# syzhang092218-source/dgppo

Measured on AMD Instinct MI355X. Metric: env-steps/sec whole node, LidarSpread n=8 4096 envs, 1/2/4/8 GPUs, higher is better.
Workload: dtype f32

## Files before the change

dgppo_amd/csrc/graph_feats.hip:

```cpp
#include "graph_topo.h"

struct FeatArgs {
  dgppo_env_cfg cfg;
  Topo t;
  const float* agent; long agent_se, agent_st;
  const float* goal;
  const float* obst;
  const float* hits; long hits_se, hits_st;
  const int32_t* env_ids;
  int n_env, n_time;
  float* Xa;
  float* Xo;
  float* efeat;
  float* emask;
  int Fp;
  uint32_t rcp_fp, rcp_S;
};

template <int SD>
__global__ void graph_feats_kernel(FeatArgs a) {
  extern __shared__ float sm[];
  const dgppo_env_cfg& c = a.cfg;
  const Topo& t = a.t;
  const int g = blockIdx.x;
  const int e = g / a.n_time, tt = g - e * a.n_time;
  const int env = a.env_ids ? a.env_ids[e] : e;
  const int tid = threadIdx.x, nt = blockDim.x;
  const int n = t.n, ng = t.ng, S = t.S, Fp = a.Fp;
  const int n_on = t.Ns - n - ng;
  float* s_ag = sm;
  float* s_go = s_ag + n * SD;
  float* s_ob = s_go + ng * SD;
  float* s_fa = s_ob + n_on * SD;
  float* s_fg = s_fa + n * 4;
  const float* ag = a.agent + (size_t)env * a.agent_se + (size_t)tt * a.agent_st;
  for (int i = tid; i < n * SD; i += nt) s_ag[i] = ag[i];
  for (int i = tid; i < ng * SD; i += nt) s_go[i] = a.goal[(size_t)env * ng * SD + i];
  if (n_on > 0) {
    if (t.lidar) {
      const float* hp = a.hits + (size_t)env * a.hits_se + (size_t)tt * a.hits_st;
      for (int i = tid; i < n_on * 2; i += nt) {
        const int q = i >> 1, d = i & 1;
        s_ob[q * SD + d] = hp[i];
      }
      for (int i = tid; i < n_on * (SD - 2); i += nt) {
        const int q = i / (SD - 2), d = i - q * (SD - 2);
        s_ob[q * SD + 2 + d] = 0.0f;
      }
    } else {
      for (int i = tid; i < n_on * SD; i += nt) s_ob[i] = a.obst[(size_t)env * n_on * SD + i];
    }
  }
  __syncthreads();
  for (int i = tid; i < n + ng; i += nt) {
    const float* s = (i < n) ? s_ag + i * SD : s_go + (i - n) * SD;
    float* f = (i < n) ? s_fa + i * 4 : s_fg + (i - n) * 4;
    if constexpr (SD == 5) {
      f[0] = s[0]; f[1] = s[1]; f[2] = __fmul_rn(s[4], s[2]); f[3] = __fmul_rn(s[4], s[3]);
    } else {
      f[0] = s[0]; f[1] = s[1]; f[2] = s[2]; f[3] = s[3];
    }
  }
  __syncthreads();
  constexpr int ND = SD + 3;
  for (int idx = tid; idx < t.Ns * Fp; idx += nt) {
    const int nd = (int)__umulhi((uint32_t)idx, a.rcp_fp), col = idx - nd * Fp;
    float v = 0.0f;
    if (nd < n) v = (col < SD) ? s_ag[nd * SD + col] : ((col == SD + 2) ? 1.0f : 0.0f);
    else if (nd < n + ng) v = (col < SD) ? s_go[(nd - n) * SD + col] : ((col == SD + 1) ? 1.0f : 0.0f);
    else v = (col < SD) ? s_ob[(nd - n - ng) * SD + col] : ((col == SD) ? 1.0f : 0.0f);
    if (col >= ND) v = 0.0f;
    if (nd < n) a.Xa[((size_t)g * n + nd) * Fp + col] = v;
    else a.Xo[((size_t)g * (t.Ns - n) + (nd - n)) * Fp + col] = v;
  }
  for (int idx = tid; idx < n * S; idx += nt) {
    const int i = (int)__umulhi((uint32_t)idx, a.rcp_S), s = idx - i * S;
    float4 f;
    bool mask;
    const float* fi = s_fa + i * 4;
    const float px = s_ag[i * SD], py = s_ag[i * SD + 1];
    if (s < n) {
      const float* fj = s_fa + s * 4;
      f = make_float4(__fsub_rn(fi[0], fj[0]), __fsub_rn(fi[1], fj[1]), __fsub_rn(fi[2], fj[2]), __fsub_rn(fi[3], fj[3]));
      float d = __fadd_rn(dist_rn(__fsub_rn(px, s_ag[s * SD]), __fsub_rn(py, s_ag[s * SD + 1])), (i == s) ? c.eye_offset : 0.0f);
      mask = d < c.comm_radius;
    } else if (s < n + t.gs) {
      const int gi = t.spread ? (s - n) : i;
      const float* fg = s_fg + gi * 4;
      f = make_float4(__fsub_rn(fi[0], fg[0]), __fsub_rn(fi[1], fg[1]), __fsub_rn(fi[2], fg[2]), __fsub_rn(fi[3], fg[3]));
      mask = true;
    } else {
      const int m = s - n - t.gs;
      if (t.lidar) {
        const float* hp = s_ob + (i * t.per + m) * SD;
        const float lx = __fsub_rn(px, hp[0]), ly = __fsub_rn(py, hp[1]);
        f = make_float4(lx, ly, 0.0f, 0.0f);
        mask = dist_rn(lx, ly) < c.lidar_mask_radius;
      } else {
        const float* xo = s_ob + m * SD;
        const float* xi = s_ag + i * SD;
        f = make_float4(__fsub_rn(xi[0], xo[0]), __fsub_rn(xi[1], xo[1]), __fsub_rn(xi[2], xo[2]), __fsub_rn(xi[3], xo[3]));
        mask = dist_rn(__fsub_rn(xi[0], xo[0]), __fsub_rn(xi[1], xo[1])) < c.obs_mask_radius;
      }
    }
    reinterpret_cast<float4*>(a.efeat)[(size_t)g * n * S + idx] = f;
    a.emask[(size_t)g * n * S + idx] = mask ? 1.0f : 0.0f;
  }
}

extern "C" int32_t dgppo_graph_feats(const dgppo_env_cfg* cfg, const float* agent, int64_t agent_se, int64_t agent_st,
                                     const float* goal, const float* obst, const float* hits, int64_t hits_se,
                                     int64_t hits_st, const int32_t* env_ids, int32_t n_env, int32_t n_time, float* Xa,
                                     float* Xo, float* efeat, float* emask, int32_t Fp, void* stream) {
  int32_t rc = dgppo_validate_cfg(cfg);
  if (rc) return rc;
  DGPPO_REFUSE_VMAS(cfg, "dgppo_graph_feats", "dgppo_vmas_graph_feats");
  DGPPO_REQUIRE(n_env >= 0 && n_time >= 0, "graph_feats: negative counts");
  if (n_env == 0 || n_time == 0) return 0;
  DGPPO_REQUIRE(agent && goal && Xa && efeat && emask, "graph_feats: NULL operand");
  DGPPO_REQUIRE(Fp >= cfg->node_dim && Fp <= 32, "graph_feats: Fp must be in [node_dim, 32]");
  FeatArgs a;
  a.cfg = *cfg; a.t = make_topo(*cfg);
  const int n_on = a.t.Ns - a.t.n - a.t.ng;
  DGPPO_REQUIRE(n_on == 0 || Xo, "graph_feats: Xo is NULL");
  DGPPO_REQUIRE(a.t.Ns == a.t.n || Xo, "graph_feats: Xo is NULL");
  if (n_on > 0) {
    if (a.t.lidar) DGPPO_REQUIRE(hits, "graph_feats: hits is NULL");
    else DGPPO_REQUIRE(obst, "graph_feats: obst is NULL");
  }
  DGPPO_REQUIRE(((uintptr_t)efeat & 15) == 0, "graph_feats: efeat must be 16-byte aligned");
  a.agent = agent; a.agent_se = agent_se; a.agent_st = agent_st; a.goal = goal; a.obst = obst;
  a.hits = hits; a.hits_se = hits_se; a.hits_st = hits_st; a.env_ids = env_ids; a.n_env = n_env; a.n_time = n_time;
  a.Xa = Xa; a.Xo = Xo; a.efeat = efeat; a.emask = emask; a.Fp = Fp;
  a.rcp_fp = (uint32_t)((0x100000000ull + (uint64_t)Fp - 1) / (uint64_t)Fp);
  a.rcp_S = (uint32_t)((0x100000000ull + (uint64_t)a.t.S - 1) / (uint64_t)a.t.S);
  DGPPO_REQUIRE(Fp >= 2 && a.t.S >= 2 && (long)a.t.Ns * Fp < 65536 && (long)a.t.n * a.t.S < 65536, "graph_feats: sizes out of range");
  const int SD = cfg->state_dim;
  const size_t smem = sizeof(float) * ((size_t)a.t.n * SD + a.t.ng * SD + (size_t)n_on * SD + a.t.n * 4 + a.t.ng * 4);
  const long G = (long)n_env * n_time;
  if (SD == 5) hipLaunchKernelGGL(graph_feats_kernel<5>, dim3(G), dim3(128), smem, (hipStream_t)stream, a);
  else hipLaunchKernelGGL(graph_feats_kernel<4>, dim3(G), dim3(128), smem, (hipStream_t)stream, a);
  DGPPO_LAUNCH_CHECK();
  return 0;
}
```

dgppo_amd/csrc/nn_elem.hip:

```cpp
#include "common.h"
#include "nn_ln.h"

using f32x4 = __attribute__((ext_vector_type(4))) float;

__device__ inline float wave_sum(float v) {
#pragma unroll
  for (int o = 32; o >= 1; o >>= 1) v += __shfl_xor(v, o);
  return v;
}
template <int NV>
__device__ inline void block_atomic_sums(const float (&v)[NV], float* dst) {
  __shared__ float s_red[4][NV];
  const int lane = threadIdx.x & 63, wave = threadIdx.x >> 6;
#pragma unroll
  for (int k = 0; k < NV; ++k) {
    const float w = wave_sum(v[k]);
    if (lane == 0) s_red[wave][k] = w;
  }
  __syncthreads();
  if (threadIdx.x < NV) {
    float t = 0.0f;
    for (int w = 0; w < (int)(blockDim.x >> 6); ++w) t += s_red[w][threadIdx.x];
    atomicAdd(dst + threadIdx.x, t);
  }
}

__device__ inline float row16_sum(float v) {
  v += __int_as_float(__builtin_amdgcn_update_dpp(0, __float_as_int(v), 0xB1, 0xf, 0xf, false));
  v += __int_as_float(__builtin_amdgcn_update_dpp(0, __float_as_int(v), 0x4E, 0xf, 0xf, false));
  v += __int_as_float(__builtin_amdgcn_update_dpp(0, __float_as_int(v), 0x141, 0xf, 0xf, false));
  v += __int_as_float(__builtin_amdgcn_update_dpp(0, __float_as_int(v), 0x140, 0xf, 0xf, false));
  return v;
}

__global__ void __launch_bounds__(256) ln_relu_fwd_kernel(const float* __restrict__ x, const float* __restrict__ gamma,
                                                          const float* __restrict__ beta, float* __restrict__ y,
                                                          float* __restrict__ stats, int M) {
  const int lane = threadIdx.x & 63, li = lane & 15, lq = lane >> 4;
  const int wave = (blockIdx.x * blockDim.x + threadIdx.x) >> 6;
  const int nw = (gridDim.x * blockDim.x) >> 6;
  const float4 g = reinterpret_cast<const float4*>(gamma)[li], b = reinterpret_cast<const float4*>(beta)[li];
  for (int row0 = wave * 4; row0 < M; row0 += nw * 4) {
    const int row = row0 + lq;
    const bool ok = row < M;
    const float4 v = reinterpret_cast<const float4*>(x)[(size_t)(ok ? row : M - 1) * 16 + li];
    const float mean = row16_sum((v.x + v.y) + (v.z + v.w)) * (1.0f / 64.0f);
    const float mean2 = row16_sum((v.x * v.x + v.y * v.y) + (v.z * v.z + v.w * v.w)) * (1.0f / 64.0f);
    const float var = ln_fast_var(mean, mean2);
    const float rstd = rsqrtf(var + 1e-6f);
    float4 o;
    o.x = relu_nan((v.x - mean) * rstd * g.x + b.x);
    o.y = relu_nan((v.y - mean) * rstd * g.y + b.y);
    o.z = relu_nan((v.z - mean) * rstd * g.z + b.z);
    o.w = relu_nan((v.w - mean) * rstd * g.w + b.w);
    if (ok) {
      reinterpret_cast<float4*>(y)[(size_t)row * 16 + li] = o;
      if (stats != nullptr && li == 0) reinterpret_cast<float2*>(stats)[row] = make_float2(mean, rstd);
    }
  }
}

__global__ void __launch_bounds__(256) ln_relu_bwd_kernel(const float* __restrict__ x, const float* __restrict__ y,
                                                          const float* __restrict__ stats, const float* __restrict__ gamma,
                                                          const float* __restrict__ dy, float* __restrict__ dx,
                                                          float* __restrict__ dgamma, float* __restrict__ dbeta, int M) {
  const int lane = threadIdx.x & 63, li = lane & 15, lq = lane >> 4;
  const int wave = (blockIdx.x * blockDim.x + threadIdx.x) >> 6;
  const int nw = (gridDim.x * blockDim.x) >> 6;
  const float4 g = reinterpret_cast<const float4*>(gamma)[li];
  float dg[4] = {0.f, 0.f, 0.f, 0.f}, db[4] = {0.f, 0.f, 0.f, 0.f};
  for (int row0 = wave * 4; row0 < M; row0 += nw * 4) {
    const int row = row0 + lq;
    const bool ok = row < M;
    const size_t o = (size_t)(ok ? row : M - 1) * 16 + li;
    const float4 xv = reinterpret_cast<const float4*>(x)[o], yv = reinterpret_cast<const float4*>(y)[o];
    const float4 dv = reinterpret_cast<const float4*>(dy)[o];
    const float2 st = reinterpret_cast<const float2*>(stats)[ok ? row : M - 1];
    const float mean = st.x, rstd = st.y;
    const float xh[4] = {(xv.x - mean) * rstd, (xv.y - mean) * rstd, (xv.z - mean) * rstd, (xv.w - mean) * rstd};
    const float dl[4] = {(ok && yv.x > 0.0f) ? dv.x : 0.0f, (ok && yv.y > 0.0f) ? dv.y : 0.0f,
                         (ok && yv.z > 0.0f) ? dv.z : 0.0f, (ok && yv.w > 0.0f) ? dv.w : 0.0f};
    const float gg[4] = {g.x, g.y, g.z, g.w};
    float dxh[4], s1 = 0.0f, s2 = 0.0f;
#pragma unroll
    for (int q = 0; q < 4; ++q) {
      dg[q] += dl[q] * xh[q];
      db[q] += dl[q];
      dxh[q] = dl[q] * gg[q];
      s1 += dxh[q];
      s2 += dxh[q] * xh[q];
    }
    const float m1 = row16_sum(s1) * (1.0f / 64.0f), m2 = row16_sum(s2) * (1.0f / 64.0f);
    if (ok)
      reinterpret_cast<float4*>(dx)[o] = make_float4(rstd * (dxh[0] - m1 - xh[0] * m2), rstd * (dxh[1] - m1 - xh[1] * m2),
                                                     rstd * (dxh[2] - m1 - xh[2] * m2), rstd * (dxh[3] - m1 - xh[3] * m2));
  }
  __shared__ float red[2][16][64];
  const int slot = (threadIdx.x >> 6) * 4 + lq;
#pragma unroll
  for (int q = 0; q < 4; ++q) { red[0][slot][li * 4 + q] = dg[q]; red[1][slot][li * 4 + q] = db[q]; }
  __syncthreads();
  if (threadIdx.x < 128) {
    const int which = threadIdx.x >> 6;
    float v = 0.0f;
#pragma unroll
    for (int sidx = 0; sidx < 16; ++sidx) v += red[which][sidx][lane];
    atomicAdd((which ? dbeta : dgamma) + lane, v);
  }
}

extern "C" int32_t dgppo_ln_relu_fwd(const float* x, const float* gamma, const float* beta, float* y, float* stats,
                                     int32_t M, void* stream) {
  DGPPO_REQUIRE(M >= 0, "ln_relu_fwd: M < 0");
  if (M == 0) return 0;
  DGPPO_REQUIRE(x && gamma && beta && y, "ln_relu_fwd: NULL operand");
  const int grid = min(cdiv(M, 16), 2048);
  hipLaunchKernelGGL(ln_relu_fwd_kernel, dim3(grid), dim3(256), 0, (hipStream_t)stream, x, gamma, beta, y, stats, M);
  DGPPO_LAUNCH_CHECK();
  return 0;
}

extern "C" int32_t dgppo_ln_relu_bwd(const float* x, const float* y, const float* stats, const float* gamma,
                                     const float* dy, float* dx, float* dgamma, float* dbeta, int32_t M, void* stream) {
  DGPPO_REQUIRE(M >= 0, "ln_relu_bwd: M < 0");
  if (M == 0) return 0;
  DGPPO_REQUIRE(x && y && stats && gamma && dy && dx && dgamma && dbeta, "ln_relu_bwd: NULL operand");
  const int grid = min(cdiv(M, 16), 256);
  hipLaunchKernelGGL(ln_relu_bwd_kernel, dim3(grid), dim3(256), 0, (hipStream_t)stream, x, y, stats, gamma, dy, dx, dgamma,
                     dbeta, M);
  DGPPO_LAUNCH_CHECK();
  return 0;
}

#define GRU_H 64
#define GRU_WL 194
#define GRU_HL 66

struct GruArgs {
  const float* gi;
  const float* Wh;
  const float* bhn;
  const float* h0;
  float* hs;
  float* hprev;
  float* gates;
  const float* dhs;
  float* dgi;
  float* dgh;
  float* dhn;
  int n_seq, T, n_inner;
};

__device__ inline size_t gru_row(const GruArgs& a, int s, int tau) {
  const int grp = s / a.n_inner, i = s - grp * a.n_inner;
  return ((size_t)grp * a.T + tau) * a.n_inner + i;
}
__device__ inline float sigmoidf_(float x) { return 1.0f / (1.0f + expf(-x)); }
__device__ inline float gate_sigmoid(float x) { return __builtin_amdgcn_rcpf(1.0f + __expf(-x)); }
__device__ inline float gate_tanh(float x) { return fmaf(2.0f, __builtin_amdgcn_rcpf(1.0f + __expf(-2.0f * x)), -1.0f); }


#define GRU_LDS_BARRIER() asm volatile("s_waitcnt lgkmcnt(0)\n\ts_barrier" ::: "memory")

template <int RTW>
__global__ void __launch_bounds__(256) gru_fwd_kernel(GruArgs a) {
  extern __shared__ float sm[];
  constexpr int RB = 16 * RTW;
  constexpr int HSLOT = RB * 16 / 256 > 0 ? RB * 16 / 256 : 1;
  const int tid = threadIdx.x, lane = tid & 63, w = tid >> 6, li = lane & 15, lq = lane >> 4;
  const int c = w * 16 + li;
  float breg[16][3];
#pragma unroll
  for (int kk = 0; kk < 16; ++kk)
#pragma unroll
    for (int t = 0; t < 3; ++t) breg[kk][t] = a.Wh[(size_t)(kk * 4 + lq) * 192 + t * 64 + c];
  const float bn = a.bhn[c];
  const int n_tiles = (a.n_seq + RB - 1) / RB;
  const float4 z4 = make_float4(0.f, 0.f, 0.f, 0.f);
  float hpf[HSLOT][4];
  auto fetch_h0 = [&](int tile) {
#pragma unroll
    for (int u = 0; u < HSLOT; ++u) {
      int idx = u * 256 + tid;
      idx = idx < RB * 16 ? idx : RB * 16 - 1;
      const int r = idx >> 4, q = idx & 15;
      int s = tile * RB + r;
      s = s < a.n_seq ? s : a.n_seq - 1;
      float4 v = z4;
      if (a.h0 != nullptr) v = reinterpret_cast<const float4*>(a.h0 + (size_t)s * GRU_H)[q];
      hpf[u][0] = v.x; hpf[u][1] = v.y; hpf[u][2] = v.z; hpf[u][3] = v.w;
    }
  };
  auto commit_h0 = [&](float* dst) {
#pragma unroll
    for (int u = 0; u < HSLOT; ++u) {
      const int idx = u * 256 + tid, r = idx >> 4, q = idx & 15;
      if (idx < RB * 16) { float* d = dst + r * GRU_HL + 4 * q; d[0] = hpf[u][0]; d[1] = hpf[u][1]; d[2] = hpf[u][2]; d[3] = hpf[u][3]; }
    }
  };
  int tile = blockIdx.x;
  if (tile < n_tiles) { fetch_h0(tile); commit_h0(sm); }
  __syncthreads();
  int cur = 0;
  for (; tile < n_tiles; tile += gridDim.x) {
    const int s0 = tile * RB;
    const int nxt = tile + gridDim.x;
    if (nxt < n_tiles) fetch_h0(nxt);
    int row0[RTW][4];
    bool ok[RTW][4];
#pragma unroll
    for (int rt = 0; rt < RTW; ++rt)
#pragma unroll
      for (int r = 0; r < 4; ++r) {
        int s = s0 + rt * 16 + lq * 4 + r;
        ok[rt][r] = s < a.n_seq;
        s = ok[rt][r] ? s : a.n_seq - 1;
        int rw = s;
        if (a.T != 1 && a.n_inner != 1) { const int grp = s / a.n_inner; rw = grp * a.T * a.n_inner + (s - grp * a.n_inner); }
        else if (a.T != 1) rw = s * a.T;
        row0[rt][r] = rw;
      }
    float gn[RTW][4][3];
    auto fetch_gi = [&](int tau) {
#pragma unroll
      for (int rt = 0; rt < RTW; ++rt)
#pragma unroll
        for (int r = 0; r < 4; ++r) {
          const float* gp = a.gi + (size_t)(row0[rt][r] + tau * a.n_inner) * 192 + c;
          gn[rt][r][0] = gp[0]; gn[rt][r][1] = gp[64]; gn[rt][r][2] = gp[128];
        }
    };
    fetch_gi(0);
    for (int tau = 0; tau < a.T; ++tau) {
      const float* hs_cur = sm + cur * (RB * GRU_HL);
      float* hs_nxt = sm + (cur ^ 1) * (RB * GRU_HL);
      float g[RTW][4][3];
#pragma unroll
      for (int rt = 0; rt < RTW; ++rt)
#pragma unroll
        for (int r = 0; r < 4; ++r) { g[rt][r][0] = gn[rt][r][0]; g[rt][r][1] = gn[rt][r][1]; g[rt][r][2] = gn[rt][r][2]; }
      if (tau + 1 < a.T) fetch_gi(tau + 1);
      __builtin_amdgcn_sched_barrier(0);
      float areg[RTW][16];
#pragma unroll
      for (int rt = 0; rt < RTW; ++rt)
#pragma unroll
        for (int kk = 0; kk < 16; ++kk) areg[rt][kk] = hs_cur[(rt * 16 + li) * GRU_HL + kk * 4 + lq];
      __builtin_amdgcn_sched_barrier(0);
      f32x4 acc[RTW][3];
#pragma unroll
      for (int rt = 0; rt < RTW; ++rt)
#pragma unroll
        for (int t = 0; t < 3; ++t) acc[rt][t] = f32x4{0.f, 0.f, 0.f, 0.f};
#pragma unroll
      for (int kk = 0; kk < 16; ++kk)
#pragma unroll
        for (int rt = 0; rt < RTW; ++rt)
#pragma unroll
          for (int t = 0; t < 3; ++t) acc[rt][t] = __builtin_amdgcn_mfma_f32_16x16x4f32(areg[rt][kk], breg[kk][t], acc[rt][t], 0, 0, 0);
#pragma unroll
      for (int rt = 0; rt < RTW; ++rt)
#pragma unroll
        for (int r = 0; r < 4; ++r) {
          const int rl = rt * 16 + lq * 4 + r;
          const float hp = hs_cur[rl * GRU_HL + c];
          const float rg = gate_sigmoid(g[rt][r][0] + acc[rt][0][r]);
          const float zg = gate_sigmoid(g[rt][r][1] + acc[rt][1][r]);
          const float hn = acc[rt][2][r] + bn;
          const float ng = gate_tanh(g[rt][r][2] + rg * hn);
          const float hnew = (1.0f - zg) * ng + zg * hp;
          hs_nxt[rl * GRU_HL + c] = hnew;
          if (ok[rt][r]) {
            const size_t row = (size_t)(row0[rt][r] + tau * a.n_inner);
            a.hs[row * GRU_H + c] = hnew;
            if (a.hprev != nullptr) a.hprev[row * GRU_H + c] = hp;
            if (a.gates != nullptr) {
              float* gs = a.gates + row * 256;
              gs[c] = rg; gs[64 + c] = zg; gs[128 + c] = ng; gs[192 + c] = hn;
            }
          }
        }
      GRU_LDS_BARRIER();
      cur ^= 1;
    }
    if (nxt < n_tiles) {
      commit_h0(sm + cur * (RB * GRU_HL));
      GRU_LDS_BARRIER();
    }
  }
}

template <int RTW, bool DHN_ONLY>
__global__ void __launch_bounds__(256) gru_bwd_kernel(GruArgs a) {
  extern __shared__ float sm[];
  constexpr int RB = 16 * RTW;
  const int tid = threadIdx.x, lane = tid & 63, w = tid >> 6, li = lane & 15, lq = lane >> 4;
  const int c = w * 16 + li;
  float breg[48];
#pragma unroll
  for (int kk = 0; kk < 48; ++kk) breg[kk] = a.Wh[(size_t)c * 192 + kk * 4 + lq];
  const int n_tiles = (a.n_seq + RB - 1) / RB;
  int cur = 0;
  for (int tile = blockIdx.x; tile < n_tiles; tile += gridDim.x) {
    const int s0 = tile * RB;
    int row0[RTW][4];
    bool ok[RTW][4];
#pragma unroll
    for (int rt = 0; rt < RTW; ++rt)
#pragma unroll
      for (int r = 0; r < 4; ++r) {
        int s = s0 + rt * 16 + lq * 4 + r;
        ok[rt][r] = s < a.n_seq;
        s = ok[rt][r] ? s : a.n_seq - 1;
        int rw = s;
        if (a.T != 1 && a.n_inner != 1) { const int grp = s / a.n_inner; rw = grp * a.T * a.n_inner + (s - grp * a.n_inner); }
        else if (a.T != 1) rw = s * a.T;
        row0[rt][r] = rw;
      }
    float rg[RTW][4], zg[RTW][4], ng[RTW][4], hn[RTW][4], hp[RTW][4], du[RTW][4], dh[RTW][4];
    auto fetch = [&](int tau) {
#pragma unroll
      for (int rt = 0; rt < RTW; ++rt)
#pragma unroll
        for (int r = 0; r < 4; ++r) {
          const size_t row = (size_t)(row0[rt][r] + tau * a.n_inner);
          const float* gs = a.gates + row * 256 + c;
          rg[rt][r] = gs[0]; zg[rt][r] = gs[64]; ng[rt][r] = gs[128]; hn[rt][r] = gs[192];
          hp[rt][r] = a.hprev[row * GRU_H + c];
          du[rt][r] = a.dhs[row * GRU_H + c];
        }
    };
#pragma unroll
    for (int rt = 0; rt < RTW; ++rt)
#pragma unroll
      for (int r = 0; r < 4; ++r) dh[rt][r] = 0.0f;
    fetch(a.T - 1);
    for (int tau = a.T - 1; tau >= 0; --tau) {
      float* s_g = sm + cur * (RB * GRU_WL);
#pragma unroll
      for (int rt = 0; rt < RTW; ++rt)
#pragma unroll
        for (int r = 0; r < 4; ++r) {
          const int rl = rt * 16 + lq * 4 + r;
          const float d = ok[rt][r] ? dh[rt][r] + du[rt][r] : 0.0f;
          const float dz = d * (hp[rt][r] - ng[rt][r]);
          const float dn = d * (1.0f - zg[rt][r]);
          const float dan = dn * (1.0f - ng[rt][r] * ng[rt][r]);
          const float dhn = dan * rg[rt][r];
          const float dar = dan * hn[rt][r] * rg[rt][r] * (1.0f - rg[rt][r]);
          const float daz = dz * zg[rt][r] * (1.0f - zg[rt][r]);
          dh[rt][r] = d * zg[rt][r];
          s_g[rl * GRU_WL + c] = dar;
          s_g[rl * GRU_WL + 64 + c] = daz;
          s_g[rl * GRU_WL + 128 + c] = dhn;
          if (ok[rt][r]) {
            const size_t row = (size_t)(row0[rt][r] + tau * a.n_inner);
            float* o = a.dgi + row * 192 + c;
            o[0] = dar; o[64] = daz; o[128] = dan;
            if (DHN_ONLY) {
              a.dhn[row * GRU_H + c] = dhn;
            } else {
              float* p = a.dgh + row * 192 + c;
              p[0] = dar; p[64] = daz; p[128] = dhn;
            }
          }
        }
      GRU_LDS_BARRIER();
      if (tau > 0) fetch(tau - 1);
      __builtin_amdgcn_sched_barrier(0);
      f32x4 acc[RTW];
#pragma unroll
      for (int rt = 0; rt < RTW; ++rt) acc[rt] = f32x4{0.f, 0.f, 0.f, 0.f};
#pragma unroll
      for (int k0 = 0; k0 < 48; k0 += 16) {
        float areg[RTW][16];
#pragma unroll
        for (int rt = 0; rt < RTW; ++rt)
#pragma unroll
          for (int u = 0; u < 16; ++u) areg[rt][u] = s_g[(rt * 16 + li) * GRU_WL + (k0 + u) * 4 + lq];
        __builtin_amdgcn_sched_barrier(0);
#pragma unroll
        for (int u = 0; u < 16; ++u)
#pragma unroll
          for (int rt = 0; rt < RTW; ++rt) acc[rt] = __builtin_amdgcn_mfma_f32_16x16x4f32(areg[rt][u], breg[k0 + u], acc[rt], 0, 0, 0);
      }
#pragma unroll
      for (int rt = 0; rt < RTW; ++rt)
#pragma unroll
        for (int r = 0; r < 4; ++r) dh[rt][r] += acc[rt][r];
      cur ^= 1;
    }
    GRU_LDS_BARRIER();
  }
}

static int gru_resident(const void* fn, size_t smem) {
  int per_cu = 0, dev = 0, cus = 256;
  if (hipOccupancyMaxActiveBlocksPerMultiprocessor(&per_cu, fn, 256, smem) != hipSuccess || per_cu < 1) per_cu = 1;
  if (hipGetDevice(&dev) != hipSuccess ||
      hipDeviceGetAttribute(&cus, hipDeviceAttributeMultiprocessorCount, dev) != hipSuccess || cus < 1) cus = 256;
  return per_cu * cus;
}

static int32_t gru_check(const GruArgs& a) {
  DGPPO_REQUIRE(a.n_seq >= 0 && a.T >= 1 && a.n_inner >= 1, "gru: bad sizes n_seq=%d T=%d n_inner=%d", a.n_seq, a.T, a.n_inner);
  DGPPO_REQUIRE(a.n_seq % a.n_inner == 0, "gru: n_seq must be a multiple of n_inner");
  return 0;
}

extern "C" int32_t dgppo_gru_fwd(const float* gi, const float* Wh, const float* bhn, const float* h0, float* hs,
                                 float* hprev, float* gates, int32_t n_seq, int32_t T, int32_t n_inner, void* stream) {
  GruArgs a{};
  a.gi = gi; a.Wh = Wh; a.bhn = bhn; a.h0 = h0; a.hs = hs; a.hprev = hprev; a.gates = gates;
  a.n_seq = n_seq; a.T = T; a.n_inner = n_inner;
  int32_t rc = gru_check(a);
  if (rc) return rc;
  if (n_seq == 0) return 0;
  DGPPO_REQUIRE(gi && Wh && bhn && hs, "gru_fwd: NULL operand");
  if (cdiv(n_seq, 32) >= 512) {
    const size_t smem = sizeof(float) * 2 * 32 * GRU_HL;
    static thread_local int cap = 0;
    if (cap == 0) cap = gru_resident(reinterpret_cast<const void*>(&gru_fwd_kernel<2>), smem);
    const int tiles = cdiv(n_seq, 32);
    hipLaunchKernelGGL(gru_fwd_kernel<2>, dim3(tiles < cap ? tiles : cap), dim3(256), smem, (hipStream_t)stream, a);
  } else {
    const size_t smem = sizeof(float) * 2 * 16 * GRU_HL;
    static thread_local int cap = 0;
    if (cap == 0) cap = gru_resident(reinterpret_cast<const void*>(&gru_fwd_kernel<1>), smem);
    const int tiles = cdiv(n_seq, 16);
    hipLaunchKernelGGL(gru_fwd_kernel<1>, dim3(tiles < cap ? tiles : cap), dim3(256), smem, (hipStream_t)stream, a);
  }
  DGPPO_LAUNCH_CHECK();
  return 0;
}

template <bool DHN_ONLY>
static int32_t gru_bwd_launch(GruArgs a, hipStream_t stream) {
  int32_t rc = gru_check(a);
  if (rc) return rc;
  if (a.n_seq == 0) return 0;
  DGPPO_REQUIRE(a.dhs && a.Wh && a.hprev && a.gates && a.dgi && (DHN_ONLY ? a.dhn : a.dgh), "gru_bwd: NULL operand");
  if (cdiv(a.n_seq, 32) >= 512) {
    const size_t smem = sizeof(float) * 2 * 32 * GRU_WL;
    static thread_local int cap = 0;
    if (cap == 0) cap = gru_resident(reinterpret_cast<const void*>(&gru_bwd_kernel<2, DHN_ONLY>), smem);
    const int tiles = cdiv(a.n_seq, 32);
    hipLaunchKernelGGL((gru_bwd_kernel<2, DHN_ONLY>), dim3(tiles < cap ? tiles : cap), dim3(256), smem, stream, a);
  } else {
    const size_t smem = sizeof(float) * 2 * 16 * GRU_WL;
    static thread_local int cap = 0;
    if (cap == 0) cap = gru_resident(reinterpret_cast<const void*>(&gru_bwd_kernel<1, DHN_ONLY>), smem);
    const int tiles = cdiv(a.n_seq, 16);
    hipLaunchKernelGGL((gru_bwd_kernel<1, DHN_ONLY>), dim3(tiles < cap ? tiles : cap), dim3(256), smem, stream, a);
  }
  DGPPO_LAUNCH_CHECK();
  return 0;
}

extern "C" int32_t dgppo_gru_bwd(const float* dhs, const float* Wh, const float* hprev, const float* gates, float* dgi,
                                 float* dgh, int32_t n_seq, int32_t T, int32_t n_inner, void* stream) {
  GruArgs a{};
  a.dhs = dhs; a.Wh = Wh; a.hprev = (float*)hprev; a.gates = (float*)gates; a.dgi = dgi; a.dgh = dgh;
  a.n_seq = n_seq; a.T = T; a.n_inner = n_inner;
  return gru_bwd_launch<false>(a, (hipStream_t)stream);
}

extern "C" int32_t dgppo_gru_bwd_dhn(const float* dhs, const float* Wh, const float* hprev, const float* gates, float* dgi,
                                     float* dhn, int32_t n_seq, int32_t T, int32_t n_inner, void* stream) {
  GruArgs a{};
  a.dhs = dhs; a.Wh = Wh; a.hprev = (float*)hprev; a.gates = (float*)gates; a.dgi = dgi; a.dhn = dhn;
  a.n_seq = n_seq; a.T = T; a.n_inner = n_inner;
  return gru_bwd_launch<true>(a, (hipStream_t)stream);
}

#define STD_INIT_INV (-0.43275212956718856f)
#define STD_MIN 1e-5f
#define THRESH 0.999f
#define INV_THRESH 3.8002011672502f
#define LOG_EPS (-6.907755278982137f)
#define HALF_LOG_2PI 0.9189385332046727f
#define LOG2_F 0.6931471805599453f

__device__ inline float softplusf_(float x) { return (x > 20.0f) ? x : log1pf(expf(x)); }
#define NDTR_SERIES_BELOW (-10.0f)
__device__ inline float ndtr_tail_series(float z2) { return 1.0f - 1.0f / z2 + 3.0f / (z2 * z2) - 15.0f / (z2 * z2 * z2); }
__device__ inline float log_ndtrf_(float z) {
  if (z > NDTR_SERIES_BELOW) return logf(0.5f * erfcf(-z * 0.70710678118654752f));
  const float z2 = z * z;
  return -0.5f * z2 - logf(-z) - HALF_LOG_2PI + logf(ndtr_tail_series(z2));
}
__device__ inline float dlog_ndtrf_(float z) {
  if (z > NDTR_SERIES_BELOW) return 0.3989422804014327f * expf(-0.5f * z * z) / (0.5f * erfcf(-z * 0.70710678118654752f));
  return -z / ndtr_tail_series(z * z);
}
__device__ inline float tanh_fldj(float x) { return 2.0f * (LOG2_F - x - softplusf_(-2.0f * x)); }

struct HeadArgs {
  const float* ms;
  const float* eps;
  const float* action_in;
  float* action;
  float* log_pi;
  float* entropy;
  int rows, n_agents, mode;
  const float* log_pi_old;
  const float* adv;
  float* dms;
  float* stats;
  float clip_eps, coef_ent, inv_count;
};

__device__ inline float tn_log_prob_dim(float act, float mu, float sd) {
  const float ac = fminf(fmaxf(act, -THRESH), THRESH);
  if (ac <= -THRESH) return log_ndtrf_((-INV_THRESH - mu) / sd) - LOG_EPS;
  if (ac >= THRESH) return log_ndtrf_(-(INV_THRESH - mu) / sd) - LOG_EPS;
  const float x = atanhf(ac);
  const float z = (x - mu) / sd;
  return -0.5f * z * z - logf(sd) - HALF_LOG_2PI - tanh_fldj(x);
}

__global__ void __launch_bounds__(256) policy_head_kernel(HeadArgs a) {
  float acc[4] = {0.0f, 0.0f, 0.0f, 0.0f};
  const int rows_pad = (a.rows + 255) & ~255;
  for (int row_raw = blockIdx.x * blockDim.x + threadIdx.x; row_raw < rows_pad; row_raw += gridDim.x * blockDim.x) {
  const bool valid = row_raw < a.rows;
  const int row = valid ? row_raw : a.rows - 1;
  const float4 m = reinterpret_cast<const float4*>(a.ms)[row];
  const float mu[2] = {m.x, m.y};
  const float st[2] = {m.z, m.w};
  float sd[2];
  for (int d = 0; d < 2; ++d) sd[d] = softplusf_(st[d] + STD_INIT_INV) + STD_MIN;
  if (a.mode == 1) {
    if (valid) {
      a.action[row * 2] = tanhf(mu[0]);
      a.action[row * 2 + 1] = tanhf(mu[1]);
    }
    continue;
  }
  float act[2];
  if (a.mode == 0) {
    for (int d = 0; d < 2; ++d) act[d] = tanhf(mu[d] + sd[d] * a.eps[row * 2 + d]);
    if (valid) {
      a.action[row * 2] = act[0];
      a.action[row * 2 + 1] = act[1];
      a.log_pi[row] = tn_log_prob_dim(act[0], mu[0], sd[0]) + tn_log_prob_dim(act[1], mu[1], sd[1]);
    }
    continue;
  }
  act[0] = a.action_in[row * 2];
  act[1] = a.action_in[row * 2 + 1];
  const int ag = row % a.n_agents;
  float lp = 0.0f, ent = 0.0f;
  float dlp_dmu[2], dlp_dsd[2], dent_dmu[2], dent_dsd[2];
  for (int d = 0; d < 2; ++d) {
    const float ac = fminf(fmaxf(act[d], -THRESH), THRESH);
    if (ac <= -THRESH) {
      const float u = (-INV_THRESH - mu[d]) / sd[d];
      lp += log_ndtrf_(u) - LOG_EPS;
      const float r = dlog_ndtrf_(u);
      dlp_dmu[d] = -r / sd[d];
      dlp_dsd[d] = -r * u / sd[d];
    } else if (ac >= THRESH) {
      const float u = (mu[d] - INV_THRESH) / sd[d];
      lp += log_ndtrf_(u) - LOG_EPS;
      const float r = dlog_ndtrf_(u);
      dlp_dmu[d] = r / sd[d];
      dlp_dsd[d] = -r * u / sd[d];
    } else {
      const float x = atanhf(ac);
      const float z = (x - mu[d]) / sd[d];
      lp += -0.5f * z * z - logf(sd[d]) - HALF_LOG_2PI - tanh_fldj(x);
      dlp_dmu[d] = z / sd[d];
      dlp_dsd[d] = (z * z - 1.0f) / sd[d];
    }
    const float eh = a.eps[ag * 2 + d];
    const float y = mu[d] + sd[d] * eh;
    ent += 0.5f + HALF_LOG_2PI + logf(sd[d]) + tanh_fldj(y);
    const float th = tanhf(y);
    dent_dmu[d] = -2.0f * th;
    dent_dsd[d] = 1.0f / sd[d] - 2.0f * th * eh;
  }
  if (valid) {
    a.log_pi[row] = lp;
    a.entropy[row] = ent;
  }
  if (a.dms == nullptr) continue;
  const float A = a.adv[row];
  const float rho = expf(lp - a.log_pi_old[row]);
  const float l1 = -rho * A;
  const float l2 = -fminf(fmaxf(rho, 1.0f - a.clip_eps), 1.0f + a.clip_eps) * A;
  const float lsel = fmaxf(l1, l2);
  const float dl_dlp = ((l2 > l1) ? 0.0f : -rho * A) * a.inv_count;
  const float dl_dent = -a.coef_ent * a.inv_count;
  if (valid) {
    float4 o;
    const float dsd0 = dl_dlp * dlp_dsd[0] + dl_dent * dent_dsd[0];
    const float dsd1 = dl_dlp * dlp_dsd[1] + dl_dent * dent_dsd[1];
    o.x = dl_dlp * dlp_dmu[0] + dl_dent * dent_dmu[0];
    o.y = dl_dlp * dlp_dmu[1] + dl_dent * dent_dmu[1];
    o.z = dsd0 * sigmoidf_(st[0] + STD_INIT_INV);
    o.w = dsd1 * sigmoidf_(st[1] + STD_INIT_INV);
    reinterpret_cast<float4*>(a.dms)[row] = o;
  }
  if (valid) {
    acc[0] += lsel; acc[1] += ent; acc[2] += (l2 > l1) ? 1.0f : 0.0f; acc[3] += fabsf(rho - 1.0f);
  }
  }
  if (a.mode == 2 && a.dms != nullptr) block_atomic_sums<4>(acc, a.stats);
}

extern "C" int32_t dgppo_policy_head(const float* ms, const float* eps, const float* action_in, float* action,
                                     float* log_pi, float* entropy, int32_t rows, int32_t n_agents, int32_t mode,
                                     const float* log_pi_old, const float* adv, float* dms, float* stats, float clip_eps,
                                     float coef_ent, void* stream) {
  DGPPO_REQUIRE(rows >= 0 && n_agents >= 1 && mode >= 0 && mode <= 2, "policy_head: bad arguments");
  if (rows == 0) return 0;
  DGPPO_REQUIRE(ms, "policy_head: ms is NULL");
  DGPPO_REQUIRE(((uintptr_t)ms & 15) == 0, "policy_head: ms must be 16-byte aligned");
  if (mode == 0) DGPPO_REQUIRE(eps && action && log_pi, "policy_head(sample): NULL operand");
  if (mode == 1) DGPPO_REQUIRE(action, "policy_head(mode): NULL operand");
  if (mode == 2) {
    DGPPO_REQUIRE(eps && action_in && log_pi && entropy, "policy_head(eval): NULL operand");
    if (dms) DGPPO_REQUIRE(log_pi_old && adv && stats && ((uintptr_t)dms & 15) == 0, "policy_head(eval+loss): NULL operand");
  }
  HeadArgs a{};
  a.ms = ms; a.eps = eps; a.action_in = action_in; a.action = action; a.log_pi = log_pi; a.entropy = entropy;
  a.rows = rows; a.n_agents = n_agents; a.mode = mode; a.log_pi_old = log_pi_old; a.adv = adv; a.dms = dms; a.stats = stats;
  a.clip_eps = clip_eps; a.coef_ent = coef_ent; a.inv_count = 1.0f / (float)rows;
  const int blocks = cdiv(rows, 256);
  hipLaunchKernelGGL(policy_head_kernel, dim3(blocks < 512 ? blocks : 512), dim3(256), 0, (hipStream_t)stream, a);
  DGPPO_LAUNCH_CHECK();
  return 0;
}

__global__ void __launch_bounds__(256) value_loss_kernel(const float* __restrict__ v, const float* __restrict__ target,
                                                         float* __restrict__ dv, float* __restrict__ stats, int count,
                                                         float count_f) {
  float l[1] = {0.0f};
  for (int i = blockIdx.x * blockDim.x + threadIdx.x; i < count; i += gridDim.x * blockDim.x) {
    const float d = v[i] - target[i];
    dv[i] = d / count_f;
    l[0] += 0.5f * d * d;
  }
  block_atomic_sums<1>(l, stats);
}

extern "C" int32_t dgppo_value_loss(const float* v, const float* target, float* dv, float* stats, int32_t count,
                                    void* stream) {
  DGPPO_REQUIRE(count >= 0, "value_loss: count < 0");
  if (count == 0) return 0;
  DGPPO_REQUIRE(v && target && dv && stats, "value_loss: NULL operand");
  const int blocks = cdiv(count, 256);
  hipLaunchKernelGGL(value_loss_kernel, dim3(blocks < 256 ? blocks : 256), dim3(256), 0, (hipStream_t)stream, v, target, dv,
                     stats, count, (float)count);
  DGPPO_LAUNCH_CHECK();
  return 0;
}

__global__ void mean_agents_kernel(const float* __restrict__ x, float* __restrict__ y, int G, int n, int D, int backward,
                                   const float* __restrict__ relu_mask) {
  const int idx = blockIdx.x * blockDim.x + threadIdx.x;
  if (backward) {
    if (idx >= G * n * D) return;
    const int d = idx % D, g = idx / (n * D);
    const float v = (backward == 2) ? y[idx] + x[(size_t)g * D + d] : x[(size_t)g * D + d] / (float)n;
    y[idx] = (relu_mask == nullptr || relu_mask[idx] > 0.0f) ? v : 0.0f;
  } else {
    if (idx >= G * D) return;
    const int d = idx % D, g = idx / D;
    float acc = 0.0f;
    for (int i = 0; i < n; ++i) acc += x[((size_t)g * n + i) * D + d];
    y[idx] = acc / (float)n;
  }
}

extern "C" int32_t dgppo_mean_agents(const float* x, float* y, int32_t G, int32_t n, int32_t D, int32_t backward,
                                     const float* relu_mask, void* stream) {
  DGPPO_REQUIRE(G >= 0 && n >= 1 && D >= 1, "mean_agents: bad sizes");
  DGPPO_REQUIRE(backward >= 0 && backward <= 2, "mean_agents: backward must be 0, 1 or 2");
  if (G == 0) return 0;
  DGPPO_REQUIRE(x && y, "mean_agents: NULL operand");
  const long total = backward ? (long)G * n * D : (long)G * D;
  hipLaunchKernelGGL(mean_agents_kernel, dim3(cdiv(total, 256)), dim3(256), 0, (hipStream_t)stream, x, y, G, n, D, backward,
                     backward ? relu_mask : nullptr);
  DGPPO_LAUNCH_CHECK();
  return 0;
}

__global__ void relu_bwd_kernel(float* __restrict__ dy, const float* __restrict__ y, long count) {
  const long i = (long)blockIdx.x * blockDim.x + threadIdx.x;
  if (i < count && !(y[i] > 0.0f)) dy[i] = 0.0f;
}

extern "C" int32_t dgppo_relu_bwd(float* dy, const float* y, int64_t count, void* stream) {
  DGPPO_REQUIRE(count >= 0, "relu_bwd: count < 0");
  if (count == 0) return 0;
  DGPPO_REQUIRE(dy && y, "relu_bwd: NULL operand");
  hipLaunchKernelGGL(relu_bwd_kernel, dim3(cdiv(count, 256)), dim3(256), 0, (hipStream_t)stream, dy, y, (long)count);
  DGPPO_LAUNCH_CHECK();
  return 0;
}
```

dgppo_amd/engine.py:

```python
from __future__ import annotations

import dataclasses
from typing import Callable, Dict, Optional

import numpy as np
import os
import torch

from . import _native as N
from . import nets
from . import ops_algo as OA
from . import ops_env as OE
from . import ops_nn as K
from .utils import checkpoint as CK


@dataclasses.dataclass
class Hyper:
    gamma: float = 0.99
    gae_lambda: float = 0.95
    clip_eps: float = 0.25
    coef_ent: float = 1e-2
    max_grad_norm: float = 2.0
    lr_actor: float = 3e-4
    lr_Vl: float = 1e-3
    lr_Vh: float = 1e-3
    batch_size: int = 16384
    rnn_step: int = 16
    alpha: float = 10.0
    cbf_eps: float = 1e-2
    cbf_weight: float = 1.0
    cbf_schedule: bool = True
    train_steps: int = 100000
    actor_gnn_layers: int = 2
    Vl_gnn_layers: int = 2
    Vh_gnn_layers: int = 1
    use_rnn: bool = True
    use_lstm: bool = False
    rnn_layers: int = 1
    lagr_init: float = 0.78
    lr_lagr: float = 1e-7
    cost_weight: float = 0.0
    cost_schedule: bool = False


class RolloutData:

    def __init__(self, cfg: N.EnvCfg, B: int, T: int, device, stochastic: bool, carry_dim: int = nets.HID):
        n = cfg.n_agents
        self.cfg, self.B, self.T, self.stochastic = cfg, B, T, stochastic
        z = lambda *s: torch.empty(*s, device=device)
        step, env = OE.record_fields(cfg)
        self.step_tm = {k: z(T + 1, B, *shape) for k, shape in step.items()}
        self.env = {k: z(B, *shape) for k, shape in env.items()}
        self.step: Dict[str, torch.Tensor] = {}
        for k in OE.STEP_FIELDS:
            setattr(self, k + "_tm", self.step_tm.get(k))
            setattr(self, k, None)
        for k in OE.ENV_FIELDS:
            setattr(self, k, self.env.get(k))
        self.action_tm = z(T, B, n, 2)
        self.log_pi_tm = z(T, B, n) if stochastic else None
        self.rnn_tm = z(T + 1, B, n, carry_dim)
        self.reward_tm = z(T, B)
        self.cost_tm = z(T, B, n, cfg.n_cost)
        self._env_major = False
        views = {k: v.unbind(0) for k, v in self.step_tm.items()}
        self.states_tm = [OE.State({k: v[t] for k, v in views.items()}, self.env) for t in range(T + 1)]

    def finalize(self):
        if self._env_major:
            return self

        def tr(name, x):
            if x is None:
                return None
            cur = getattr(self, name, None)
            want = (x.shape[1], x.shape[0]) + tuple(x.shape[2:])
            if cur is None or tuple(cur.shape) != want:
                cur = torch.empty(want, device=x.device, dtype=x.dtype)
            cur.copy_(x.transpose(0, 1))
            return cur
        for k, v in self.step_tm.items():
            self.step[k] = tr(k, v)
            setattr(self, k, self.step[k])
        self.actions = tr("actions", self.action_tm)
        self.log_pis = tr("log_pis", self.log_pi_tm) if self.stochastic else None
        self._rnn_em = tr("_rnn_em", self.rnn_tm)
        self.rnn_states = self._rnn_em[:, :self.T] if self.stochastic else self._rnn_em[:, 1:]
        self.rewards = tr("rewards", self.reward_tm)
        self.costs = tr("costs", self.cost_tm)
        self._env_major = True
        return self


class OptState:
    def __init__(self, n: int, device):
        self.m = torch.zeros(n, device=device)
        self.v = torch.zeros(n, device=device)
        self.state = torch.zeros(N.OPT_STATE_FLOATS, device=device)


class Engine:
    def __init__(self, cfg: N.EnvCfg, hyper: Hyper, device, T: int = 128,
                 allreduce: Optional[Callable[[torch.Tensor], None]] = None, world: int = 1, prepass_graphs: int = 1 << 20,
                 use_graphs: bool = False, multi_stream: bool = False, algo: str = "dgppo", rank: int = 0):
        self.cfg, self.hp, self.device, self.T = cfg, hyper, device, T
        assert algo in ("dgppo", "informarl", "hcbfcrpo", "informarl_lagr"), algo
        self.algo = algo
        self.use_graphs = use_graphs and os.environ.get("DGPPO_HIPGRAPH", "1") != "0"
        self.multi_stream = multi_stream and os.environ.get("DGPPO_MULTI_STREAM", "1") != "0"
        self._side_streams = None
        self._ro_cache: Dict[tuple, dict] = {}
        self._upd_graph: dict = {}
        self.n_cost = cfg.n_cost
        spec = [("policy", "policy", hyper.actor_gnn_layers, 2), ("Vl", "Vl", hyper.Vl_gnn_layers, 1)]
        if algo == "dgppo":
            spec.append(("Vh", "Vh", hyper.Vh_gnn_layers, self.n_cost))
        elif algo == "informarl_lagr":
            spec.append(("Vh", "Vhg", hyper.Vh_gnn_layers, self.n_cost))
        def rnn_kw(name):
            if not hyper.use_rnn:
                return dict(rnn="none", rnn_layers=0)
            if name == "Vh" and algo == "dgppo":
                return dict(rnn="gru", rnn_layers=1)
            return dict(rnn="lstm" if hyper.use_lstm else "gru", rnn_layers=hyper.rnn_layers)
        sizes = [nets.make_layout(kind, cfg.node_dim, layers, n_out, **rnn_kw(k)).size for k, kind, layers, n_out in spec]
        offs, tot = [], 0
        for sz in sizes:
            offs.append(tot)
            tot += (sz + 3) // 4 * 4
        self.flat_grads = torch.zeros(tot + 4 * 8, device=device)
        self.n_reduced = tot + 3 * 8
        self.stats = self.flat_grads[tot:tot + 32].view(4, 8)
        built = {k: nets.Net(kind, cfg, layers, n_out, device, grads=self.flat_grads[o:o + sz], **rnn_kw(k))
                 for (k, kind, layers, n_out), o, sz in zip(spec, offs, sizes)}
        if algo == "informarl_lagr":
            self.lagr = torch.full((cfg.n_agents, self.n_cost), float(hyper.lagr_init), device=device)
            self.lagr_sums = torch.zeros(cfg.n_agents * self.n_cost, device=device)
        self.policy, self.Vl, self.Vh = built["policy"], built["Vl"], built.get("Vh")
        self.HC = self.policy.carry_dim
        self.opt = {k: OptState(net.layout.size, device) for k, net in self.nets.items()}
        self.arena = nets.Arena(device)
        self.allreduce = allreduce
        self.world, self.rank = int(world), int(rank)
        assert self.world >= 1 and (allreduce is not None or self.world == 1), "world > 1 needs an allreduce"
        assert 0 <= self.rank < self.world, f"rank {rank} outside world {world}"
        self.prepass_graphs = int(os.environ.get("DGPPO_PREPASS_GRAPHS", prepass_graphs))
        self.lam_pow = OA.lam_pow_table(hyper.gae_lambda, T, device)
        self.eps_hat = torch.zeros(cfg.n_agents, 2, device=device)
        self.reset_failed = torch.zeros(1, dtype=torch.int32, device=device)
        self.grad_hook: Optional[Callable[[str, nets.Net, int], None]] = None
        self._mb = 0

    @property
    def nets(self) -> Dict[str, nets.Net]:
        d = {"policy": self.policy, "Vl": self.Vl}
        if self.Vh is not None:
            d["Vh"] = self.Vh
        return d

    def set_entropy_noise(self, seed: int):
        OE.randn(seed, 0, self.eps_hat.view(-1))

    _CFG_IDENTITY = ("kind", "n_agents", "n_obs", "n_rays", "top_k", "node_dim", "n_cost")

    def _identity(self) -> dict:
        ident = {"algo": CK.encode_str(self.algo)}
        ident.update({f"cfg.{k}": int(getattr(self.cfg, k)) for k in self._CFG_IDENTITY})
        for f in dataclasses.fields(Hyper):
            v = getattr(self.hp, f.name)
            ident[f"hyper.{f.name}"] = int(v) if isinstance(v, (bool, int)) else float(v)
        ident["T"], ident["world"] = int(self.T), int(self.world)
        ident.update({f"size.{k}": int(net.layout.size) for k, net in self.nets.items()})
        return ident

    def _state_tensors(self) -> Dict[str, torch.Tensor]:
        t = {}
        for k, net in self.nets.items():
            opt = self.opt[k]
            t.update({f"{k}/params": net.params, f"{k}/m": opt.m, f"{k}/v": opt.v, f"{k}/state": opt.state})
        t["eps_hat"] = self.eps_hat
        if self.algo == "informarl_lagr":
            t["lagr"] = self.lagr
        return t

    def state_dict(self) -> dict:
        out = {"identity": self._identity()}
        for path, x in self._state_tensors().items():
            node = out
            *dirs, leaf = path.split("/")
            for d in dirs:
                node = node.setdefault(d, {})
            node[leaf] = x.detach().cpu().numpy().copy()
        return out

    def load_state_dict(self, d: dict) -> None:
        mine, theirs = self._identity(), d.get("identity", {})
        show = lambda v: repr(CK.decode_str(v)) if isinstance(v, np.ndarray) else repr(v)
        for k, v in mine.items():
            if k not in theirs:
                raise ValueError(f"state dict does not fit this engine: it has no identity field '{k}'")
            if not np.array_equal(np.asarray(v), np.asarray(theirs[k])):
                raise ValueError(f"state dict does not fit this engine: '{k}' is {show(theirs[k])} there, {show(v)} here")
        src = {}
        for path, x in self._state_tensors().items():
            node = d
            for part in path.split("/"):
                node = node.get(part) if isinstance(node, dict) else None
            if not isinstance(node, np.ndarray) or node.dtype != np.float32 or node.shape != tuple(x.shape):
                raise ValueError(f"state dict does not fit this engine: '{path}' is not a float32 array of shape {tuple(x.shape)}")
            src[path] = node
        for path, x in self._state_tensors().items():
            x.copy_(torch.from_numpy(src[path]).to(self.device))
        for net in self.nets.values():
            net.prepare()

    def _feats(self, tag, st: OE.State, n_env, n_time=1, slots=1, env_ids=None):
        f = nets.GraphFeats(self.cfg, n_env * n_time, self.arena, tag)
        return f.compute_record(st.step, slots, st.env, env_ids, n_env, n_time)

    def _rollout_steps(self, ro: RolloutData, eps, B: int, stochastic: bool):
        cfg, T, n = self.cfg, self.T, self.cfg.n_agents
        tag = "ro" if stochastic else "rod"
        for t in range(T):
            feats = self._feats(tag, ro.states_tm[t], B)
            act = self.policy.forward(feats, n_seq=B * n, T=1, h0=ro.rnn_tm[t].view(B * n, self.HC), tag=tag,
                                      hs_out=ro.rnn_tm[t + 1].view(B * n, self.HC), train=False)
            a_t = ro.action_tm[t].view(B * n, 2)
            if stochastic:
                K.policy_head(act["ms"], eps[t], None, a_t, ro.log_pi_tm[t].view(B * n), None, n, 0)
            else:
                K.policy_head(act["ms"], None, None, a_t, None, None, n, 1)
            OE.step(cfg, ro.states_tm[t], ro.action_tm[t], ro.states_tm[t + 1], ro.reward_tm[t], ro.cost_tm[t])

    def rollout(self, seeds: torch.Tensor, stochastic: bool, noise_seed: int = 0) -> RolloutData:
        cfg, T = self.cfg, self.T
        B = int(seeds.shape[0])
        n = cfg.n_agents
        slot = None
        if self.use_graphs:
            slot = self._ro_cache.setdefault((B, stochastic), {"ro": None, "graph": None, "gen": -1, "calls": 0})
            if slot["ro"] is None:
                slot["ro"] = RolloutData(cfg, B, T, self.device, stochastic, self.HC)
            ro = slot["ro"]
            ro._env_major = False
        else:
            ro = RolloutData(cfg, B, T, self.device, stochastic, self.HC)
        OE.reset(cfg, seeds, ro.states_tm[0], self.reset_failed)
        ro.rnn_tm[0].zero_()
        eps = None
        if stochastic:
            eps = self.arena.get("ro.eps", T, B * n, 2)
            OE.randn_rows(noise_seed, eps.view(T, B * n * 2), self.world * B * n * 2, self.rank * B * n * 2)
        if slot is None:
            self._rollout_steps(ro, eps, B, stochastic)
            return ro
        slot["calls"] += 1
        if slot["graph"] is not None and slot["gen"] != self._arena_generation():
            slot["graph"] = None
        if slot["graph"] is not None:
            slot["graph"].replay()
            K.FLOPS[0] += slot.get("flops", 0.0)
            return ro
        f0 = K.FLOPS[0]
        self._rollout_steps(ro, eps, B, stochastic)
        slot["flops"] = K.FLOPS[0] - f0
        if not slot.get("failed", False):
            graph = torch.cuda.CUDAGraph()
            try:
                f1 = K.FLOPS[0]
                with torch.cuda.graph(graph, capture_error_mode="thread_local"):
                    self._rollout_steps(ro, eps, B, stochastic)
                K.FLOPS[0] = f1 + slot["flops"]
                slot["graph"], slot["gen"] = graph, self._arena_generation()
                graph.replay()
            except Exception as ex:
                slot["failed"] = True
                torch.cuda.synchronize()
                print(f"[dgppo_amd] HIP-graph capture of the rollout loop failed ({type(ex).__name__}: {ex}); "
                      f"continuing with eager launches", flush=True)
        return ro

    def _update_generation(self) -> int:
        return self.arena.generation + sum(net.arena.generation + net.ws_arena.generation for net in self.nets.values())

    def _arena_generation(self) -> int:
        return self.arena.generation + self.policy.arena.generation

    def rollout_pair(self, seeds: torch.Tensor, det_seeds: torch.Tensor, noise_seed: int = 0):
        if not (self.multi_stream and self.device.type == "cuda"):
            return self.rollout(seeds, True, noise_seed), self.rollout(det_seeds, False)
        main = torch.cuda.current_stream(self.device)
        s0, s1 = self._net_streams()[:2]
        out = [None, None]
        for k, (st, sd, stoch) in enumerate(((s0, seeds, True), (s1, det_seeds, False))):
            st.wait_stream(main)
            with torch.cuda.stream(st):
                out[k] = self.rollout(sd, stoch, noise_seed if stoch else 0)
        main.wait_stream(s0)
        main.wait_stream(s1)
        return out[0], out[1]

    def _block_feats(self, tag, ro: RolloutData, e0, Eb, t0, n_time, env_ids=None):
        envs = slice(e0, None) if env_ids is None else slice(None)
        st = OE.State({k: v[envs, t0] for k, v in ro.step.items()}, {k: v[envs] for k, v in ro.env.items()})
        return self._feats(tag, st, Eb, n_time, self.T + 1, env_ids)

    def _vh_carry(self, ro: RolloutData, e0: int, Eb: int) -> torch.Tensor:
        return ro.rnn_states[e0:e0 + Eb][..., :nets.HID]

    def values_prepass(self, ro: RolloutData, want_Vl: bool, want_Vh: bool = True):
        cfg, T, B = self.cfg, self.T, ro.B
        n, nh, H = cfg.n_agents, self.n_cost, nets.HID
        kind = "ro" if ro.stochastic else "det"
        Vl_buf = self.arena.get(f"tg.Vl.{kind}", B, T + 1) if want_Vl else None
        Vh_buf = self.arena.get(f"tg.Vh.{kind}", B, T + 1, n, nh) if want_Vh else None
        block = max(1, min(B, self.prepass_graphs // (T + 1)))
        for e0 in range(0, B, block):
            Eb = min(block, B - e0)
            feats = self._block_feats("pre", ro, e0, Eb, 0, T + 1)
            if want_Vl:
                act = self.Vl.forward(feats, n_seq=Eb, T=T + 1, h0=None, tag="pre", train=False)
                Vl_buf[e0:e0 + Eb].copy_(act["v"].view(Eb, T + 1))
            if not want_Vh:
                continue
            fin = self._block_feats("fin", ro, e0, Eb, T, 1)
            HC = self.HC
            h_last = self.arena.get("pre.hlast", Eb * n, HC)
            h_last.view(Eb, n, HC).copy_(ro.rnn_states[e0:e0 + Eb, T - 1])
            h0_all = self.arena.get("pre.h0all", Eb, T + 1, n, H)
            hstar = self.arena.get("pre.hstar", Eb * n, HC)
            self.policy.forward(fin, n_seq=Eb * n, T=1, h0=h_last, tag="fin", hs_out=hstar, train=False)
            h0_all[:, :T].copy_(self._vh_carry(ro, e0, Eb))
            h0_all[:, T].copy_(hstar.view(Eb, n, HC)[..., :H])
            act = self.Vh.forward(feats, n_seq=Eb * (T + 1) * n, T=1, h0=h0_all.view(-1, H) if self.hp.use_rnn else None,
                                  tag="pre", train=False)
            Vh_buf[e0:e0 + Eb].copy_(act["v"].view(Eb, T + 1, n, nh))
        return Vl_buf, Vh_buf

    def require_landscape(self):
        if self.algo != "dgppo":
            why = {"informarl_lagr": "its constraint-value net carries its own scan state, which needs a sequence pass first"}
            raise ValueError(f"vh_landscape: algo '{self.algo}' is not supported: "
                             + why.get(self.algo, "it has no constraint-value network"))
        if self.cfg.is_vmas:
            raise ValueError("vh_landscape: VMASReverseTransport is not supported")

    def vh_landscape(self, ro: RolloutData, env_index: int, agent_id: int, frame_ids, xs, ys,
                     events: Optional[list] = None) -> torch.Tensor:
        self.require_landscape()
        cfg, T = self.cfg, self.T
        n, nh, H = cfg.n_agents, self.n_cost, nets.HID
        ro.finalize()
        if not 0 <= int(env_index) < ro.B:
            raise ValueError(f"vh_landscape: env_index {env_index} outside [0, {ro.B})")
        if not 0 <= int(agent_id) < n:
            raise ValueError(f"vh_landscape: agent_id {agent_id} outside [0, {n})")
        frames = np.asarray(frame_ids, dtype=np.int64).reshape(-1)
        if frames.size == 0 or frames.min() < 0 or frames.max() >= T:
            raise ValueError(f"vh_landscape: frame_ids must be a non-empty subset of [0, {T})")
        xs, ys = K.sweep_axis(xs, "xs", self.device), K.sweep_axis(ys, "ys", self.device)
        nx, ny, F = int(xs.numel()), int(ys.numel()), int(frames.size)
        e = int(env_index)
        step = {k: v[e] for k, v in ro.step.items()}
        env = {k: v[e] for k, v in ro.env.items()}
        rc, rs = OE._rays(cfg, self.device)
        carry = self._vh_carry(ro, e, 1)[0] if self.hp.use_rnn else None
        out = torch.empty(F, ny, nx, n, nh, device=self.device)
        ids_dev = torch.from_numpy(frames.astype(np.int32)).to(self.device)
        cap = max(1, self.prepass_graphs)
        fb = max(1, cap // (ny * nx))
        yb = ny if cap >= ny * nx else max(1, cap // nx)
        xb = nx if cap >= nx else cap
        for f0 in range(0, F, fb):
            f1 = min(F, f0 + fb)
            fr = frames[f0:f1]
            for y0 in range(0, ny, yb):
                y1 = min(ny, y0 + yb)
                for x0 in range(0, nx, xb):
                    x1 = min(nx, x0 + xb)
                    P = (y1 - y0) * (x1 - x0)
                    Gb = (f1 - f0) * P
                    feats = nets.GraphFeats(cfg, Gb, self.arena, "land")
                    ev = [torch.cuda.Event(enable_timing=True) for _ in range(3)] if events is not None else None
                    if ev:
                        ev[0].record()
                    feats.compute_sweep(step, env, ids_dev[f0:f1], f1 - f0, agent_id, xs[x0:x1], ys[y0:y1], rc, rs,
                                        frame_max=int(fr.max()))
                    if ev:
                        ev[1].record()
                    h0 = None
                    if carry is not None:
                        h0 = self.arena.get("land.h0", Gb * n, H)
                        for j, t in enumerate(fr):
                            h0.view(f1 - f0, P, n, H)[j].copy_(carry[int(t)].unsqueeze(0).expand(P, n, H))
                    act = self.Vh.forward(feats, n_seq=Gb * n, T=1, h0=h0, tag="land", train=False)
                    out[f0:f1, y0:y1, x0:x1].copy_(act["v"].view(f1 - f0, y1 - y0, x1 - x0, n, nh))
                    if ev:
                        ev[2].record()
                        events.append(tuple(ev))
        return out

    def cost_landscape(self, ro: RolloutData, env_index: int, agent_id: int, frame_ids, xs, ys) -> torch.Tensor:
        cfg, T = self.cfg, self.T
        if cfg.is_vmas:
            raise ValueError("cost_landscape: VMASReverseTransport is not supported")
        n = cfg.n_agents
        ro.finalize()
        if not 0 <= int(env_index) < ro.B:
            raise ValueError(f"cost_landscape: env_index {env_index} outside [0, {ro.B})")
        if not 0 <= int(agent_id) < n:
            raise ValueError(f"cost_landscape: agent_id {agent_id} outside [0, {n})")
        frames = np.asarray(frame_ids, dtype=np.int64).reshape(-1)
        if frames.size == 0 or frames.min() < 0 or frames.max() >= T:
            raise ValueError(f"cost_landscape: frame_ids must be a non-empty subset of [0, {T})")
        xs, ys = K.sweep_axis(xs, "xs", self.device), K.sweep_axis(ys, "ys", self.device)
        nx, ny, F = int(xs.numel()), int(ys.numel()), int(frames.size)
        e = int(env_index)
        step = {k: v[e] for k, v in ro.step.items()}
        env = {k: v[e] for k, v in ro.env.items()}
        rc, rs = OE._rays(cfg, self.device)
        out = torch.empty(F, ny, nx, n, self.n_cost, device=self.device)
        K.cost_sweep(cfg, step["agent"], n * cfg.state_dim, env.get("obst"), step.get("hits"), n * cfg.top_k * 2, rc, rs,
                     frames, F, int(agent_id), xs, ys, out.view(F * ny * nx, n, self.n_cost))
        return out

    def cbf_weight_at(self, step: int) -> float:
        hp = self.hp
        w = hp.cbf_weight
        if hp.cbf_schedule:
            if step >= int(hp.train_steps * 0.5):
                w *= 2
            if step >= int(hp.train_steps * 0.75):
                w *= 2
        return w

    def cost_weight_at(self, step: int) -> float:
        hp = self.hp
        w = hp.cost_weight
        if hp.cost_schedule:
            if step >= int(hp.train_steps * 0.5):
                w *= 5
            if step >= int(hp.train_steps * 0.75):
                w *= 5
        return w

    def targets_hcbfcrpo(self, ro: RolloutData, step: int):
        cfg, T, B, hp = self.cfg, self.T, ro.B, self.hp
        n, nh, dev = cfg.n_agents, self.n_cost, self.device
        Vl, _ = self.values_prepass(ro, want_Vl=True, want_Vh=False)
        fin = OE.State({k: v[:, T].contiguous() for k, v in ro.step.items()}, ro.env)
        A = self.arena
        fin_cost = A.get("tg.fin_cost", B, n, nh)
        OE.step(cfg, fin, torch.zeros(B, n, 2, device=dev), fin.like(), torch.empty(B, device=dev), fin_cost)
        Vh = A.get("tg.Vh.crafted", B, T + 1, n, nh)
        Vh[:, :T].copy_(ro.costs)
        Vh[:, T].copy_(fin_cost)
        Qh = A.get("tg.Qh", B, T, n, nh)
        Ql = A.get("tg.Ql", B, T)
        OA.gae(ro.costs, ro.rewards, Vh, Vl, self.lam_pow, hp.gamma, hp.gae_lambda, Qh, Ql)
        adv = A.get("tg.adv", B, T, n)
        self.stats.zero_()
        OA.advantage(Ql, Vl, Vh, cfg.dt, hp.alpha, hp.cbf_eps, self.cbf_weight_at(step), adv, self.stats[3])
        return dict(Vl=Vl, Vh=Vh, Ql=Ql, Qh=Qh, adv=adv)

    def targets_informarl(self, ro: RolloutData, step: int):
        cfg, T, B, hp = self.cfg, self.T, ro.B, self.hp
        n, nh, dev = cfg.n_agents, self.n_cost, self.device
        Vl, _ = self.values_prepass(ro, want_Vl=True, want_Vh=False)
        A = self.arena
        Vh = A.get("tg.Vh.bcast", B, T + 1, n, nh)
        Vh.copy_(Vl.view(B, T + 1, 1, 1).expand(B, T + 1, n, nh))
        shaped = A.get("tg.shaped", B, T)
        OA.shaped_reward(ro.rewards, ro.costs, self.cost_weight_at(step), shaped)
        Qh = A.get("tg.Qh", B, T, n, nh)
        Ql = A.get("tg.Ql", B, T)
        OA.gae(ro.costs, shaped, Vh, Vl, self.lam_pow, hp.gamma, hp.gae_lambda, Qh, Ql)
        adv = A.get("tg.adv", B, T, n)
        self.stats.zero_()
        OA.advantage(Ql, Vl, None, cfg.dt, 0.0, 0.0, 0.0, adv, self.stats[3])
        return dict(Vl=Vl, Ql=Ql, Qh=Qh, adv=adv)

    def targets_lagr(self, ro: RolloutData, step: int):
        cfg, T, B, hp = self.cfg, self.T, ro.B, self.hp
        n, nh, A = cfg.n_agents, self.n_cost, self.arena
        Vl, _ = self.values_prepass(ro, want_Vl=True, want_Vh=False)
        Vh = A.get("tg.Vh.lagr", B, T + 1, n, nh)
        block = max(1, min(B, self.prepass_graphs // (T + 1)))
        for e0 in range(0, B, block):
            Eb = min(block, B - e0)
            feats = self._block_feats("pre", ro, e0, Eb, 0, T + 1)
            act = self.Vh.forward(feats, n_seq=Eb * n, T=T + 1, h0=None, tag="pre", train=False)
            Vh[e0:e0 + Eb].copy_(act["v"].view(Eb, T + 1, n, nh))
        cpos = A.get("tg.costs_pos", B, T, n, nh)
        OA.relu_fwd(ro.costs, cpos)
        Qh = A.get("tg.Qh", B, T, n, nh)
        Ql = A.get("tg.Ql", B, T)
        OA.gae(cpos, ro.rewards, Vh, Vl, self.lam_pow, hp.gamma, hp.gae_lambda, Qh, Ql)
        adv = A.get("tg.adv", B, T, n)
        Ah = A.get("tg.Ah", B, T, n, nh)
        self.stats.zero_()
        OA.advantage_lagr(Ql, Vl, Qh, Vh, self.lagr, adv, Ah)
        return dict(Vl=Vl, Vh=Vh, Ql=Ql, Qh=Qh, adv=adv, Ah=Ah)

    def _net_streams(self):
        if self._side_streams is None:
            self._side_streams = [torch.cuda.Stream(self.device) for _ in range(3)]
        return self._side_streams

    def _opt_step(self, name: str, lr: float):
        net, opt = self.nets[name], self.opt[name]
        if self.grad_hook is not None:
            self.grad_hook(name, net, self._mb)
        OA.clip_adam_step(net.params, net.grads, opt.m, opt.v, opt.state, lr, self.hp.max_grad_norm,
                          grad_scale=1.0 / self.world)
        net.prepare()

    def targets(self, ro: RolloutData, det: RolloutData, step: int):
        cfg, T, B, hp = self.cfg, self.T, ro.B, self.hp
        n, nh = cfg.n_agents, self.n_cost
        Vl, Vh = self.values_prepass(ro, want_Vl=True)
        _, Vh_det = self.values_prepass(det, want_Vl=False)
        A = self.arena
        Qh = A.get("tg.Qh", B, T, n, nh)
        Ql = A.get("tg.Ql", B, T)
        OA.gae(ro.costs, ro.rewards, Vh, Vl, self.lam_pow, hp.gamma, hp.gae_lambda, Qh, Ql)
        Qh_det = A.get("tg.Qh_det", B, T, n, nh)
        Ql_det = A.get("tg.Ql_det", B, T)
        OA.gae(det.costs, det.rewards, Vh_det, Vl, self.lam_pow, hp.gamma, hp.gae_lambda, Qh_det, Ql_det)
        adv = A.get("tg.adv", B, T, n)
        self.stats.zero_()
        OA.advantage(Ql, Vl, Vh, cfg.dt, hp.alpha, hp.cbf_eps, self.cbf_weight_at(step), adv, self.stats[3])
        return dict(Vl=Vl, Vh=Vh, Vh_det=Vh_det, Ql=Ql, Qh=Qh, Qh_det=Qh_det, adv=adv)

    def update(self, ro: RolloutData, det: RolloutData, step: int, perm: np.ndarray) -> dict:
        cfg, T, B, hp = self.cfg, self.T, ro.B, self.hp
        n, nh, H = cfg.n_agents, self.n_cost, nets.HID
        informarl = self.algo in ("informarl", "hcbfcrpo")
        lagr = self.algo == "informarl_lagr"
        import time as _time
        th = [_time.perf_counter()]
        ro.finalize()
        if self.algo == "dgppo":
            det.finalize()
        assert B * T >= hp.batch_size, "n_env_train * T must be >= batch_size (dgppo.py:153)"
        Eb = hp.batch_size // T
        assert B % Eb == 0 and T % hp.rnn_step == 0, "B % (batch_size // T) == 0 and T % rnn_step == 0 required (SURVEY A.11)"
        C = T // hp.rnn_step
        tg = (self.targets_informarl(ro, step) if self.algo == "informarl" else
              self.targets_hcbfcrpo(ro, step) if self.algo == "hcbfcrpo" else
              self.targets_lagr(ro, step) if lagr else self.targets(ro, det, step))
        th.append(_time.perf_counter())
        idx_all = torch.from_numpy(np.ascontiguousarray(perm.astype(np.int64))).to(self.device)
        n_mb = B // Eb
        G = Eb * T
        R = G * n
        is_cuda = self.device.type == "cuda"
        reduce = self.allreduce is not None
        A = self.arena
        mb_idx = A.get("mb.idx", Eb, dtype=torch.int64)
        mb_idx32 = A.get("mb.idx32", Eb, dtype=torch.int32)
        Ql_mb = A.get("mb.Ql", Eb, T)
        act_mb = A.get("mb.act", Eb, T, n, 2)
        lp_old_mb = A.get("mb.lp_old", Eb, T, n)
        adv_mb = A.get("mb.adv", Eb, T, n)
        if self.algo == "dgppo":
            h0_det = A.get("mb.h0_det", Eb, T, n, H)
            Qh_det_mb = A.get("mb.Qh_det", Eb, T, n, nh)
        if lagr:
            Qh_mb = A.get("mb.Qh", Eb, T, n, nh)
            Vh_mb = A.get("mb.Vh", Eb, T + 1, n, nh)
            Ah_mb = A.get("mb.Ah", Eb, T, n, nh)

        ctx = {}

        def lagr_step(apply_now: bool):
            full = self.policy.forward(ctx["feats"], n_seq=Eb * n, T=T, h0=None, tag="lg", train=False)
            lp_full = A.get("mb.lp_full", R)
            K.policy_head(full["ms"], self.eps_hat, act_mb.view(R, 2), None, lp_full, A.get("mb.ent_full", R), n, 2)
            if apply_now:
                OA.lagr_update(lp_full.view(Eb, T, n), lp_old_mb, Vh_mb, Ah_mb, self.lagr, self.lagr_sums, hp.gamma, hp.lr_lagr)
            else:
                OA.lagr_sums(lp_full.view(Eb, T, n), lp_old_mb, Vh_mb, Ah_mb, self.lagr_sums, hp.gamma)

        def body_pre():
            main = torch.cuda.current_stream(self.device) if is_cuda else None
            side = self._net_streams() if (self.multi_stream and main is not None) else None
            self.stats[:3].zero_()
            feats = ctx["feats"] = self._block_feats("mb", ro, 0, Eb, 0, T, env_ids=mb_idx32)
            torch.index_select(tg["Ql"], 0, mb_idx, out=Ql_mb)
            if self.algo == "dgppo":
                feats_det = self._block_feats("mbd", det, 0, Eb, 0, T, env_ids=mb_idx32)
                if self.HC == H:
                    torch.index_select(det.rnn_states, 0, mb_idx, out=h0_det)
                else:
                    full = A.get("mb.h0_det_full", Eb, T, n, self.HC)
                    torch.index_select(det.rnn_states, 0, mb_idx, out=full)
                    h0_det.copy_(full[..., :H])
                torch.index_select(tg["Qh_det"], 0, mb_idx, out=Qh_det_mb)
            if lagr:
                torch.index_select(tg["Qh"], 0, mb_idx, out=Qh_mb)
                torch.index_select(tg["Vh"], 0, mb_idx, out=Vh_mb)
                torch.index_select(tg["Ah"], 0, mb_idx, out=Ah_mb)
            torch.index_select(ro.actions, 0, mb_idx, out=act_mb)
            torch.index_select(ro.log_pis, 0, mb_idx, out=lp_old_mb)
            torch.index_select(tg["adv"], 0, mb_idx, out=adv_mb)

            def update_Vl():
                act = self.Vl.forward(feats, n_seq=Eb * C, T=hp.rnn_step, h0=None, tag="tr")
                dv = A.get("mb.dv", G, 1)
                K.value_loss(act["v"], Ql_mb.view(G, 1), dv, self.stats[0])
                self.Vl.zero_grads()
                self.Vl.backward(act, dv)
                if not reduce:
                    self._opt_step("Vl", hp.lr_Vl)

            def update_Vh():
                if lagr:
                    act = self.Vh.forward(feats, n_seq=Eb * C * n, T=hp.rnn_step, h0=None, tag="tr")
                    target = Qh_mb
                else:
                    act = self.Vh.forward(feats_det, n_seq=R, T=1, h0=h0_det.view(R, H) if hp.use_rnn else None, tag="tr")
                    target = Qh_det_mb
                dvh = A.get("mb.dvh", R, nh)
                K.value_loss(act["v"], target.view(R, nh), dvh, self.stats[1])
                self.Vh.zero_grads()
                self.Vh.backward(act, dvh)
                if not reduce:
                    self._opt_step("Vh", hp.lr_Vh)

            def update_policy():
                act = self.policy.forward(feats, n_seq=Eb * C * n, T=hp.rnn_step, h0=None, tag="tr")
                lp = A.get("mb.lp", R)
                ent = A.get("mb.ent", R)
                dms = A.get("mb.dms", R, 4)
                K.policy_head(act["ms"], self.eps_hat, act_mb.view(R, 2), None, lp, ent, n, 2, lp_old_mb.view(R),
                              adv_mb.view(R), dms, self.stats[2], hp.clip_eps, hp.coef_ent)
                self.policy.zero_grads()
                self.policy.backward(act, dms)
                if not reduce:
                    self._opt_step("policy", hp.lr_actor)
                if lagr and not reduce:
                    lagr_step(apply_now=True)

            if informarl:
                update_Vh = lambda: None
            if side is None:
                update_Vl(); update_Vh(); update_policy()
            else:
                ready = main.record_event()
                for fn, st in ((update_policy, side[0]), (update_Vl, side[1]), (update_Vh, side[2])):
                    with torch.cuda.stream(st):
                        st.wait_event(ready)
                        fn()
                for st in side:
                    main.wait_stream(st)

        def body_post():
            self._opt_step("Vl", hp.lr_Vl)
            if not informarl:
                self._opt_step("Vh", hp.lr_Vh)
            self._opt_step("policy", hp.lr_actor)
            if lagr:
                lagr_step(apply_now=False)

        def exchange_lagr():
            self.allreduce(self.lagr_sums)
            OA.lagr_apply(self.lagr, self.lagr_sums, self.world * Eb * T, hp.lr_lagr)

        def exchange():
            self.allreduce(self.flat_grads[:self.n_reduced])

        def step_body():
            body_pre()
            if reduce:
                exchange()
                body_post()
                if lagr:
                    exchange_lagr()

        slot = None
        if self.use_graphs and is_cuda and self.grad_hook is None:
            key = (self.algo, B, Eb, ro.agent.data_ptr(), det.agent.data_ptr() if det is not None else 0,
                   tg["adv"].data_ptr(), tg["Ql"].data_ptr(), mb_idx.data_ptr(), self._update_generation())
            slot = self._upd_graph
            if slot.get("key") != key:
                slot.clear()
                slot["key"] = key
        for mb in range(n_mb):
            self._mb = mb
            mb_idx.copy_(idx_all[mb * Eb:(mb + 1) * Eb])
            mb_idx32.copy_(mb_idx)
            if slot is not None and slot.get("graph") is not None:
                slot["graph"].replay()
                if reduce:
                    exchange()
                    slot["graph_post"].replay()
                    if lagr:
                        exchange_lagr()
                K.FLOPS[0] += slot["flops"]
                continue
            f0 = K.FLOPS[0]
            step_body()
            if slot is not None and not slot.get("failed", False):
                slot["flops"] = K.FLOPS[0] - f0
                if slot.get("key")[-1] != self._update_generation():
                    slot["key"] = slot["key"][:-1] + (self._update_generation(),)
                    continue
                graph = torch.cuda.CUDAGraph()
                try:
                    f1 = K.FLOPS[0]
                    with torch.cuda.graph(graph, capture_error_mode="thread_local"):
                        body_pre()
                    if reduce:
                        gpost = torch.cuda.CUDAGraph()
                        with torch.cuda.graph(gpost, capture_error_mode="thread_local"):
                            body_post()
                        slot["graph_post"] = gpost
                    K.FLOPS[0] = f1
                    slot["graph"] = graph
                except Exception as ex:
                    slot["failed"] = True
                    torch.cuda.synchronize()
                    print(f"[dgppo_amd] HIP-graph capture of the minibatch step failed ({type(ex).__name__}: {ex}); "
                          f"continuing with eager launches", flush=True)
        th.append(_time.perf_counter())
        self._last = dict(Ql_mb=Ql_mb, G=G, R=R, nh=nh, B=B, Qh_mb=Qh_mb if lagr else None)
        out = self.info(ro)
        th.append(_time.perf_counter())
        self.host_ms = {"issue_targets": 1e3 * (th[1] - th[0]), "issue_minibatches": 1e3 * (th[2] - th[1]),
                        "wait_device": 1e3 * (th[3] - th[2])}
        return out

    def info(self, ro: RolloutData) -> dict:
        from . import dist as D
        L = self._last
        s = self.stats.cpu().numpy().copy()
        n_bad = int(self.reset_failed.item())
        if n_bad:
            self.reset_failed.zero_()
            raise RuntimeError(f"env reset: {n_bad} environment(s) of the last rollouts got no valid scene within the kernels' "
                               f"rejection-loop bounds (too many agents / obstacles for the area?) — the batch is invalid")
        s[:3] /= self.world
        G, R, nh, B = L["G"], L["R"], L["nh"], L["B"]
        o = {k: self.opt[k].state[:8].cpu().numpy() for k in self.opt}
        pol_loss = s[2, 0] / R - self.hp.coef_ent * s[2, 1] / R
        lagr = self.algo == "informarl_lagr"
        ext = [float(L["Ql_mb"].max()), -float(L["Ql_mb"].min()), -float(ro.log_pis.min())]
        if lagr:
            ext += [float(L["Qh_mb"].max()), -float(L["Qh_mb"].min())]
        ext = D.host_allreduce(np.asarray(ext, np.float64), "max", self.world)
        safe = float(D.host_allreduce(np.asarray([s[3, 0]], np.float64), "sum", self.world)[0])
        out = {
            "Vl/loss": float(s[0, 0] / G), "Vl/grad_norm": float(o["Vl"][4]), "Vl/has_nan": float(o["Vl"][5]),
            "Vl/max_target": float(ext[0]), "Vl/min_target": float(-ext[1]),
            "policy/loss": float(pol_loss), "policy/grad_norm": float(o["policy"][4]), "policy/has_nan": float(o["policy"][5]),
            "policy/log_pi_min": float(-ext[2]), "policy/clip_frac": float(s[2, 2] / R),
            "policy/entropy": float(s[2, 1] / R), "policy/total_variation_dist": float(0.5 * s[2, 3] / R),
        }
        if lagr:
            out.update({"Vh/loss": float(s[1, 0] / (R * nh)), "Vh/grad_norm": float(o["Vh"][4]), "Vh/has_nan": float(o["Vh"][5]),
                        "Vh/max_target": float(ext[3]), "Vh/min_target": float(-ext[4]),
                        "policy/lagr_mean": float(self.lagr.mean())})
        if self.algo == "dgppo":
            out.update({"Vh/loss_Vh": float(s[1, 0] / (R * nh)), "Vh/grad_Vh_norm": float(o["Vh"][4]),
                        "Vh/grad_Vh_has_nan": float(o["Vh"][5])})
        if self.algo in ("dgppo", "hcbfcrpo"):
            out["eval/safe_data"] = safe / (self.world * B * self.T * self.cfg.n_agents)
        return out
```

dgppo_amd/nets.py:

```python
from __future__ import annotations

import math
from typing import Dict, List, Optional, Tuple

import numpy as np
import torch

from . import _native as N
from . import ops_nn as K

H_HEADS = 3
MSG_DIM = 32
OUT_DIM = 64
HID = 64


def _ceil4(x):
    return (x + 3) // 4 * 4


class Layout:
    def __init__(self):
        self.entries: Dict[str, Tuple[int, Tuple[int, ...]]] = {}
        self.size = 0

    def add(self, name, *shape):
        n = int(np.prod(shape))
        self.size = (self.size + 3) // 4 * 4
        self.entries[name] = (self.size, tuple(shape))
        self.size += n

    def view(self, flat: torch.Tensor, name: str) -> torch.Tensor:
        off, shape = self.entries[name]
        return flat[off:off + math.prod(shape)].view(shape)


def make_layout(kind: str, node_dim: int, gnn_layers: int, n_out: int, rnn: str = "gru", rnn_layers: int = 1) -> Layout:
    L = Layout()
    f = node_dim
    for l in range(gnn_layers):
        d = OUT_DIM if l == gnn_layers - 1 else MSG_DIM
        hd = H_HEADS * d
        for nm, shp in (("Wq", (f, hd)), ("bq", (hd,)), ("Wk", (f, hd)), ("bk", (hd,)), ("Wv", (f, hd)), ("bv", (hd,)),
                        ("We", (4, hd)), ("Wu", (f, d)), ("bu", (d,))):
            L.add(f"gnn{l}.{nm}", *shp)
        f = d
    for i in (1, 2):
        L.add(f"mlp.W{i}", 2 * HID if (kind == "Vhg" and i == 1) else HID, HID)
        L.add(f"mlp.b{i}", HID)
        L.add(f"mlp.g{i}", HID)
        L.add(f"mlp.be{i}", HID)
    assert rnn in ("gru", "lstm", "none"), rnn
    for l in range(rnn_layers if rnn == "lstm" else 0):
        L.add(f"lstm{l}.Wi", HID, 4 * HID)
        L.add(f"lstm{l}.Wh", HID, 4 * HID)
        L.add(f"lstm{l}.bh", 4 * HID)
    for l in range(rnn_layers if rnn == "gru" else 0):
        pre = "gru" if l == 0 else f"gru{l}"
        L.add(f"{pre}.Wi", HID, 3 * HID)
        L.add(f"{pre}.bi", 3 * HID)
        L.add(f"{pre}.Wh", HID, 3 * HID)
        L.add(f"{pre}.bhn", HID)
    if kind == "policy":
        L.add("head.Ws", HID, HID)
        L.add("head.bs", HID)
        L.add("head.Wms", HID, 2 * n_out)
        L.add("head.bms", 2 * n_out)
    else:
        L.add("head.Wo", HID, n_out)
        L.add("head.bo", n_out)
    return L


class Arena:

    def __init__(self, device):
        self.device = device
        self.bufs: Dict[str, torch.Tensor] = {}
        self.generation = 0

    def get(self, name: str, *shape, dtype=torch.float32, zero=False) -> torch.Tensor:
        n = math.prod(shape)
        b = self.bufs.get(name)
        if b is None or b.numel() < n or b.dtype != dtype:
            if b is not None:
                self.generation += 1
            b = torch.empty(max(n, 1), dtype=dtype, device=self.device)
            self.bufs[name] = b
        v = b[:n].view(shape)
        if zero:
            v.zero_()
        return v


class GraphFeats:

    def __init__(self, cfg: N.EnvCfg, G: int, arena: Arena, tag: str):
        self.cfg, self.G = cfg, G
        n, S = cfg.n_agents, cfg.fan_in
        self.n_other = cfg.num_nodes - 1 - n
        self.Fp = input_width(cfg)
        self.Xa = arena.get(f"{tag}.Xa0", G * n, self.Fp)
        self.Xo = arena.get(f"{tag}.Xo0", max(G * self.n_other, 1), self.Fp)[:G * self.n_other]
        self.efeat = arena.get(f"{tag}.efeat", G * n, S, 4)
        self.emask = arena.get(f"{tag}.emask", G * n, S)

    def compute(self, agent, agent_se, agent_st, goal, obst, hits, hits_se, hits_st, env_ids, n_env, n_time):
        assert n_env * n_time == self.G
        K.graph_feats(self.cfg, agent, agent_se, agent_st, goal, obst, hits, hits_se, hits_st, env_ids, n_env, n_time,
                      self.Xa, self.Xo if self.n_other > 0 else None, self.efeat, self.emask, self.Fp)
        return self

    def compute_record(self, step, slots: int, env, env_ids, n_env, n_time):
        cfg, n = self.cfg, self.cfg.n_agents
        se, st = slots, int(slots > 1)
        if cfg.is_vmas:
            return self.compute_vmas(step["agent"], se * n * 4, st * n * 4, step["body"], se * 4, st * 4, env["scene"], env_ids,
                                     n_env, n_time)
        ia, ih = n * cfg.state_dim, n * cfg.top_k * 2
        return self.compute(step["agent"], se * ia, st * ia, env["goal"], env.get("obst"), step.get("hits"), se * ih, st * ih,
                            env_ids, n_env, n_time)

    def compute_sweep(self, step, env, frame_ids, n_frames, agent_id, xs, ys, ray_cos=None, ray_sin=None, hits_out=None,
                      frame_max=None):
        cfg, n = self.cfg, self.cfg.n_agents
        if cfg.is_vmas:
            raise ValueError("compute_sweep: VMASReverseTransport has no sweep entry point")
        K.graph_feats_sweep(cfg, step["agent"], n * cfg.state_dim, env["goal"], env.get("obst"), step.get("hits"),
                            n * cfg.top_k * 2, ray_cos, ray_sin, frame_ids, n_frames, agent_id, xs, ys, self.Xa,
                            self.Xo if self.n_other > 0 else None, self.efeat, self.emask, self.Fp, hits_out, frame_max)
        return self

    def compute_vmas(self, agent, agent_se, agent_st, body, body_se, body_st, scene, env_ids, n_env, n_time):
        assert n_env * n_time == self.G
        K.vmas_graph_feats(self.cfg, agent, agent_se, agent_st, body, body_se, body_st, scene, env_ids, n_env, n_time,
                           self.Xa, self.efeat, self.emask, self.Fp)
        return self


def input_width(cfg: N.EnvCfg) -> int:
    return _ceil4(cfg.node_dim) if cfg.is_vmas else 8


class Net:

    def __init__(self, kind: str, cfg: N.EnvCfg, gnn_layers: int, n_out: int, device, grads: Optional[torch.Tensor] = None,
                 rnn: str = "gru", rnn_layers: int = 1):
        assert kind in ("policy", "Vl", "Vh", "Vhg")
        self.kind, self.cfg, self.gnn_layers, self.n_out, self.device = kind, cfg, gnn_layers, n_out, device
        self.rnn, self.rnn_layers = rnn, (rnn_layers if rnn != "none" else 0)
        self.carry_dim = HID * max(self.rnn_layers, 1) * (2 if rnn == "lstm" else 1)
        self.layout = make_layout(kind, cfg.node_dim, gnn_layers, n_out, rnn, rnn_layers)
        self.params = torch.zeros(self.layout.size, device=device)
        if grads is None:
            grads = torch.zeros(self.layout.size, device=device)
        assert grads.shape == (self.layout.size,) and grads.is_contiguous() and grads.data_ptr() % 16 == 0
        self.grads = grads
        self.arena = Arena(device)
        self.ws_arena = Arena(device)
        self._views: Dict[tuple, torch.Tensor] = {}
        self.dims = []
        f = cfg.node_dim
        for l in range(gnn_layers):
            d = OUT_DIM if l == gnn_layers - 1 else MSG_DIM
            fp = input_width(cfg) if l == 0 else f
            kp = _ceil4(fp + H_HEADS * (fp + 4) + 1)
            self.dims.append((f, fp, d, kp))
            f = d
        self.prep_layout = Layout()
        for l, (f, fp, d, kp) in enumerate(self.dims):
            self.prep_layout.add(f"gnn{l}.Mcat", fp, H_HEADS * fp)
            self.prep_layout.add(f"gnn{l}.cvec", H_HEADS * fp)
            self.prep_layout.add(f"gnn{l}.Wout", kp, d)
        self.prep = torch.zeros(self.prep_layout.size, device=device)
        self.prep_grads = torch.zeros(self.prep_layout.size, device=device)

    def _cached(self, kind: str, layout, flat, name):
        key = (kind, name)
        v = self._views.get(key)
        if v is None:
            v = self._views[key] = layout.view(flat, name)
        return v

    def p(self, name):
        return self._cached("p", self.layout, self.params, name)

    def g(self, name):
        return self._cached("g", self.layout, self.grads, name)

    def pp(self, name):
        return self._cached("pp", self.prep_layout, self.prep, name)

    def pg(self, name):
        return self._cached("pg", self.prep_layout, self.prep_grads, name)

    def prepare(self):
        for l, (f, fp, d, kp) in enumerate(self.dims):
            q = lambda nm: self.p(f"gnn{l}.{nm}")
            K.gnn_prep(q("Wq"), q("bq"), q("Wk"), q("Wv"), q("bv"), q("We"), q("Wu"), self.pp(f"gnn{l}.Mcat"),
                       self.pp(f"gnn{l}.cvec"), self.pp(f"gnn{l}.Wout"), f, fp, d, H_HEADS, kp)

    def _xo_fusable(self, l: int) -> bool:
        if l != 0 or self.gnn_layers != 2:
            return False
        key = "_xo_ok"
        if not hasattr(self, key):
            f1, fp1, d1, kp1 = self.dims[1]
            setattr(self, key, self.dims[0][1] == 8 and self.dims[0][2] == 32 and fp1 == 32 and
                    K.attn_xo_supported(self.cfg, fp1, H_HEADS, kp1))
        return getattr(self, key)

    def zero_grads(self):
        self.grads.zero_()

    def forward(self, feats: GraphFeats, n_seq: int, T: int, h0: Optional[torch.Tensor], tag: str = "f",
                hs_out: Optional[torch.Tensor] = None, train: bool = True):
        cfg, G, A = self.cfg, feats.G, self.arena
        n = cfg.n_agents
        R = G * n
        Ro = G * feats.n_other
        act = {"feats": feats, "G": G, "n_seq": n_seq, "T": T}
        Xa, Xo = feats.Xa, feats.Xo
        xo_fused = None
        for l, (f, fp, d, kp) in enumerate(self.dims):
            qt = A.get(f"{tag}.qt{l}", R, H_HEADS * fp)
            K.dense_fwd(Xa, self.pp(f"gnn{l}.Mcat"), self.pp(f"gnn{l}.cvec"), qt)
            zcat = A.get(f"{tag}.zcat{l}", R, kp)
            attn = A.get(f"{tag}.attn{l}", R, cfg.fan_in, H_HEADS) if train else None
            if xo_fused is not None:
                K.attn_fwd_xo(cfg, fp, H_HEADS, kp, qt, Xa, xo_fused[0], xo_fused[1], xo_fused[2], feats.efeat, feats.emask, zcat, attn, G)
            else:
                K.attn_fwd(cfg, fp, H_HEADS, kp, qt, Xa, Xo if Ro > 0 else None, feats.efeat, feats.emask, zcat, attn, G)
            act[f"xo_fused{l}"] = xo_fused
            xo_fused = None
            Xa_n = A.get(f"{tag}.Xa{l + 1}", R, d)
            K.dense_fwd(zcat, self.pp(f"gnn{l}.Wout"), self.p(f"gnn{l}.bu"), Xa_n, act=1)
            act[f"Xa{l}"], act[f"Xo{l}"], act[f"qt{l}"], act[f"zcat{l}"], act[f"attn{l}"] = Xa, Xo, qt, zcat, attn
            if l < self.gnn_layers - 1 and Ro > 0:
                if self._xo_fusable(l):
                    xo_fused = (Xo, self.pp(f"gnn{l}.Wout")[:fp], self.p(f"gnn{l}.bu"))
                    Xo = None
                else:
                    Xo_n = A.get(f"{tag}.Xo{l + 1}", Ro, d)
                    K.dense_fwd(Xo, self.pp(f"gnn{l}.Wout")[:fp], self.p(f"gnn{l}.bu"), Xo_n, act=1)
                    Xo = Xo_n
            Xa = Xa_n
        act[f"Xa{self.gnn_layers}"] = Xa
        if self.kind == "Vl":
            pooled = A.get(f"{tag}.pool", G, OUT_DIM)
            K.mean_agents(Xa, pooled, G, n, OUT_DIM)
            x, Rh, n_inner = pooled, G, 1
        else:
            x, Rh, n_inner = Xa, R, n
        if self.kind == "Vhg":
            pooled = A.get(f"{tag}.pool", G, OUT_DIM)
            K.mean_agents(Xa, pooled, G, n, OUT_DIM)
            xcat = A.get(f"{tag}.xcat", R, 2 * OUT_DIM)
            xcat[:, :OUT_DIM].copy_(Xa)
            xcat.view(G, n, 2 * OUT_DIM)[:, :, OUT_DIM:].copy_(pooled.view(G, 1, OUT_DIM).expand(G, n, OUT_DIM))
            x = xcat
        act["Rh"], act["n_inner"], act["mlp_in"] = Rh, n_inner, x
        gi = A.get(f"{tag}.gi", Rh, 3 * HID)
        if self.kind == "Vhg" or self.rnn != "gru":
            sv = {nm: A.get(f"{tag}.{nm}", Rh, w) for nm, w in (("p1", HID), ("y1", HID), ("st1", 2), ("p2", HID), ("y2", HID), ("st2", 2))}
            K.dense_fwd(x, self.p("mlp.W1"), self.p("mlp.b1"), sv["p1"])
            K.ln_relu_fwd(sv["p1"], self.p("mlp.g1"), self.p("mlp.be1"), sv["y1"], sv["st1"])
            K.dense_fwd(sv["y1"], self.p("mlp.W2"), self.p("mlp.b2"), sv["p2"])
            K.ln_relu_fwd(sv["p2"], self.p("mlp.g2"), self.p("mlp.be2"), sv["y2"], sv["st2"])
            if self.rnn == "gru":
                K.dense_fwd(sv["y2"], self.p("gru.Wi"), self.p("gru.bi"), gi)
            act.update(sv)
        else:
            saves = None
            if train:
                saves = tuple(A.get(f"{tag}.{nm}{i}", Rh, w) for i in (1, 2) for nm, w in (("p", HID), ("y", HID), ("st", 2)))
                for i in (1, 2):
                    act[f"p{i}"], act[f"y{i}"], act[f"st{i}"] = saves[3 * (i - 1):3 * i]
            K.mlp_gi_fwd(x, self.p("mlp.W1"), self.p("mlp.b1"), self.p("mlp.g1"), self.p("mlp.be1"), self.p("mlp.W2"),
                         self.p("mlp.b2"), self.p("mlp.g2"), self.p("mlp.be2"), self.p("gru.Wi"), self.p("gru.bi"), gi, saves)
        assert n_seq * T == Rh, (n_seq, T, Rh)
        L, CD = self.rnn_layers, self.carry_dim
        if h0 is not None:
            assert tuple(h0.shape) == (n_seq, CD), (tuple(h0.shape), n_seq, CD)
        if hs_out is not None:
            assert tuple(hs_out.shape) == (Rh, CD), (tuple(hs_out.shape), Rh, CD)
        act["gi"] = gi
        simple = (self.rnn == "gru" and L == 1)
        if simple:
            hs = hs_out if hs_out is not None else A.get(f"{tag}.hs", Rh, HID)
            hprev_is_h0 = train and T == 1 and h0 is not None and self.kind != "policy"
            hprev = A.get(f"{tag}.hprev", Rh, HID) if (train and not hprev_is_h0) else None
            gates = A.get(f"{tag}.gates", Rh, 4 * HID) if train else None
            feat = hs
            act["hs"], act["hprev"], act["gates"] = hs, hprev, gates
        fused_tail = (simple and T == 1 and self.kind == "policy")
        if simple and not fused_tail:
            K.gru_fwd(gi, self.p("gru.Wh"), self.p("gru.bhn"), h0, hs, hprev, gates, n_seq, T, n_inner)
            if hprev_is_h0:
                act["hprev"] = h0
        if self.rnn == "none":
            feat = act["y2"]
            if hs_out is not None:
                if h0 is not None and T == 1:
                    hs_out.copy_(h0)
                else:
                    hs_out.zero_()
        elif self.rnn == "lstm":
            x_l = act["y2"]
            act["stack"] = []
            for l in range(L):
                zi = A.get(f"{tag}.zi{l}", Rh, 4 * HID)
                for half in (slice(0, 2 * HID), slice(2 * HID, 4 * HID)):
                    K.dense_fwd(x_l, self.p(f"lstm{l}.Wi")[:, half], None, zi[:, half])
                c0_l = h0_l = None
                if h0 is not None:
                    c0_l, h0_l = A.get(f"{tag}.c0_{l}", n_seq, HID), A.get(f"{tag}.h0_{l}", n_seq, HID)
                    c0_l.copy_(h0[:, (2 * l) * HID:(2 * l + 1) * HID])
                    h0_l.copy_(h0[:, (2 * l + 1) * HID:(2 * l + 2) * HID])
                cs_l, hs_l = A.get(f"{tag}.cs{l}", Rh, HID), A.get(f"{tag}.hs{l}", Rh, HID)
                cprev_l = A.get(f"{tag}.cprev{l}", Rh, HID) if train else None
                hprev_l = A.get(f"{tag}.hprev{l}", Rh, HID) if train else None
                gates_l = A.get(f"{tag}.gates{l}", Rh, 4 * HID) if train else None
                K.lstm_fwd(zi, self.p(f"lstm{l}.Wh"), self.p(f"lstm{l}.bh"), c0_l, h0_l, cs_l, hs_l, cprev_l, hprev_l, gates_l,
                           n_seq, T, n_inner)
                if hs_out is not None:
                    hs_out[:, (2 * l) * HID:(2 * l + 1) * HID].copy_(cs_l)
                    hs_out[:, (2 * l + 1) * HID:(2 * l + 2) * HID].copy_(hs_l)
                act["stack"].append(dict(x=x_l, hs=hs_l, cprev=cprev_l, hprev=hprev_l, gates=gates_l))
                x_l = hs_l
            feat = x_l
        elif not simple:
            x_l = None
            act["stack"] = []
            for l in range(L):
                pre = "gru" if l == 0 else f"gru{l}"
                gi_l = gi if l == 0 else A.get(f"{tag}.gi{l}", Rh, 3 * HID)
                if l > 0:
                    K.dense_fwd(x_l, self.p(f"{pre}.Wi"), self.p(f"{pre}.bi"), gi_l)
                h0_l = None
                if h0 is not None:
                    h0_l = A.get(f"{tag}.h0_{l}", n_seq, HID)
                    h0_l.copy_(h0[:, l * HID:(l + 1) * HID])
                hs_l = A.get(f"{tag}.hs{l}", Rh, HID)
                hprev_l = A.get(f"{tag}.hprev{l}", Rh, HID) if train else None
                gates_l = A.get(f"{tag}.gates{l}", Rh, 4 * HID) if train else None
                K.gru_fwd(gi_l, self.p(f"{pre}.Wh"), self.p(f"{pre}.bhn"), h0_l, hs_l, hprev_l, gates_l, n_seq, T, n_inner)
                if hs_out is not None:
                    hs_out[:, l * HID:(l + 1) * HID].copy_(hs_l)
                act["stack"].append(dict(x=x_l, gi=gi_l, hs=hs_l, hprev=hprev_l, gates=gates_l))
                x_l = hs_l
            feat = x_l
        act["feat"] = feat
        if self.kind == "policy":
            u = A.get(f"{tag}.u", Rh, HID) if (train or not fused_tail) else None
            ms = A.get(f"{tag}.ms", Rh, 4)
            if fused_tail:
                K.gru1_head_fwd(gi, self.p("gru.Wh"), self.p("gru.bhn"), h0, self.p("head.Ws"), self.p("head.bs"),
                                self.p("head.Wms"), self.p("head.bms"), hs, hprev, gates, u, ms)
            else:
                K.dense_fwd(feat, self.p("head.Ws"), self.p("head.bs"), u)
                K.dense_fwd(u, self.p("head.Wms"), self.p("head.bms"), ms)
            act["u"], act["ms"] = u, ms
        else:
            v = A.get(f"{tag}.v", Rh, self.n_out)
            K.dense_fwd(feat, self.p("head.Wo"), self.p("head.bo"), v)
            act["v"] = v
        return act

    def backward(self, act, dout: torch.Tensor, tag: str = "b"):
        A = self.arena
        ws_floats = getattr(self, "_bwdw_floats", 16 << 20)

        def _alloc(n_floats):
            self._bwdw_floats = max(ws_floats, n_floats)
            return self.ws_arena.get(f"{tag}.bwdw_ws", self._bwdw_floats)
        batch = K.BwdWBatch(self.device, _alloc) if dout.is_cuda else None
        if batch is not None:
            batch.__enter__()
        try:
            self._backward_body(act, dout, tag)
        except BaseException:
            if batch is not None:
                batch.__exit__(RuntimeError, None, None)
            raise
        if batch is not None:
            batch.__exit__(None, None, None)
        for l, (f, fp, d, kp) in enumerate(self.dims):
            q = lambda nm: self.p(f"gnn{l}.{nm}")
            gq = lambda nm: self.g(f"gnn{l}.{nm}")
            K.gnn_unprep(self.pg(f"gnn{l}.Mcat"), self.pg(f"gnn{l}.cvec"), self.pg(f"gnn{l}.Wout"), q("Wq"), q("bq"), q("Wk"),
                         gq("Wq"), gq("bq"), gq("Wk"), gq("Wv"), gq("bv"), gq("We"), gq("Wu"), f, fp, d, H_HEADS, kp)
        self.prep_grads.zero_()

    def _backward_body(self, act, dout: torch.Tensor, tag: str):
        cfg, A = self.cfg, self.arena
        G, Rh, n_inner, n_seq, T = act["G"], act["Rh"], act["n_inner"], act["n_seq"], act["T"]
        n = cfg.n_agents
        R = G * n
        feats: GraphFeats = act["feats"]
        Ro = G * feats.n_other
        feat = act["feat"]
        fused_trunk = self.rnn == "gru" and self.rnn_layers == 1 and self.kind != "Vhg" and dout.is_cuda
        dgi0 = None
        dhs = A.get(f"{tag}.dhs", Rh, HID)
        if self.kind == "policy":
            K.dense_bwd_w(act["u"], dout, self.g("head.Wms"), self.g("head.bms"))
            du = A.get(f"{tag}.du", Rh, HID)
            K.dense_fwd(dout, self.p("head.Wms"), None, du, trans_w=True)
            K.dense_bwd_w(feat, du, self.g("head.Ws"), self.g("head.bs"))
            K.dense_fwd(du, self.p("head.Ws"), None, dhs, trans_w=True)
        else:
            K.dense_bwd_w(feat, dout, self.g("head.Wo"), self.g("head.bo"))
            K.dense_fwd(dout, self.p("head.Wo"), None, dhs, trans_w=True)
        if self.rnn == "none":
            dy = dhs
        elif self.rnn == "lstm":
            stack = act["stack"]
            for l in range(len(stack) - 1, -1, -1):
                st = stack[l]
                dz = A.get(f"{tag}.dz_lstm{l}", Rh, 4 * HID)
                K.lstm_bwd(dhs, self.p(f"lstm{l}.Wh"), st["cprev"], st["gates"], dz, n_seq, T, n_inner)
                for half in (slice(0, 2 * HID), slice(2 * HID, 4 * HID)):
                    K.dense_bwd_w(st["hprev"], dz[:, half], self.g(f"lstm{l}.Wh")[:, half], self.g(f"lstm{l}.bh")[half])
                    K.dense_bwd_w(st["x"], dz[:, half], self.g(f"lstm{l}.Wi")[:, half], None)
                dx = A.get(f"{tag}.dy" if l == 0 else f"{tag}.dx{l}", Rh, HID)
                K.dense_fwd(dz, self.p(f"lstm{l}.Wi"), None, dx, trans_w=True)
                dhs = dx
            dy = dhs
        else:
            stack = act.get("stack") or [dict(x=None, gi=act["gi"], hs=act["hs"], hprev=act["hprev"], gates=act["gates"])]
            if act.get("stack") is None and dout.is_cuda:
                st = stack[0]
                dgi = A.get(f"{tag}.dgi0", Rh, 3 * HID)
                dhn = A.get(f"{tag}.dhn0", Rh, HID)
                K.gru_bwd_dhn(dhs, self.p("gru.Wh"), st["hprev"], st["gates"], dgi, dhn, n_seq, T, n_inner)
                K.gru_bwd_w(act["y2"], st["hprev"], dgi, dhn, self.g("gru.Wi"), self.g("gru.bi"), self.g("gru.Wh"), self.g("gru.bhn"))
                if fused_trunk:
                    dgi0 = dgi
                else:
                    dhs = A.get(f"{tag}.dy", Rh, HID)
                    K.dense_fwd(dgi, self.p("gru.Wi"), None, dhs, trans_w=True)
                stack = []
            for l in range(len(stack) - 1, -1, -1):
                st = stack[l]
                pre = "gru" if l == 0 else f"gru{l}"
                dgi = A.get(f"{tag}.dgi{l}", Rh, 3 * HID)
                dgh = A.get(f"{tag}.dgh{l}", Rh, 3 * HID)
                K.gru_bwd(dhs, self.p(f"{pre}.Wh"), st["hprev"], st["gates"], dgi, dgh, n_seq, T, n_inner)
                K.dense_bwd_w(st["hprev"], dgh[:, :2 * HID], self.g(f"{pre}.Wh")[:, :2 * HID], None)
                K.dense_bwd_w(st["hprev"], dgh[:, 2 * HID:], self.g(f"{pre}.Wh")[:, 2 * HID:], self.g(f"{pre}.bhn"))
                x_l = act["y2"] if l == 0 else st["x"]
                K.dense_bwd_w(x_l, dgi, self.g(f"{pre}.Wi"), self.g(f"{pre}.bi"))
                if l == 0 and fused_trunk:
                    dgi0 = dgi
                    break
                dx = A.get(f"{tag}.dy" if l == 0 else f"{tag}.dx{l}", Rh, HID)
                K.dense_fwd(dgi, self.p(f"{pre}.Wi"), None, dx, trans_w=True)
                dhs = dx
            dy = dhs
        x_in = {1: act["mlp_in"], 2: act["y1"]}
        top = act[f"Xa{self.gnn_layers}"]
        if fused_trunk:
            dpre2, dpre1 = A.get(f"{tag}.dpre2", Rh, HID), A.get(f"{tag}.dpre1", Rh, HID)
            dy = A.get(f"{tag}.dyy1", Rh, HID)
            K.mlp_gi_bwd(dgi0, self.p("gru.Wi"), self.p("mlp.W2"), self.p("mlp.W1"), self.p("mlp.g2"), self.p("mlp.g1"),
                         act["p2"], act["y2"], act["st2"], act["p1"], act["y1"], act["st1"],
                         top if self.kind in ("policy", "Vh") else None, dpre2, dpre1, dy,
                         self.g("mlp.g2"), self.g("mlp.be2"), self.g("mlp.g1"), self.g("mlp.be1"))
            K.dense_bwd_w(x_in[2], dpre2, self.g("mlp.W2"), self.g("mlp.b2"))
            K.dense_bwd_w(x_in[1], dpre1, self.g("mlp.W1"), self.g("mlp.b1"))
        for i in (() if fused_trunk else (2, 1)):
            dpre = A.get(f"{tag}.dpre{i}", Rh, HID)
            K.ln_relu_bwd(act[f"p{i}"], act[f"y{i}"], act[f"st{i}"], self.p(f"mlp.g{i}"), dy, dpre, self.g(f"mlp.g{i}"),
                          self.g(f"mlp.be{i}"))
            K.dense_bwd_w(x_in[i], dpre, self.g(f"mlp.W{i}"), self.g(f"mlp.b{i}"))
            dy = A.get(f"{tag}.dyy{i}", Rh, HID if not (self.kind == "Vhg" and i == 1) else 2 * HID)
            K.dense_fwd(dpre, self.p(f"mlp.W{i}"), None, dy, trans_w=True,
                        relu_mask=top if (i == 1 and self.kind in ("policy", "Vh")) else None)
        if self.kind == "Vl":
            dXa = A.get(f"{tag}.dXaL", R, OUT_DIM)
            K.mean_agents(dy, dXa, G, n, OUT_DIM, backward=True, relu_mask=top)
        elif self.kind == "Vhg":
            dXa = A.get(f"{tag}.dXaL", R, OUT_DIM)
            dXa.copy_(dy[:, :OUT_DIM])
            dglob = A.get(f"{tag}.dglob", R, OUT_DIM)
            dglob.copy_(dy[:, OUT_DIM:])
            dpool = A.get(f"{tag}.dpool", G, OUT_DIM)
            K.mean_agents(dglob, dpool, G, n, OUT_DIM)
            K.mean_agents(dpool, dXa, G, n, OUT_DIM, backward=2, relu_mask=top)
        else:
            dXa = dy
        dXo = None
        for l in range(self.gnn_layers - 1, -1, -1):
            f, fp, d, kp = self.dims[l]
            K.dense_bwd_w(act[f"zcat{l}"], dXa, self.pg(f"gnn{l}.Wout"), self.g(f"gnn{l}.bu"))
            dz = A.get(f"{tag}.dz{l}", R, kp)
            K.dense_fwd(dXa, self.pp(f"gnn{l}.Wout"), None, dz, trans_w=True)
            if dXo is not None:
                K.dense_bwd_w(act[f"Xo{l}"], dXo, self.pg(f"gnn{l}.Wout")[:fp], self.g(f"gnn{l}.bu"))
            dqt = A.get(f"{tag}.dqt{l}", R, H_HEADS * fp)
            need_dx = l > 0
            dXa_l = A.get(f"{tag}.dXa{l}", R, fp) if need_dx else None
            dXo_prev = dXo
            dXo_l = A.get(f"{tag}.dXo{l}", Ro, fp) if (need_dx and Ro > 0) else None
            more_dXo = dXo_prev is not None and dXo_l is not None
            xf = act.get(f"xo_fused{l}")
            if xf is not None and dXa_l is not None and not more_dXo:
                ws = A.get(f"{tag}.xo_ws", K.attn_xo_workspace_floats(G), 1).view(-1)
                K.attn_bwd_xo_dw(cfg, fp, H_HEADS, kp, dz, act[f"attn{l}"], act[f"qt{l}"], act[f"Xa{l}"], xf[0], xf[1], xf[2],
                                 feats.efeat, dqt, dXa_l, self.pg(f"gnn{l - 1}.Wout")[:self.dims[l - 1][1]], self.g(f"gnn{l - 1}.bu"), ws, G)
                dXo_l = None
            elif xf is not None:
                K.attn_bwd_xo(cfg, fp, H_HEADS, kp, dz, act[f"attn{l}"], act[f"qt{l}"], act[f"Xa{l}"], xf[0], xf[1], xf[2],
                              feats.efeat, dqt, dXa_l, dXo_l, G, relu_xo=(dXo_l is not None and not more_dXo))
            else:
                K.attn_bwd(cfg, fp, H_HEADS, kp, dz, act[f"attn{l}"], act[f"qt{l}"], act[f"Xa{l}"],
                           act[f"Xo{l}"] if Ro > 0 else None, feats.efeat, dqt, dXa_l, dXo_l, G,
                           relu_xo=(dXo_l is not None and not more_dXo))
            K.dense_bwd_w(act[f"Xa{l}"], dqt, self.pg(f"gnn{l}.Mcat"), self.pg(f"gnn{l}.cvec"))
            if need_dx:
                K.dense_fwd(dqt, self.pp(f"gnn{l}.Mcat"), None, dXa_l, accumulate=True, trans_w=True, relu_mask=act[f"Xa{l}"])
                if more_dXo:
                    K.dense_fwd(dXo_prev, self.pp(f"gnn{l}.Wout")[:fp], None, dXo_l, accumulate=True, trans_w=True,
                                relu_mask=act[f"Xo{l}"])
            dXa, dXo = dXa_l, dXo_l

    def load_tree(self, tree: dict):
        t = tree["params"]
        to = lambda x: torch.as_tensor(np.asarray(x), dtype=torch.float32).to(self.device)
        if self.kind == "policy":
            base, gnn, head_name = t["PolicyNet_0"], t["PolicyNet_0"]["GraphTransformerGNN_0"], "PolicyGNNHead"
        else:
            base, gnn, head_name = t, t["GraphTransformerGNN_0"], "ValueGNNHead"
        for l in range(self.gnn_layers):
            gl = gnn[f"GraphTransformer_{l}"]
            for nm, dn, key in (("Wq", "Dense_0", "kernel"), ("bq", "Dense_0", "bias"), ("Wk", "Dense_1", "kernel"),
                                ("bk", "Dense_1", "bias"), ("Wv", "Dense_2", "kernel"), ("bv", "Dense_2", "bias"),
                                ("We", "Dense_3", "kernel"), ("Wu", "Dense_4", "kernel"), ("bu", "Dense_4", "bias")):
                self.p(f"gnn{l}.{nm}").copy_(to(gl[dn][key]))
        hd = base[head_name]
        for i in (1, 2):
            self.p(f"mlp.W{i}").copy_(to(hd[f"Dense_{i - 1}"]["kernel"]))
            self.p(f"mlp.b{i}").copy_(to(hd[f"Dense_{i - 1}"]["bias"]))
            self.p(f"mlp.g{i}").copy_(to(hd[f"LayerNorm_{i - 1}"]["scale"]))
            self.p(f"mlp.be{i}").copy_(to(hd[f"LayerNorm_{i - 1}"]["bias"]))
        for l in range(self.rnn_layers if self.rnn == "lstm" else 0):
            lc = base["RNN_0"][f"LSTMCell_{3 * l + 2}"]
            self.p(f"lstm{l}.Wi").copy_(torch.cat([to(lc[k]["kernel"]) for k in ("ii", "if", "ig", "io")], dim=1))
            self.p(f"lstm{l}.Wh").copy_(torch.cat([to(lc[k]["kernel"]) for k in ("hi", "hf", "hg", "ho")], dim=1))
            self.p(f"lstm{l}.bh").copy_(torch.cat([to(lc[k]["bias"]) for k in ("hi", "hf", "hg", "ho")]))
        for l in range(self.rnn_layers if self.rnn == "gru" else 0):
            pre = "gru" if l == 0 else f"gru{l}"
            gr = base["RNN_0"][f"GRUCell_{2 * l + 1}"]
            self.p(f"{pre}.Wi").copy_(torch.cat([to(gr[k]["kernel"]) for k in ("ir", "iz", "in")], dim=1))
            self.p(f"{pre}.bi").copy_(torch.cat([to(gr[k]["bias"]) for k in ("ir", "iz", "in")]))
            self.p(f"{pre}.Wh").copy_(torch.cat([to(gr[k]["kernel"]) for k in ("hr", "hz", "hn")], dim=1))
            self.p(f"{pre}.bhn").copy_(to(gr["hn"]["bias"]))
        if self.kind == "policy":
            self.p("head.Ws").copy_(to(t["ScaleHid"]["kernel"]))
            self.p("head.bs").copy_(to(t["ScaleHid"]["bias"]))
            self.p("head.Wms").copy_(torch.cat([to(t["OutputDenseMean"]["kernel"]), to(t["OutputDenseStdTrans"]["kernel"])], 1))
            self.p("head.bms").copy_(torch.cat([to(t["OutputDenseMean"]["bias"]), to(t["OutputDenseStdTrans"]["bias"])]))
        else:
            self.p("head.Wo").copy_(to(t["Dense_0"]["kernel"]))
            self.p("head.bo").copy_(to(t["Dense_0"]["bias"]))
        self.prepare()

    def to_tree(self, flat: Optional[torch.Tensor] = None) -> dict:
        flat = self.params if flat is None else flat
        v = lambda nm: self.layout.view(flat, nm).detach().cpu().numpy().copy()
        gnn = {}
        for l in range(self.gnn_layers):
            gnn[f"GraphTransformer_{l}"] = {
                "Dense_0": {"kernel": v(f"gnn{l}.Wq"), "bias": v(f"gnn{l}.bq")},
                "Dense_1": {"kernel": v(f"gnn{l}.Wk"), "bias": v(f"gnn{l}.bk")},
                "Dense_2": {"kernel": v(f"gnn{l}.Wv"), "bias": v(f"gnn{l}.bv")},
                "Dense_3": {"kernel": v(f"gnn{l}.We")},
                "Dense_4": {"kernel": v(f"gnn{l}.Wu"), "bias": v(f"gnn{l}.bu")},
            }
        head = {}
        for i in (1, 2):
            head[f"Dense_{i - 1}"] = {"kernel": v(f"mlp.W{i}"), "bias": v(f"mlp.b{i}")}
            head[f"LayerNorm_{i - 1}"] = {"scale": v(f"mlp.g{i}"), "bias": v(f"mlp.be{i}")}
        rnn = {}
        for l in range(self.rnn_layers if self.rnn == "lstm" else 0):
            Wi, Wh, bh = v(f"lstm{l}.Wi"), v(f"lstm{l}.Wh"), v(f"lstm{l}.bh")
            cell = {}
            for q, g_ in enumerate("ifgo"):
                cell["i" + g_] = {"kernel": Wi[:, q * 64:(q + 1) * 64]}
                cell["h" + g_] = {"kernel": Wh[:, q * 64:(q + 1) * 64], "bias": bh[q * 64:(q + 1) * 64]}
            rnn[f"LSTMCell_{3 * l + 2}"] = cell
        for l in range(self.rnn_layers if self.rnn == "gru" else 0):
            pre = "gru" if l == 0 else f"gru{l}"
            Wi, bi, Wh = v(f"{pre}.Wi"), v(f"{pre}.bi"), v(f"{pre}.Wh")
            rnn[f"GRUCell_{2 * l + 1}"] = {
                "ir": {"kernel": Wi[:, :64], "bias": bi[:64]}, "iz": {"kernel": Wi[:, 64:128], "bias": bi[64:128]},
                "in": {"kernel": Wi[:, 128:], "bias": bi[128:]}, "hr": {"kernel": Wh[:, :64]}, "hz": {"kernel": Wh[:, 64:128]},
                "hn": {"kernel": Wh[:, 128:], "bias": v(f"{pre}.bhn")}}
        if self.kind == "policy":
            Wms, bms = v("head.Wms"), v("head.bms")
            k = self.n_out
            return {"params": {
                "PolicyNet_0": dict({"GraphTransformerGNN_0": gnn, "PolicyGNNHead": head}, **({"RNN_0": rnn} if rnn else {})),
                "ScaleHid": {"kernel": v("head.Ws"), "bias": v("head.bs")},
                "OutputDenseMean": {"kernel": Wms[:, :k], "bias": bms[:k]},
                "OutputDenseStdTrans": {"kernel": Wms[:, k:], "bias": bms[k:]}}}
        return {"params": dict({"GraphTransformerGNN_0": gnn, "ValueGNNHead": head, "Dense_0": {"kernel": v("head.Wo"), "bias": v("head.bo")}},
                               **({"RNN_0": rnn} if rnn else {}))}
```

dgppo_amd/ops_nn.py:

```python
from __future__ import annotations

import ctypes as C
from typing import Optional

import numpy as np
import torch

from . import _native as N

FLOPS = [0.0]


def _mat(t: torch.Tensor, name: str):
    if t.dim() != 2:
        raise ValueError(f"{name} must be 2-D, got {tuple(t.shape)}")
    if not t.is_cuda:
        raise RuntimeError(f"{name} must live on the GPU (the HIP path has no CPU fallback)")
    if t.dtype != torch.float32:
        raise TypeError(f"{name} must be float32")
    if t.shape[1] > 1 and t.stride(1) != 1:
        raise ValueError(f"{name} must have unit inner stride")
    ld = t.stride(0) if t.shape[0] > 1 else max(t.shape[1], t.stride(0))
    return C.c_void_p(t.data_ptr()), int(ld), int(t.shape[0]), int(t.shape[1])


def _p(t: Optional[torch.Tensor], name="tensor", dtype=torch.float32):
    return N.ptr(t, dtype, name)


def dense_fwd(X, W, bias, Y, act: int = 0, accumulate: bool = False, trans_w: bool = False, relu_mask=None):
    xp, ldx, M, K = _mat(X, "X")
    wp, ldw, wr, wc = _mat(W, "W")
    yp, ldy, My, Ncol = _mat(Y, "Y")
    Kw, Nw = (wc, wr) if trans_w else (wr, wc)
    if Kw != K or Nw != Ncol or My != M:
        raise ValueError(f"dense_fwd: shape mismatch X{tuple(X.shape)} W{tuple(W.shape)} trans={trans_w} Y{tuple(Y.shape)}")
    if bias is not None:
        N.expect_shape(bias, (Ncol,), "bias")
    mp, ldm = C.c_void_p(0), 0
    if relu_mask is not None:
        mp, ldm, Mm, Nm = _mat(relu_mask, "relu_mask")
        if (Mm, Nm) != (M, Ncol):
            raise ValueError(f"dense_fwd: relu_mask {tuple(relu_mask.shape)} does not match Y {tuple(Y.shape)}")
    FLOPS[0] += 2.0 * M * K * Ncol
    rc = N.lib().dgppo_dense_fwd(xp, ldx, wp, ldw, _p(bias, "bias"), yp, ldy, M, K, Ncol, int(act), int(accumulate),
                                 int(trans_w), mp, ldm, N.stream_ptr())
    N.check(rc, "dgppo_dense_fwd")


def mlp_gi_fwd(X, W1, b1, g1, be1, W2, b2, g2, be2, Wi, bi, gi, saves=None):
    xp, ldx, M, K = _mat(X, "X")
    if K != 64:
        raise ValueError(f"mlp_gi_fwd: X must be [M, 64], got {tuple(X.shape)}")
    for t, shp, nm in ((W1, (64, 64), "W1"), (W2, (64, 64), "W2"), (Wi, (64, 192), "Wi"), (b1, (64,), "b1"), (g1, (64,), "g1"),
                       (be1, (64,), "be1"), (b2, (64,), "b2"), (g2, (64,), "g2"), (be2, (64,), "be2"), (bi, (192,), "bi"),
                       (gi, (M, 192), "gi")):
        N.expect_shape(t, shp, nm)
    sv = [None] * 6
    if saves is not None:
        for t, shp, nm in zip(saves, ((M, 64), (M, 64), (M, 2), (M, 64), (M, 64), (M, 2)), ("p1", "y1", "st1", "p2", "y2", "st2")):
            N.expect_shape(t, shp, nm)
        sv = list(saves)
    FLOPS[0] += 2.0 * M * (64 * 64 * 2 + 64 * 192)
    rc = N.lib().dgppo_mlp_gi_fwd(xp, ldx, _p(W1), _p(b1), _p(g1), _p(be1), _p(W2), _p(b2), _p(g2), _p(be2), _p(Wi), _p(bi),
                                  *[_p(t) for t in sv], _p(gi), M, N.stream_ptr())
    N.check(rc, "dgppo_mlp_gi_fwd")


def mlp_gi_bwd(dgi, Wi, W2, W1, g2, g1, p2, y2, st2, p1, y1, st1, relu_mask, dpre2, dpre1, dx, dg2, db2, dg1, db1):
    M = dgi.shape[0]
    N.expect_shape(dgi, (M, 192), "dgi")
    for t, shp, nm in ((Wi, (64, 192), "Wi"), (W2, (64, 64), "W2"), (W1, (64, 64), "W1"), (g2, (64,), "g2"), (g1, (64,), "g1"),
                       (p2, (M, 64), "p2"), (y2, (M, 64), "y2"), (st2, (M, 2), "st2"), (p1, (M, 64), "p1"), (y1, (M, 64), "y1"),
                       (st1, (M, 2), "st1"), (dpre2, (M, 64), "dpre2"), (dpre1, (M, 64), "dpre1"), (dx, (M, 64), "dx"),
                       (dg2, (64,), "dg2"), (db2, (64,), "db2"), (dg1, (64,), "dg1"), (db1, (64,), "db1")):
        N.expect_shape(t, shp, nm)
    mp, ldm = (None, 0)
    if relu_mask is not None:
        mp, ldm, Mm, Km = _mat(relu_mask, "relu_mask")
        if (Mm, Km) != (M, 64):
            raise ValueError(f"mlp_gi_bwd: relu_mask must be [M, 64], got {tuple(relu_mask.shape)}")
    FLOPS[0] += 2.0 * M * (64 * 64 * 2 + 64 * 192)
    rc = N.lib().dgppo_mlp_gi_bwd(_p(dgi), _p(Wi), _p(W2), _p(W1), _p(g2), _p(g1), _p(p2), _p(y2), _p(st2), _p(p1), _p(y1), _p(st1),
                                  mp if mp is not None else C.c_void_p(0), ldm, _p(dpre2), _p(dpre1), _p(dx), 64,
                                  _p(dg2), _p(db2), _p(dg1), _p(db1), M, N.stream_ptr())
    N.check(rc, "dgppo_mlp_gi_bwd")


def gru1_head_fwd(gi, Wh, bhn, h0, W1, b1, W2, b2, hs, hprev, gates, u, out):
    M = gi.shape[0]
    n_out = out.shape[1]
    N.expect_shape(gi, (M, 192), "gi"); N.expect_shape(Wh, (64, 192), "Wh"); N.expect_shape(bhn, (64,), "bhn")
    N.expect_shape(hs, (M, 64), "hs"); N.expect_shape(out, (M, n_out), "out")
    if h0 is not None:
        N.expect_shape(h0, (M, 64), "h0")
    if W2 is not None:
        N.expect_shape(W1, (64, 64), "W1"); N.expect_shape(b1, (64,), "b1")
        N.expect_shape(W2, (64, n_out), "W2"); N.expect_shape(b2, (n_out,), "b2")
    else:
        N.expect_shape(W1, (64, n_out), "W1"); N.expect_shape(b1, (n_out,), "b1")
    for t, shp, nm in ((hprev, (M, 64), "hprev"), (gates, (M, 256), "gates"), (u, (M, 64), "u")):
        if t is not None:
            N.expect_shape(t, shp, nm)
    FLOPS[0] += 2.0 * M * (64 * 192 + (64 * 64 + 64 * n_out if W2 is not None else 64 * n_out))
    rc = N.lib().dgppo_gru1_head_fwd(_p(gi), _p(Wh), _p(bhn), _p(h0), _p(W1), _p(b1), _p(W2), _p(b2), _p(hs), _p(hprev),
                                     _p(gates), _p(u), _p(out), M, n_out, N.stream_ptr())
    N.check(rc, "dgppo_gru1_head_fwd")


_WS: dict = {}


def _bwd_w_workspace(device, K: int, Ncol: int) -> torch.Tensor:
    lib = N.lib()
    lib.dgppo_dense_bwd_w_workspace_bytes.restype = C.c_int64
    need = int(lib.dgppo_dense_bwd_w_workspace_bytes(C.c_int32(K), C.c_int32(Ncol)))
    need = min(need, 64 << 20)
    key = (device.index, torch.cuda.current_stream(device).cuda_stream)
    ws = _WS.get(key)
    if ws is None or ws.numel() * 4 < need:
        ws = torch.empty(need // 4, dtype=torch.float32, device=device)
        _WS[key] = ws
    return ws


class ReduceDesc(C.Structure):
    _fields_ = [("part", C.c_void_p), ("dW", C.c_void_p), ("db", C.c_void_p), ("part_stride", C.c_int32), ("slabs", C.c_int32),
                ("ldw", C.c_int32), ("K", C.c_int32), ("N", C.c_int32), ("pending", C.c_int32)]


class BwdWBatch:
    _active = {}

    def __init__(self, device, alloc):
        self.device, self.alloc = device, alloc
        self.key = None
        self.descs = []
        self.offset = 0
        self.ws = None

    def __enter__(self):
        self.key = (self.device.index, torch.cuda.current_stream(self.device).cuda_stream)
        if self.key in BwdWBatch._active:
            raise RuntimeError("BwdWBatch: nested batches on one stream")
        BwdWBatch._active[self.key] = self
        return self

    def region(self, nbytes: int):
        nbytes = (nbytes + 255) & ~255
        if self.ws is None or self.ws.numel() * 4 < self.offset + nbytes:
            if self.descs:
                self.flush()
            self.ws = self.alloc(max(self.offset + nbytes, 2 * (self.ws.numel() * 4 if self.ws is not None else 0)) // 4)
        view = self.ws[self.offset // 4:(self.offset + nbytes) // 4]
        self.offset += nbytes
        return view

    def flush(self):
        if self.descs:
            arr = (ReduceDesc * len(self.descs))(*self.descs)
            N.check(N.lib().dgppo_dense_bwd_w_reduce_batch(arr, C.c_int32(len(self.descs)), N.stream_ptr()),
                    "dgppo_dense_bwd_w_reduce_batch")
        self.descs = []
        self.offset = 0

    def __exit__(self, *exc):
        try:
            if exc[0] is None:
                self.flush()
        finally:
            BwdWBatch._active.pop(self.key, None)
        return False


def dense_bwd_w(X, dY, dW, db=None):
    xp, ldx, M, K = _mat(X, "X")
    yp, ldy, My, Ncol = _mat(dY, "dY")
    wp, ldw, Kw, Nw = _mat(dW, "dW")
    if My != M or Kw != K or Nw != Ncol:
        raise ValueError(f"dense_bwd_w: shape mismatch X{tuple(X.shape)} dY{tuple(dY.shape)} dW{tuple(dW.shape)}")
    if db is not None:
        N.expect_shape(db, (Ncol,), "db")
    FLOPS[0] += 2.0 * M * K * Ncol
    batch = BwdWBatch._active.get((X.device.index, torch.cuda.current_stream(X.device).cuda_stream)) if X.is_cuda else None
    if batch is not None:
        lib = N.lib()
        lib.dgppo_dense_bwd_w_workspace_bytes.restype = C.c_int64
        need = min(int(lib.dgppo_dense_bwd_w_workspace_bytes(C.c_int32(K), C.c_int32(Ncol))), 64 << 20)
        ws = batch.region(need)
        d = ReduceDesc()
        rc = lib.dgppo_dense_bwd_w_deferred(xp, ldx, yp, ldy, wp, ldw, _p(db, "db"), M, K, Ncol, _p(ws, "workspace"),
                                            C.c_int64(ws.numel() * 4), C.byref(d), N.stream_ptr())
        N.check(rc, "dgppo_dense_bwd_w_deferred")
        if d.pending:
            batch.descs.append(d)
        return
    ws = _bwd_w_workspace(X.device, K, Ncol)
    rc = N.lib().dgppo_dense_bwd_w(xp, ldx, yp, ldy, wp, ldw, _p(db, "db"), M, K, Ncol, _p(ws, "workspace"),
                                   C.c_int64(ws.numel() * 4), N.stream_ptr())
    N.check(rc, "dgppo_dense_bwd_w")


def _check_strided(fn: str, name: str, t_, se: int, st: int, inner: tuple, env_ids, n_env: int, n_time: int):
    if not (t_.is_cuda and t_.dtype == torch.float32):
        raise ValueError(f"{fn}: {name} must be a float32 CUDA tensor")
    want, acc = [], 1
    for d in reversed(inner):
        want.append(acc)
        acc *= d
    if tuple(t_.shape[-len(inner):]) != tuple(inner) or list(t_.stride()[-len(inner):]) != want[::-1]:
        raise ValueError(f"{fn}: the trailing {inner} block of {name} must be dense (got shape {tuple(t_.shape)}, "
                         f"strides {t_.stride()})")
    avail = t_.untyped_storage().nbytes() // 4 - t_.storage_offset()
    if env_ids is None and (n_env - 1) * se + (n_time - 1) * st + acc > avail:
        raise ValueError(f"{fn}: {name}: the strides reach beyond its storage")


def graph_feats(cfg: N.EnvCfg, agent, agent_se, agent_st, goal, obst, hits, hits_se, hits_st, env_ids, n_env, n_time,
                Xa, Xo, efeat, emask, Fp):
    G = n_env * n_time
    n, S = cfg.n_agents, cfg.fan_in
    n_other = cfg.num_nodes - 1 - n
    N.expect_shape(Xa, (G * n, Fp), "Xa")
    if n_other > 0:
        N.expect_shape(Xo, (G * n_other, Fp), "Xo")
    N.expect_shape(efeat, (G * n, S, 4), "efeat")
    N.expect_shape(emask, (G * n, S), "emask")
    _check_strided("graph_feats", "agent", agent, agent_se, agent_st, (n, cfg.state_dim), env_ids, n_env, n_time)
    if hits is not None:
        _check_strided("graph_feats", "hits", hits, hits_se, hits_st, (n, cfg.top_k, 2), env_ids, n_env, n_time)
    rc = N.lib().dgppo_graph_feats(
        C.byref(cfg), C.c_void_p(agent.data_ptr()), C.c_int64(agent_se), C.c_int64(agent_st), _p(goal, "goal"),
        _p(obst, "obst") if (obst is not None and not cfg.is_lidar) else C.c_void_p(0),
        C.c_void_p(hits.data_ptr()) if hits is not None else C.c_void_p(0), C.c_int64(hits_se), C.c_int64(hits_st),
        _p(env_ids, "env_ids", torch.int32), C.c_int32(n_env), C.c_int32(n_time), _p(Xa, "Xa"), _p(Xo, "Xo"),
        _p(efeat, "efeat"), _p(emask, "emask"), C.c_int32(Fp), N.stream_ptr())
    N.check(rc, "dgppo_graph_feats")


def sweep_axis(x, name: str, device) -> torch.Tensor:
    if torch.is_tensor(x):
        t_ = x.to(device=device, dtype=torch.float32).contiguous()
        ok = t_.ndim == 1 and t_.numel() > 0 and bool(torch.isfinite(t_).all())
    else:
        a = np.ascontiguousarray(np.asarray(x, dtype=np.float32))
        ok = a.ndim == 1 and a.size > 0 and bool(np.isfinite(a).all())
        t_ = torch.from_numpy(a).to(device) if ok else None
    if not ok:
        raise ValueError(f"graph_feats_sweep: {name} must be a non-empty 1-D array of finite coordinates")
    return t_


def _sweep_grid(fn: str, cfg: N.EnvCfg, frame_ids, n_frames, agent_id, xs, ys, frame_max):
    n = cfg.n_agents
    if not 0 <= int(agent_id) < n:
        raise ValueError(f"{fn}: agent_id {agent_id} outside [0, {n})")
    for name, t_ in (("xs", xs), ("ys", ys)):
        if not (torch.is_tensor(t_) and t_.is_cuda and t_.dtype == torch.float32 and t_.ndim == 1 and t_.is_contiguous()):
            raise ValueError(f"{fn}: {name} must be a dense 1-D float32 CUDA tensor (sweep_axis)")
        if t_.numel() == 0:
            raise ValueError(f"{fn}: {name} is empty")
    ids = ids_dev = None
    if torch.is_tensor(frame_ids):
        if frame_max is None or n_frames < 1 or tuple(frame_ids.shape) != (n_frames,):
            raise ValueError(f"{fn}: a device frame_ids needs its shape (n_frames,) and frame_max")
        ids_dev, last = frame_ids, int(frame_max)
    elif frame_ids is not None:
        ids = np.asarray(frame_ids, dtype=np.int64).reshape(-1)
        if ids.size != n_frames or n_frames == 0 or ids.min() < 0:
            raise ValueError(f"{fn}: frame_ids must hold n_frames >= 1 frame numbers >= 0")
        last = int(ids.max())
    else:
        if n_frames < 1:
            raise ValueError(f"{fn}: n_frames must be >= 1")
        last = n_frames - 1
    return int(xs.numel()), int(ys.numel()), ids, ids_dev, last


def _sweep_record(fn: str, cfg: N.EnvCfg, agent, agent_st, obst, hits, hits_st, ray_cos, ray_sin, last, hits_out, G) -> bool:
    n = cfg.n_agents
    _check_strided(fn, "agent", agent, 0, agent_st, (n, cfg.state_dim), None, 1, last + 1)
    cast = cfg.is_lidar and cfg.n_obs > 0
    if cfg.n_obs > 0:
        if obst is None:
            raise ValueError(f"{fn}: obst is required when n_obs > 0")
        N.expect_shape(obst, (cfg.n_obs, cfg.obst_stride), "obst")
    if cast:
        if hits is None:
            raise ValueError(f"{fn}: hits is required for a LiDAR kind with obstacles")
        _check_strided(fn, "hits", hits, 0, hits_st, (n, cfg.top_k, 2), None, 1, last + 1)
        N.expect_shape(ray_cos, (cfg.n_rays,), "ray_cos")
        N.expect_shape(ray_sin, (cfg.n_rays,), "ray_sin")
        if hits_out is not None:
            N.expect_shape(hits_out, (G, cfg.top_k, 2), "hits_out")
    return cast


def graph_feats_sweep(cfg: N.EnvCfg, agent, agent_st, goal, obst, hits, hits_st, ray_cos, ray_sin, frame_ids, n_frames,
                      agent_id, xs, ys, Xa, Xo, efeat, emask, Fp, hits_out=None, frame_max=None):
    fn = "graph_feats_sweep"
    n, S = cfg.n_agents, cfg.fan_in
    nx, ny, ids, ids_dev, last = _sweep_grid(fn, cfg, frame_ids, n_frames, agent_id, xs, ys, frame_max)
    G = n_frames * ny * nx
    n_other = cfg.num_nodes - 1 - n
    N.expect_shape(Xa, (G * n, Fp), "Xa")
    if n_other > 0:
        N.expect_shape(Xo, (G * n_other, Fp), "Xo")
    N.expect_shape(efeat, (G * n, S, 4), "efeat")
    N.expect_shape(emask, (G * n, S), "emask")
    N.expect_shape(goal, (cfg.n_goals, cfg.state_dim), "goal")
    cast = _sweep_record(fn, cfg, agent, agent_st, obst, hits, hits_st, ray_cos, ray_sin, last, hits_out, G)
    if ids is not None:
        ids_dev = torch.from_numpy(ids.astype(np.int32)).to(agent.device)
    null = C.c_void_p(0)
    rc = N.lib().dgppo_graph_feats_sweep(
        C.byref(cfg), C.c_void_p(agent.data_ptr()), C.c_int64(agent_st), _p(goal, "goal"),
        _p(obst, "obst") if cfg.n_obs > 0 else null, C.c_void_p(hits.data_ptr()) if cast else null, C.c_int64(hits_st),
        _p(ray_cos, "ray_cos") if cast else null, _p(ray_sin, "ray_sin") if cast else null,
        _p(ids_dev, "frame_ids", torch.int32), C.c_int32(n_frames), C.c_int32(int(agent_id)), _p(xs, "xs"), C.c_int32(nx),
        _p(ys, "ys"), C.c_int32(ny), _p(Xa, "Xa"), _p(Xo, "Xo") if n_other > 0 else null, _p(efeat, "efeat"), _p(emask, "emask"),
        _p(hits_out, "hits_out") if (cast and hits_out is not None) else null, C.c_int32(Fp), N.stream_ptr())
    N.check(rc, "dgppo_graph_feats_sweep")


def cost_sweep(cfg: N.EnvCfg, agent, agent_st, obst, hits, hits_st, ray_cos, ray_sin, frame_ids, n_frames, agent_id, xs, ys,
               cost, hits_out=None, frame_max=None):
    fn = "cost_sweep"
    if cfg.is_vmas:
        raise ValueError(f"{fn}: VMASReverseTransport has no sweep entry point")
    if hits_out is not None and not (cfg.is_lidar and cfg.n_obs > 0):
        raise ValueError(f"{fn}: hits_out needs a LiDAR kind with obstacles (nothing is cast here)")
    nx, ny, ids, ids_dev, last = _sweep_grid(fn, cfg, frame_ids, n_frames, agent_id, xs, ys, frame_max)
    G = n_frames * ny * nx
    N.expect_shape(cost, (G, cfg.n_agents, cfg.n_cost), "cost")
    cast = _sweep_record(fn, cfg, agent, agent_st, obst, hits, hits_st, ray_cos, ray_sin, last, hits_out, G)
    if ids is not None:
        ids_dev = torch.from_numpy(ids.astype(np.int32)).to(agent.device)
    null = C.c_void_p(0)
    rc = N.lib().dgppo_cost_sweep(
        C.byref(cfg), C.c_void_p(agent.data_ptr()), C.c_int64(agent_st), _p(obst, "obst") if cfg.n_obs > 0 else null,
        C.c_void_p(hits.data_ptr()) if cast else null, C.c_int64(hits_st), _p(ray_cos, "ray_cos") if cast else null,
        _p(ray_sin, "ray_sin") if cast else null, _p(ids_dev, "frame_ids", torch.int32), C.c_int32(n_frames),
        C.c_int32(int(agent_id)), _p(xs, "xs"), C.c_int32(nx), _p(ys, "ys"), C.c_int32(ny), _p(cost, "cost"),
        _p(hits_out, "hits_out") if cast and hits_out is not None else null, N.stream_ptr())
    N.check(rc, "dgppo_cost_sweep")


def vmas_graph_feats(cfg: N.EnvCfg, agent, agent_se, agent_st, body, body_se, body_st, scene, env_ids, n_env, n_time,
                     Xa, efeat, emask, Fp):
    G = n_env * n_time
    n = cfg.n_agents
    N.expect_shape(Xa, (G * n, Fp), "Xa")
    N.expect_shape(efeat, (G * n, n, 4), "efeat")
    N.expect_shape(emask, (G * n, n), "emask")
    _check_strided("vmas_graph_feats", "agent", agent, agent_se, agent_st, (n, 4), env_ids, n_env, n_time)
    _check_strided("vmas_graph_feats", "body", body, body_se, body_st, (4,), env_ids, n_env, n_time)
    rc = N.lib().dgppo_vmas_graph_feats(
        C.byref(cfg), C.c_void_p(agent.data_ptr()), C.c_int64(agent_se), C.c_int64(agent_st), C.c_void_p(body.data_ptr()),
        C.c_int64(body_se), C.c_int64(body_st), _p(scene, "scene"), _p(env_ids, "env_ids", torch.int32), C.c_int32(n_env),
        C.c_int32(n_time), _p(Xa, "Xa"), _p(efeat, "efeat"), _p(emask, "emask"), C.c_int32(Fp), N.stream_ptr())
    N.check(rc, "dgppo_vmas_graph_feats")


def attn_fwd(cfg, F, H, Kp, qt, Xa, Xo, efeat, emask, zcat, attn, G):
    n, S = cfg.n_agents, cfg.fan_in
    N.expect_shape(qt, (G * n, H * F), "qt")
    N.expect_shape(Xa, (G * n, F), "Xa")
    N.expect_shape(zcat, (G * n, Kp), "zcat")
    if attn is not None:
        N.expect_shape(attn, (G * n, S, H), "attn")
    FLOPS[0] += 2.0 * G * n * H * S * (2 * F + 4)
    rc = N.lib().dgppo_attn_fwd(C.byref(cfg), F, H, Kp, _p(qt), _p(Xa), _p(Xo), _p(efeat), _p(emask), _p(zcat), _p(attn),
                                G, N.stream_ptr())
    N.check(rc, "dgppo_attn_fwd")


def attn_bwd(cfg, F, H, Kp, dzcat, attn, qt, Xa, Xo, efeat, dqt, dXa, dXo, G, relu_xo: bool = False):
    n = cfg.n_agents
    N.expect_shape(dzcat, (G * n, Kp), "dzcat")
    N.expect_shape(dqt, (G * n, H * F), "dqt")
    if dXa is not None:
        N.expect_shape(dXa, (G * n, F), "dXa")
    FLOPS[0] += 4.0 * G * n * H * cfg.fan_in * (2 * F + 4)
    rc = N.lib().dgppo_attn_bwd(C.byref(cfg), F, H, Kp, _p(dzcat), _p(attn), _p(qt), _p(Xa), _p(Xo), _p(efeat), _p(dqt),
                                _p(dXa), _p(dXo), int(relu_xo), G, N.stream_ptr())
    N.check(rc, "dgppo_attn_bwd")


def attn_xo_supported(cfg, F, H, Kp) -> bool:
    return bool(N.lib().dgppo_attn_xo_supported(C.byref(cfg), F, H, Kp))


def _wo_ptr(Wo):
    if not Wo.is_cuda or Wo.dtype != torch.float32:
        raise TypeError("Wo must be a float32 GPU tensor")
    return C.c_void_p(Wo.data_ptr())


def _wo_ld(Wo):
    if Wo.dim() != 2 or Wo.shape[0] != 8 or Wo.shape[1] < 32 or Wo.stride(1) != 1:
        raise ValueError(f"Wo must be [8, >= 32] with contiguous rows, got {tuple(Wo.shape)} strides {Wo.stride()}")
    return int(Wo.stride(0))


def attn_fwd_xo(cfg, F, H, Kp, qt, Xa, Xo_raw, Wo, bo, efeat, emask, zcat, attn, G):
    n, S = cfg.n_agents, cfg.fan_in
    N.expect_shape(qt, (G * n, H * F), "qt")
    N.expect_shape(Xa, (G * n, F), "Xa")
    N.expect_shape(zcat, (G * n, Kp), "zcat")
    N.expect_shape(Xo_raw, (G * (cfg.num_nodes - 1 - n), 8), "Xo_raw")
    N.expect_shape(bo, (32,), "bo")
    if attn is not None:
        N.expect_shape(attn, (G * n, S, H), "attn")
    FLOPS[0] += 2.0 * G * n * H * S * (2 * F + 4) + 2.0 * G * (cfg.num_nodes - 1 - n) * 8 * 32
    rc = N.lib().dgppo_attn_fwd_xo(C.byref(cfg), F, H, Kp, _p(qt), _p(Xa), _p(Xo_raw), _wo_ptr(Wo),
                                   _wo_ld(Wo), _p(bo), _p(efeat), _p(emask), _p(zcat), _p(attn), G, N.stream_ptr())
    N.check(rc, "dgppo_attn_fwd_xo")


def attn_bwd_xo(cfg, F, H, Kp, dzcat, attn, qt, Xa, Xo_raw, Wo, bo, efeat, dqt, dXa, dXo, G, relu_xo: bool = False):
    n = cfg.n_agents
    N.expect_shape(dzcat, (G * n, Kp), "dzcat")
    N.expect_shape(dqt, (G * n, H * F), "dqt")
    N.expect_shape(Xo_raw, (G * (cfg.num_nodes - 1 - n), 8), "Xo_raw")
    if dXa is not None:
        N.expect_shape(dXa, (G * n, F), "dXa")
    FLOPS[0] += 4.0 * G * n * H * cfg.fan_in * (2 * F + 4) + 2.0 * G * (cfg.num_nodes - 1 - n) * 8 * 32
    rc = N.lib().dgppo_attn_bwd_xo(C.byref(cfg), F, H, Kp, _p(dzcat), _p(attn), _p(qt), _p(Xa), _p(Xo_raw),
                                   _wo_ptr(Wo), _wo_ld(Wo), _p(bo), _p(efeat), _p(dqt), _p(dXa), _p(dXo),
                                   int(relu_xo), G, N.stream_ptr())
    N.check(rc, "dgppo_attn_bwd_xo")


def attn_xo_workspace_floats(G: int) -> int:
    return int(N.lib().dgppo_attn_xo_workspace_bytes(int(G))) // 4


def attn_bwd_xo_dw(cfg, F, H, Kp, dzcat, attn, qt, Xa, Xo_raw, Wo, bo, efeat, dqt, dXa, dWo, dbo, workspace, G):
    n = cfg.n_agents
    N.expect_shape(dzcat, (G * n, Kp), "dzcat")
    N.expect_shape(dqt, (G * n, H * F), "dqt")
    N.expect_shape(dXa, (G * n, F), "dXa")
    N.expect_shape(Xo_raw, (G * (cfg.num_nodes - 1 - n), 8), "Xo_raw")
    N.expect_shape(dbo, (32,), "dbo")
    FLOPS[0] += 4.0 * G * n * H * cfg.fan_in * (2 * F + 4) + 4.0 * G * (cfg.num_nodes - 1 - n) * 8 * 32
    rc = N.lib().dgppo_attn_bwd_xo_dw(C.byref(cfg), F, H, Kp, _p(dzcat), _p(attn), _p(qt), _p(Xa), _p(Xo_raw), _wo_ptr(Wo), _wo_ld(Wo),
                                      _p(bo), _p(efeat), _p(dqt), _p(dXa), _wo_ptr(dWo), _wo_ld(dWo), _p(dbo), _p(workspace),
                                      C.c_int64(workspace.numel() * 4), G, N.stream_ptr())
    N.check(rc, "dgppo_attn_bwd_xo_dw")


def gnn_prep(Wq, bq, Wk, Wv, bv, We, Wu, Mcat, cvec, Wout, F, Fp, D, H, Kp):
    rc = N.lib().dgppo_gnn_prep(_p(Wq), _p(bq), _p(Wk), _p(Wv), _p(bv), _p(We), _p(Wu), _p(Mcat), _p(cvec), _p(Wout),
                                F, Fp, D, H, Kp, N.stream_ptr())
    N.check(rc, "dgppo_gnn_prep")


def gnn_unprep(dMcat, dcvec, dWout, Wq, bq, Wk, dWq, dbq, dWk, dWv, dbv, dWe, dWu, F, Fp, D, H, Kp):
    rc = N.lib().dgppo_gnn_unprep(_p(dMcat), _p(dcvec), _p(dWout), _p(Wq), _p(bq), _p(Wk), _p(dWq), _p(dbq), _p(dWk),
                                  _p(dWv), _p(dbv), _p(dWe), _p(dWu), F, Fp, D, H, Kp, N.stream_ptr())
    N.check(rc, "dgppo_gnn_unprep")


def ln_relu_fwd(x, gamma, beta, y, stats):
    M = x.shape[0]
    N.expect_shape(x, (M, 64), "x")
    N.expect_shape(y, (M, 64), "y")
    rc = N.lib().dgppo_ln_relu_fwd(_p(x), _p(gamma), _p(beta), _p(y), _p(stats), M, N.stream_ptr())
    N.check(rc, "dgppo_ln_relu_fwd")


def ln_relu_bwd(x, y, stats, gamma, dy, dx, dgamma, dbeta):
    M = x.shape[0]
    rc = N.lib().dgppo_ln_relu_bwd(_p(x), _p(y), _p(stats), _p(gamma), _p(dy), _p(dx), _p(dgamma), _p(dbeta), M,
                                   N.stream_ptr())
    N.check(rc, "dgppo_ln_relu_bwd")


def gru_fwd(gi, Wh, bhn, h0, hs, hprev, gates, n_seq, T, n_inner):
    rows = n_seq * T
    N.expect_shape(gi, (rows, 192), "gi")
    N.expect_shape(hs, (rows, 64), "hs")
    N.expect_shape(Wh, (64, 192), "Wh")
    if h0 is not None:
        N.expect_shape(h0, (n_seq, 64), "h0")
    FLOPS[0] += 2.0 * rows * 64 * 192
    rc = N.lib().dgppo_gru_fwd(_p(gi), _p(Wh), _p(bhn), _p(h0), _p(hs), _p(hprev), _p(gates), n_seq, T, n_inner,
                               N.stream_ptr())
    N.check(rc, "dgppo_gru_fwd")


def gru_bwd(dhs, Wh, hprev, gates, dgi, dgh, n_seq, T, n_inner):
    rows = n_seq * T
    N.expect_shape(dhs, (rows, 64), "dhs")
    N.expect_shape(dgi, (rows, 192), "dgi")
    N.expect_shape(dgh, (rows, 192), "dgh")
    FLOPS[0] += 2.0 * rows * 64 * 192
    rc = N.lib().dgppo_gru_bwd(_p(dhs), _p(Wh), _p(hprev), _p(gates), _p(dgi), _p(dgh), n_seq, T, n_inner, N.stream_ptr())
    N.check(rc, "dgppo_gru_bwd")


def gru_bwd_dhn(dhs, Wh, hprev, gates, dgi, dhn, n_seq, T, n_inner):
    rows = n_seq * T
    N.expect_shape(dhs, (rows, 64), "dhs")
    N.expect_shape(dgi, (rows, 192), "dgi")
    N.expect_shape(dhn, (rows, 64), "dhn")
    FLOPS[0] += 2.0 * rows * 64 * 192
    rc = N.lib().dgppo_gru_bwd_dhn(_p(dhs), _p(Wh), _p(hprev), _p(gates), _p(dgi), _p(dhn), n_seq, T, n_inner, N.stream_ptr())
    N.check(rc, "dgppo_gru_bwd_dhn")


def gru_bwd_w(x, hprev, dgi, dhn, dWi, dbi, dWh, dbhn):
    xp, ldx, M, Kx = _mat(x, "x")
    hp, ldh, Mh, Kh = _mat(hprev, "hprev")
    wip, ldwi, _, _ = _mat(dWi, "dWi")
    whp, ldwh, _, _ = _mat(dWh, "dWh")
    if Kx != 64 or (Mh, Kh) != (M, 64) or tuple(dWi.shape) != (64, 192) or tuple(dWh.shape) != (64, 192):
        raise ValueError(f"gru_bwd_w: shape mismatch x{tuple(x.shape)} hprev{tuple(hprev.shape)} dWi{tuple(dWi.shape)} "
                         f"dWh{tuple(dWh.shape)}")
    N.expect_shape(dgi, (M, 192), "dgi"); N.expect_shape(dhn, (M, 64), "dhn")
    N.expect_shape(dbi, (192,), "dbi"); N.expect_shape(dbhn, (64,), "dbhn")
    FLOPS[0] += 2.0 * M * 64 * (128 + 64 + 192)
    lib = N.lib()
    lib.dgppo_gru_bwd_w_workspace_bytes.restype = C.c_int64
    need = int(lib.dgppo_gru_bwd_w_workspace_bytes())
    batch = BwdWBatch._active.get((x.device.index, torch.cuda.current_stream(x.device).cuda_stream)) if x.is_cuda else None
    if batch is not None:
        ws = batch.region(need)
        d = (ReduceDesc * 3)()
        pend = d
    else:
        key = (x.device.index, torch.cuda.current_stream(x.device).cuda_stream, "gru")
        ws = _WS.get(key)
        if ws is None or ws.numel() * 4 < need:
            ws = _WS[key] = torch.empty(need // 4, dtype=torch.float32, device=x.device)
        pend = None
    rc = lib.dgppo_gru_bwd_w(xp, ldx, hp, ldh, _p(dgi, "dgi"), _p(dhn, "dhn"), wip, ldwi, _p(dbi, "dbi"), whp, ldwh,
                             _p(dbhn, "dbhn"), M, _p(ws, "workspace"), C.c_int64(ws.numel() * 4), pend, N.stream_ptr())
    N.check(rc, "dgppo_gru_bwd_w")
    if batch is not None:
        for i in range(3):
            if d[i].pending:
                batch.descs.append(ReduceDesc.from_buffer_copy(d[i]))


def policy_head(ms, eps, action_in, action, log_pi, entropy, n_agents, mode, log_pi_old=None, adv=None, dms=None,
                stats=None, clip_eps=0.25, coef_ent=0.01):
    rows = ms.shape[0]
    N.expect_shape(ms, (rows, 4), "ms")
    rc = N.lib().dgppo_policy_head(_p(ms), _p(eps), _p(action_in), _p(action), _p(log_pi), _p(entropy), rows, n_agents,
                                   mode, _p(log_pi_old), _p(adv), _p(dms), _p(stats), C.c_float(clip_eps),
                                   C.c_float(coef_ent), N.stream_ptr())
    N.check(rc, "dgppo_policy_head")


def value_loss(v, target, dv, stats):
    rc = N.lib().dgppo_value_loss(_p(v), _p(target), _p(dv), _p(stats), v.numel(), N.stream_ptr())
    N.check(rc, "dgppo_value_loss")


def mean_agents(x, y, G, n, D, backward=False, relu_mask=None):
    rc = N.lib().dgppo_mean_agents(_p(x), _p(y), G, n, D, int(backward), _p(relu_mask), N.stream_ptr())
    N.check(rc, "dgppo_mean_agents")


def relu_bwd(dy, y):
    rc = N.lib().dgppo_relu_bwd(_p(dy), _p(y), C.c_int64(dy.numel()), N.stream_ptr())
    N.check(rc, "dgppo_relu_bwd")


def lstm_fwd(zi, Wh, bh, c0, h0, cs, hs, cprev, hprev, gates, n_seq, T, n_inner):
    rows = n_seq * T
    N.expect_shape(zi, (rows, 256), "zi"); N.expect_shape(Wh, (64, 256), "Wh"); N.expect_shape(bh, (256,), "bh")
    N.expect_shape(cs, (rows, 64), "cs"); N.expect_shape(hs, (rows, 64), "hs")
    for t, nm in ((c0, "c0"), (h0, "h0")):
        if t is not None:
            N.expect_shape(t, (n_seq, 64), nm)
    FLOPS[0] += 2.0 * rows * 64 * 256
    rc = N.lib().dgppo_lstm_fwd(_p(zi), _p(Wh), _p(bh), _p(c0), _p(h0), _p(cs), _p(hs), _p(cprev), _p(hprev), _p(gates),
                                n_seq, T, n_inner, N.stream_ptr())
    N.check(rc, "dgppo_lstm_fwd")


def lstm_bwd(dhs, Wh, cprev, gates, dz, n_seq, T, n_inner):
    rows = n_seq * T
    N.expect_shape(dhs, (rows, 64), "dhs"); N.expect_shape(dz, (rows, 256), "dz")
    FLOPS[0] += 2.0 * rows * 64 * 256
    rc = N.lib().dgppo_lstm_bwd(_p(dhs), _p(Wh), _p(cprev), _p(gates), _p(dz), n_seq, T, n_inner, N.stream_ptr())
    N.check(rc, "dgppo_lstm_bwd")
```

include/dgppo_hip.h:

```cpp
#ifndef DGPPO_HIP_H
#define DGPPO_HIP_H

#include <stdint.h>

#ifdef __cplusplus
extern "C" {
#endif

#define DGPPO_ABI_VERSION 3

enum {
  DGPPO_ENV_LIDAR_SPREAD = 0,
  DGPPO_ENV_LIDAR_TARGET = 1,
  DGPPO_ENV_LIDAR_BICYCLE_TARGET = 2,
  DGPPO_ENV_MPE_SPREAD = 3,
  DGPPO_ENV_MPE_TARGET = 4,
  DGPPO_ENV_LIDAR_LINE = 5,
  DGPPO_ENV_MPE_LINE = 6,
  DGPPO_ENV_MPE_FORMATION = 7,
  DGPPO_ENV_MPE_CORRIDOR = 8,
  DGPPO_ENV_MPE_CONNECT_SPREAD = 9,
  DGPPO_ENV_VMAS_REVERSE_TRANSPORT = 10
};
enum {
  DGPPO_GOALS_NODES = 0,
  DGPPO_GOALS_LINE = 1,
  DGPPO_GOALS_LINE_INTERIOR = 2,
  DGPPO_GOALS_CIRCLE = 3
};

#define DGPPO_RECT_STRIDE 16

typedef struct dgppo_env_cfg {
  int32_t kind;
  int32_t n_agents;
  int32_t n_goals;
  int32_t n_obs;
  int32_t n_rays;
  int32_t top_k;
  int32_t state_dim;
  int32_t node_dim;
  float area_size;
  float dt;
  float car_radius;
  float comm_radius;
  float obs_radius;
  float dist2goal;
  float two_car_radius;
  float lidar_mask_radius;
  float eye_offset;
  float car_plus_obs;
  float vel_limit;
  float reset_min_dist;
  int32_t reward_goals;
  int32_t n_cost;
  float obs_mask_radius;
  float y_limit;
  float connect_radius;
  float reset_side_y;
  float goal_shift_y;
  float line_min_dist;
} dgppo_env_cfg;

typedef struct dgppo_graph_out {
  float*   nodes;
  float*   edges;
  float*   states;
  int32_t* receivers;
  int32_t* senders;
  int32_t* node_type;
  int32_t* n_node;
  int32_t* n_edge;
} dgppo_graph_out;

int32_t     dgppo_abi_version(void);
const char* dgppo_last_error(void);

int32_t dgppo_env_num_nodes(const dgppo_env_cfg* cfg);
int32_t dgppo_env_num_edges(const dgppo_env_cfg* cfg);


int32_t dgppo_env_step(const dgppo_env_cfg* cfg,
                       const float* agent, const float* action, const float* goal,
                       const float* obst, const float* hits,
                       const float* ray_cos, const float* ray_sin,
                       float* next_agent, float* next_hits, float* reward, float* cost,
                       const dgppo_graph_out* gout, int32_t B, void* stream);

int32_t dgppo_graph_materialize(const dgppo_env_cfg* cfg,
                                const float* agent, const float* goal,
                                const float* obst, const float* hits,
                                const dgppo_graph_out* gout, int32_t B, void* stream);

int32_t dgppo_env_reset(const dgppo_env_cfg* cfg, const uint64_t* seeds,
                        float* agent, float* goal, float* obst, int32_t B, void* stream);
int32_t dgppo_env_reset_checked(const dgppo_env_cfg* cfg, const uint64_t* seeds, float* agent, float* goal, float* obst,
                                int32_t* n_failed, int32_t B, void* stream);


int32_t dgppo_vmas_reset_checked(const dgppo_env_cfg* cfg, const uint64_t* seeds, float* agent, float* body, float* scene,
                                 int32_t* n_failed, int32_t B, void* stream);
int32_t dgppo_vmas_step(const dgppo_env_cfg* cfg, const float* agent, const float* body, const float* scene,
                        const float* action, float* next_agent, float* next_body, float* reward, float* cost,
                        const dgppo_graph_out* gout, int32_t B, void* stream);
int32_t dgppo_vmas_graph_materialize(const dgppo_env_cfg* cfg, const float* agent, const float* body, const float* scene,
                                     const dgppo_graph_out* gout, int32_t B, void* stream);
int32_t dgppo_vmas_graph_feats(const dgppo_env_cfg* cfg, const float* agent, int64_t agent_se, int64_t agent_st,
                               const float* body, int64_t body_se, int64_t body_st, const float* scene,
                               const int32_t* env_ids, int32_t n_env, int32_t n_time, float* Xa, float* efeat, float* emask,
                               int32_t Fp, void* stream);

int32_t dgppo_randn(uint64_t seed, uint64_t offset, float* out, int64_t n_elem, void* stream);
int32_t dgppo_randn_rows(uint64_t seed, float* out, int64_t rows, int64_t row_len, int64_t global_row_len,
                         int64_t col_offset, void* stream);


int32_t dgppo_dense_fwd(const float* X, int32_t ldx, const float* W, int32_t ldw, const float* bias, float* Y,
                        int32_t ldy, int32_t M, int32_t K, int32_t N, int32_t act, int32_t accumulate,
                        int32_t trans_w, const float* relu_mask, int32_t ldm, void* stream);
int32_t dgppo_dense_bwd_w(const float* X, int32_t ldx, const float* dY, int32_t ldy, float* dW, int32_t ldw,
                          float* db, int32_t M, int32_t K, int32_t N, float* workspace, int64_t workspace_bytes,
                          void* stream);
int32_t dgppo_mlp_gi_fwd(const float* X, int32_t ldx, const float* W1, const float* b1, const float* g1, const float* be1,
                         const float* W2, const float* b2, const float* g2, const float* be2, const float* Wi,
                         const float* bi, float* p1, float* y1, float* st1, float* p2, float* y2, float* st2, float* gi,
                         int32_t M, void* stream);
int32_t dgppo_mlp_gi_bwd(const float* dgi, const float* Wi, const float* W2, const float* W1, const float* g2,
                         const float* g1, const float* p2, const float* y2, const float* st2, const float* p1,
                         const float* y1, const float* st1, const float* relu_mask, int32_t ldm, float* dpre2, float* dpre1,
                         float* dx, int32_t lddx, float* dg2, float* db2, float* dg1, float* db1, int32_t M, void* stream);
#define DGPPO_REDUCE_BATCH 16
typedef struct dgppo_reduce_desc {
  const float* part;
  float* dW;
  float* db;
  int32_t part_stride, slabs, ldw, K, N;
  int32_t pending;
} dgppo_reduce_desc;
int32_t dgppo_dense_bwd_w_deferred(const float* X, int32_t ldx, const float* dY, int32_t ldy, float* dW, int32_t ldw,
                                   float* db, int32_t M, int32_t K, int32_t N, float* workspace, int64_t workspace_bytes,
                                   dgppo_reduce_desc* pending, void* stream);
int32_t dgppo_dense_bwd_w_reduce_batch(const dgppo_reduce_desc* descs, int32_t n, void* stream);
int32_t dgppo_gru1_head_fwd(const float* gi, const float* Wh, const float* bhn, const float* h0, const float* W1,
                            const float* b1, const float* W2, const float* b2, float* hs, float* hprev, float* gates,
                            float* u, float* out, int32_t M, int32_t n_out, void* stream);
int64_t dgppo_dense_bwd_w_workspace_bytes(int32_t K, int32_t N);

int32_t dgppo_graph_feats(const dgppo_env_cfg* cfg, const float* agent, int64_t agent_se, int64_t agent_st,
                          const float* goal, const float* obst, const float* hits, int64_t hits_se, int64_t hits_st,
                          const int32_t* env_ids, int32_t n_env, int32_t n_time, float* Xa, float* Xo, float* efeat,
                          float* emask, int32_t Fp, void* stream);

int32_t dgppo_graph_feats_sweep(const dgppo_env_cfg* cfg, const float* agent, int64_t agent_st, const float* goal,
                                const float* obst, const float* hits, int64_t hits_st, const float* ray_cos,
                                const float* ray_sin, const int32_t* frame_ids, int32_t n_frames, int32_t agent_id,
                                const float* xs, int32_t nx, const float* ys, int32_t ny, float* Xa, float* Xo,
                                float* efeat, float* emask, float* hits_out, int32_t Fp, void* stream);

int32_t dgppo_cost_sweep(const dgppo_env_cfg* cfg, const float* agent, int64_t agent_st, const float* obst, const float* hits,
                         int64_t hits_st, const float* ray_cos, const float* ray_sin, const int32_t* frame_ids,
                         int32_t n_frames, int32_t agent_id, const float* xs, int32_t nx, const float* ys, int32_t ny,
                         float* cost, float* hits_out, void* stream);

int32_t dgppo_attn_fwd(const dgppo_env_cfg* cfg, int32_t F, int32_t H, int32_t Kp, const float* qt, const float* Xa,
                       const float* Xo, const float* efeat, const float* emask, float* zcat, float* attn, int32_t G,
                       void* stream);
int32_t dgppo_attn_bwd(const dgppo_env_cfg* cfg, int32_t F, int32_t H, int32_t Kp, const float* dzcat,
                       const float* attn, const float* qt, const float* Xa, const float* Xo, const float* efeat,
                       float* dqt, float* dXa, float* dXo, int32_t relu_xo, int32_t G, void* stream);
int32_t dgppo_attn_xo_supported(const dgppo_env_cfg* cfg, int32_t F, int32_t H, int32_t Kp);
int32_t dgppo_attn_fwd_xo(const dgppo_env_cfg* cfg, int32_t F, int32_t H, int32_t Kp, const float* qt, const float* Xa,
                          const float* Xo_raw, const float* Wo, int32_t ldwo, const float* bo, const float* efeat,
                          const float* emask, float* zcat, float* attn, int32_t G, void* stream);
int32_t dgppo_attn_bwd_xo(const dgppo_env_cfg* cfg, int32_t F, int32_t H, int32_t Kp, const float* dzcat,
                          const float* attn, const float* qt, const float* Xa, const float* Xo_raw, const float* Wo,
                          int32_t ldwo, const float* bo, const float* efeat, float* dqt, float* dXa, float* dXo,
                          int32_t relu_xo, int32_t G, void* stream);
int64_t dgppo_attn_xo_workspace_bytes(int32_t G);
int32_t dgppo_attn_bwd_xo_dw(const dgppo_env_cfg* cfg, int32_t F, int32_t H, int32_t Kp, const float* dzcat,
                             const float* attn, const float* qt, const float* Xa, const float* Xo_raw, const float* Wo,
                             int32_t ldwo, const float* bo, const float* efeat, float* dqt, float* dXa, float* dWo,
                             int32_t lddwo, float* dbo, float* workspace, int64_t workspace_bytes, int32_t G, void* stream);

int32_t dgppo_gnn_prep(const float* Wq, const float* bq, const float* Wk, const float* Wv, const float* bv,
                       const float* We, const float* Wu, float* Mcat, float* cvec, float* Wout, int32_t F, int32_t Fp,
                       int32_t D, int32_t H, int32_t Kp, void* stream);
int32_t dgppo_gnn_unprep(const float* dMcat, const float* dcvec, const float* dWout, const float* Wq, const float* bq,
                         const float* Wk, float* dWq, float* dbq, float* dWk, float* dWv, float* dbv, float* dWe,
                         float* dWu, int32_t F, int32_t Fp, int32_t D, int32_t H, int32_t Kp, void* stream);

int32_t dgppo_ln_relu_fwd(const float* x, const float* gamma, const float* beta, float* y, float* stats, int32_t M,
                          void* stream);
int32_t dgppo_ln_relu_bwd(const float* x, const float* y, const float* stats, const float* gamma, const float* dy,
                          float* dx, float* dgamma, float* dbeta, int32_t M, void* stream);

int32_t dgppo_gru_fwd(const float* gi, const float* Wh, const float* bhn, const float* h0, float* hs, float* hprev,
                      float* gates, int32_t n_seq, int32_t T, int32_t n_inner, void* stream);
int32_t dgppo_gru_bwd(const float* dhs, const float* Wh, const float* hprev, const float* gates, float* dgi,
                      float* dgh, int32_t n_seq, int32_t T, int32_t n_inner, void* stream);
int32_t dgppo_gru_bwd_dhn(const float* dhs, const float* Wh, const float* hprev, const float* gates, float* dgi,
                          float* dhn, int32_t n_seq, int32_t T, int32_t n_inner, void* stream);
int64_t dgppo_gru_bwd_w_workspace_bytes(void);
int32_t dgppo_gru_bwd_w(const float* x, int32_t ldx, const float* hprev, int32_t ldh, const float* dgi, const float* dhn,
                        float* dWi, int32_t ldwi, float* dbi, float* dWh, int32_t ldwh, float* dbhn, int32_t M,
                        float* workspace, int64_t workspace_bytes, dgppo_reduce_desc* pending, void* stream);

int32_t dgppo_lstm_fwd(const float* zi, const float* Wh, const float* bh, const float* c0, const float* h0, float* cs,
                       float* hs, float* cprev, float* hprev, float* gates, int32_t n_seq, int32_t T, int32_t n_inner,
                       void* stream);
int32_t dgppo_lstm_bwd(const float* dhs, const float* Wh, const float* cprev, const float* gates, float* dz,
                       int32_t n_seq, int32_t T, int32_t n_inner, void* stream);

int32_t dgppo_policy_head(const float* ms, const float* eps, const float* action_in, float* action, float* log_pi,
                          float* entropy, int32_t rows, int32_t n_agents, int32_t mode, const float* log_pi_old,
                          const float* adv, float* dms, float* stats, float clip_eps, float coef_ent, void* stream);

int32_t dgppo_value_loss(const float* v, const float* target, float* dv, float* stats, int32_t count, void* stream);
int32_t dgppo_mean_agents(const float* x, float* y, int32_t G, int32_t n, int32_t D, int32_t backward,
                          const float* relu_mask, void* stream);
int32_t dgppo_relu_bwd(float* dy, const float* y, int64_t count, void* stream);


int32_t dgppo_gae(const float* costs, const float* rewards, const float* Vh, const float* Vl, const float* lam_pow,
                  float gamma, float one_minus_gamma, float one_minus_lam, float* Qh, float* Ql, int32_t B, int32_t T,
                  int32_t n, int32_t nh, void* stream);
int32_t dgppo_advantage(const float* Ql, const float* Vl, const float* Vh, float dt, float alpha, float cbf_eps,
                        float cbf_weight, float* adv, float* stats, int32_t B, int32_t T, int32_t n, int32_t nh,
                        void* stream);
int32_t dgppo_advantage_lagr(const float* Ql, const float* Vl, const float* Qh, const float* Vh, const float* lagr,
                             float* adv, float* Ah, int32_t B, int32_t T, int32_t n, int32_t nh, void* stream);
int32_t dgppo_lagr_update(const float* lp_new, const float* lp_old, const float* Vh, int64_t vh_env_stride,
                          const float* Ah, float* lagr, float* sums, int32_t n_env, int32_t T, int32_t n, int32_t nh,
                          float one_minus_gamma, float lr, void* stream);
int32_t dgppo_lagr_sums(const float* lp_new, const float* lp_old, const float* Vh, int64_t vh_env_stride, const float* Ah,
                        float* sums, int32_t n_env, int32_t T, int32_t n, int32_t nh, float one_minus_gamma, void* stream);
int32_t dgppo_lagr_apply(float* lagr, float* sums, int32_t count, int64_t rows_total, float lr, void* stream);
int32_t dgppo_relu_fwd(const float* x, float* out, int64_t count, void* stream);
int32_t dgppo_shaped_reward(const float* reward, const float* cost, float cost_weight, float* out, int64_t rows,
                            int32_t n, int32_t nh, void* stream);
#define DGPPO_OPT_PARTIALS 256
#define DGPPO_OPT_STATE_FLOATS (8 + 2 * DGPPO_OPT_PARTIALS)
int32_t dgppo_clip_adam_step(float* params, const float* grads, float* m, float* v, int64_t n, float* state, float lr,
                             float b1, float b2, float eps, float max_norm, float grad_scale, void* stream);

#define DGPPO_COMM_ID_BYTES 128
int32_t dgppo_comm_unique_id(uint8_t* id_out);
int32_t dgppo_comm_version(int32_t* version_out);
int32_t dgppo_comm_init(const uint8_t* id, int32_t rank, int32_t world, void** comm_out);
int32_t dgppo_comm_allreduce_sum_f32(void* comm, float* buf, int64_t count, void* stream);
int32_t dgppo_comm_destroy(void* comm);

#ifdef __cplusplus
}
#endif
#endif
```

Measured before the change: 4.087 million.

## Batch minibatch gathers, block-strided GRU h0, and wave-per-graph feature kernel

Adds a multi-tensor row-gather kernel that replaces several index_select calls per minibatch with one launch. Lets the GRU forward read h0 directly from block-strided storage instead of a materialized copy. Rewrites graph_feats to map one wavefront per graph in a persistent grid-stride loop, with register prefetch of the next graph's inputs, vectorized node and mask stores, and lidar hits stored compactly. This trades a larger, more complex kernel and an occupancy-sized grid for fewer launches and less copy traffic.

```diff
diff --git a/dgppo_amd/csrc/gather.hip b/dgppo_amd/csrc/gather.hip
--- /dev/null
+++ b/dgppo_amd/csrc/gather.hip
@@ -0,0 +1,55 @@
+#include "common.h"
+
+struct GatherArgs {
+  const char* src[DGPPO_GATHER_MAX];
+  char* dst[DGPPO_GATHER_MAX];
+  long row_bytes[DGPPO_GATHER_MAX], src_stride[DGPPO_GATHER_MAX];
+  int vec[DGPPO_GATHER_MAX];
+  const int32_t* ids;
+  int n_ids;
+};
+
+__global__ void __launch_bounds__(256) gather_rows_kernel(GatherArgs a) {
+  const int k = blockIdx.z;
+  const long units = a.vec[k] ? a.row_bytes[k] >> 4 : a.row_bytes[k] >> 2;
+  const long u0 = (long)blockIdx.x * blockDim.x + threadIdx.x, du = (long)gridDim.x * blockDim.x;
+  if (u0 >= units) return;
+  for (int e = blockIdx.y; e < a.n_ids; e += gridDim.y) {
+    const char* s = a.src[k] + (size_t)a.ids[e] * a.src_stride[k];
+    char* d = a.dst[k] + (size_t)e * a.row_bytes[k];
+    if (a.vec[k]) {
+      for (long u = u0; u < units; u += du) reinterpret_cast<uint4*>(d)[u] = reinterpret_cast<const uint4*>(s)[u];
+    } else {
+      for (long u = u0; u < units; u += du) reinterpret_cast<uint32_t*>(d)[u] = reinterpret_cast<const uint32_t*>(s)[u];
+    }
+  }
+}
+
+extern "C" int32_t dgppo_gather_rows(const dgppo_gather_desc* descs, int32_t n_desc, const int32_t* ids, int32_t n_ids,
+                                     void* stream) {
+  DGPPO_REQUIRE(n_desc >= 0 && n_desc <= DGPPO_GATHER_MAX, "gather_rows: n_desc must be in [0,%d] (got %d)", DGPPO_GATHER_MAX, n_desc);
+  DGPPO_REQUIRE(n_ids >= 0, "gather_rows: negative n_ids");
+  if (n_desc == 0 || n_ids == 0) return 0;
+  DGPPO_REQUIRE(descs && ids, "gather_rows: NULL operand");
+  DGPPO_REQUIRE(((uintptr_t)ids & 3) == 0, "gather_rows: ids must be 4-byte aligned");
+  GatherArgs a{};
+  long max_units = 0;
+  for (int k = 0; k < n_desc; ++k) {
+    const dgppo_gather_desc& d = descs[k];
+    DGPPO_REQUIRE(d.src && d.dst, "gather_rows: NULL pointer in descriptor %d", k);
+    DGPPO_REQUIRE(d.row_bytes > 0 && d.row_bytes % 4 == 0, "gather_rows: row_bytes of descriptor %d must be a positive multiple of 4 (got %lld)",
+                  k, (long long)d.row_bytes);
+    DGPPO_REQUIRE(d.src_stride >= 0 && d.src_stride % 4 == 0, "gather_rows: src_stride of descriptor %d must be a non-negative multiple of 4", k);
+    DGPPO_REQUIRE(((uintptr_t)d.src & 3) == 0 && ((uintptr_t)d.dst & 3) == 0, "gather_rows: descriptor %d is not 4-byte aligned", k);
+    a.src[k] = (const char*)d.src; a.dst[k] = (char*)d.dst; a.row_bytes[k] = d.row_bytes; a.src_stride[k] = d.src_stride;
+    a.vec[k] = (d.row_bytes % 16 == 0 && d.src_stride % 16 == 0 && ((uintptr_t)d.src & 15) == 0 && ((uintptr_t)d.dst & 15) == 0) ? 1 : 0;
+    const long units = a.vec[k] ? d.row_bytes >> 4 : d.row_bytes >> 2;
+    max_units = units > max_units ? units : max_units;
+  }
+  a.ids = ids; a.n_ids = n_ids;
+  const int gx = cdiv(max_units, 256) < 64 ? cdiv(max_units, 256) : 64;
+  const int gy = n_ids < 1024 ? n_ids : 1024;
+  hipLaunchKernelGGL(gather_rows_kernel, dim3(gx, gy, n_desc), dim3(256), 0, (hipStream_t)stream, a);
+  DGPPO_LAUNCH_CHECK();
+  return 0;
+}
diff --git a/dgppo_amd/csrc/graph_feats.hip b/dgppo_amd/csrc/graph_feats.hip
--- a/dgppo_amd/csrc/graph_feats.hip
+++ b/dgppo_amd/csrc/graph_feats.hip
@@ -14,98 +14,174 @@
   float* efeat;
   float* emask;
   int Fp;
-  uint32_t rcp_fp, rcp_S;
+  int vecX, vecM;
+  uint32_t rcp_fp, rcp_fq, rcp_S;
 };
 
+#define GF_PF 8
+#define GF_WAVE_SYNC()                                  \
+  do {                                                  \
+    __builtin_amdgcn_fence(__ATOMIC_SEQ_CST, "wavefront"); \
+    __builtin_amdgcn_wave_barrier();                    \
+  } while (0)
+
+struct FeatRec { const float *ag, *go, *ob; };
+
 template <int SD>
-__global__ void graph_feats_kernel(FeatArgs a) {
+__device__ inline float4 feat4(const float* s) {
+  if constexpr (SD == 5) {
+    float vx = __fmul_rn(s[4], s[2]), vy = __fmul_rn(s[4], s[3]);
+    asm volatile("" : "+v"(vx), "+v"(vy));
+    return make_float4(s[0], s[1], vx, vy);
+  } else {
+    return make_float4(s[0], s[1], s[2], s[3]);
+  }
+}
+
+template <int SD>
+__global__ void __launch_bounds__(256) graph_feats_kernel(FeatArgs a) {
   extern __shared__ float sm[];
   const dgppo_env_cfg& c = a.cfg;
   const Topo& t = a.t;
-  const int g = blockIdx.x;
-  const int e = g / a.n_time, tt = g - e * a.n_time;
-  const int env = a.env_ids ? a.env_ids[e] : e;
-  const int tid = threadIdx.x, nt = blockDim.x;
+  const int lane = threadIdx.x & 63;
+  const int wv = __builtin_amdgcn_readfirstlane(threadIdx.x >> 6), wpb = blockDim.x >> 6;
   const int n = t.n, ng = t.ng, S = t.S, Fp = a.Fp;
   const int n_on = t.Ns - n - ng;
-  float* s_ag = sm;
-  float* s_go = s_ag + n * SD;
-  float* s_ob = s_go + ng * SD;
-  float* s_fa = s_ob + n_on * SD;
-  float* s_fg = s_fa + n * 4;
-  const float* ag = a.agent + (size_t)env * a.agent_se + (size_t)tt * a.agent_st;
-  for (int i = tid; i < n * SD; i += nt) s_ag[i] = ag[i];
-  for (int i = tid; i < ng * SD; i += nt) s_go[i] = a.goal[(size_t)env * ng * SD + i];
-  if (n_on > 0) {
-    if (t.lidar) {
-      const float* hp = a.hits + (size_t)env * a.hits_se + (size_t)tt * a.hits_st;
-      for (int i = tid; i < n_on * 2; i += nt) {
-        const int q = i >> 1, d = i & 1;
-        s_ob[q * SD + d] = hp[i];
-      }
-      for (int i = tid; i < n_on * (SD - 2); i += nt) {
-        const int q = i / (SD - 2), d = i - q * (SD - 2);
-        s_ob[q * SD + 2 + d] = 0.0f;
+  const int nA = n * SD, nG = ng * SD, nO = n_on * (t.lidar ? 2 : SD), R = nA + nG + nO;
+  float* s_ag = sm + (size_t)wv * R;
+  float* s_go = s_ag + nA;
+  float* s_ob = s_go + nG;
+  const long G = (long)a.n_env * a.n_time, stride = (long)gridDim.x * wpb;
+  long g = (long)blockIdx.x * wpb + wv;
+  if (g >= G) return;
+  auto env_of = [&](long gg) { const int e = (int)gg / a.n_time; return a.env_ids ? (int)a.env_ids[e] : e; };
+  auto locate = [&](long gg, int env) {
+    const int tt = (int)gg % a.n_time;
+    FeatRec p;
+    p.ag = a.agent + (size_t)env * a.agent_se + (size_t)tt * a.agent_st;
+    p.go = a.goal + (size_t)env * nG;
+    p.ob = nullptr;
+    if (nO > 0) p.ob = t.lidar ? a.hits + (size_t)env * a.hits_se + (size_t)tt * a.hits_st : a.obst + (size_t)env * nO;
+    return p;
+  };
+  auto fetch = [&](const FeatRec& p, int i) { return i < nA ? p.ag[i] : (i < nA + nG ? p.go[i - nA] : p.ob[i - nA - nG]); };
+  float r0, r1, r2, r3, r4, r5, r6, r7;
+  static_assert(GF_PF == 8, "one register per prefetched dword");
+#define GF_EACH(OP) OP(r0, 0) OP(r1, 1) OP(r2, 2) OP(r3, 3) OP(r4, 4) OP(r5, 5) OP(r6, 6) OP(r7, 7)
+#define GF_REQUEST(r, j) { const int i = lane + 64 * j; r = 0.0f; if (i < R) r = fetch(p, i); }
+#define GF_COMMIT(r, j)  { const int i = lane + 64 * j; if (i < R) s_ag[i] = r; }
+  FeatRec p = locate(g, env_of(g));
+  GF_EACH(GF_REQUEST)
+  long gn = g + stride;
+  int env_n = gn < G ? env_of(gn) : 0;
+  for (;;) {
+    GF_EACH(GF_COMMIT)
+    for (int i = GF_PF * 64 + lane; i < R; i += 64) s_ag[i] = fetch(p, i);
+    GF_WAVE_SYNC();
+    const bool more = gn < G;
+    if (more) {
+      p = locate(gn, env_n);
+      GF_EACH(GF_REQUEST)
+      if (gn + stride < G) env_n = env_of(gn + stride);
+    }
+    auto node_src = [&](int nd, const float*& src, int& ns, int& one) {
+      if (nd < n) { src = s_ag + nd * SD; ns = SD; one = SD + 2; }
+      else if (nd < n + ng) { src = s_go + (nd - n) * SD; ns = SD; one = SD + 1; }
+      else if (t.lidar) { src = s_ob + (nd - n - ng) * 2; ns = 2; one = SD; }
+      else { src = s_ob + (nd - n - ng) * SD; ns = SD; one = SD; }
+    };
+    if (a.vecX) {
+      const int Fq = Fp >> 2;
+      for (int q = lane; q < t.Ns * Fq; q += 64) {
+        const int nd = (int)__umulhi((uint32_t)q, a.rcp_fq), col0 = (q - nd * Fq) * 4;
+        const float* src; int ns, one;
+        node_src(nd, src, ns, one);
+        float v[4];
+#pragma unroll
+        for (int k = 0; k < 4; ++k) {
+          const int col = col0 + k;
+          v[k] = (col < ns) ? src[col] : ((col == one) ? 1.0f : 0.0f);
+        }
+        float* dst = (nd < n) ? a.Xa + ((size_t)g * n + nd) * Fp + col0 : a.Xo + ((size_t)g * (t.Ns - n) + (nd - n)) * Fp + col0;
+        *reinterpret_cast<float4*>(dst) = make_float4(v[0], v[1], v[2], v[3]);
       }
     } else {
-      for (int i = tid; i < n_on * SD; i += nt) s_ob[i] = a.obst[(size_t)env * n_on * SD + i];
+      for (int idx = lane; idx < t.Ns * Fp; idx += 64) {
+        const int nd = (int)__umulhi((uint32_t)idx, a.rcp_fp), col = idx - nd * Fp;
+        const float* src; int ns, one;
+        node_src(nd, src, ns, one);
+        const float v = (col < ns) ? src[col] : ((col == one) ? 1.0f : 0.0f);
+        if (nd < n) a.Xa[((size_t)g * n + nd) * Fp + col] = v;
+        else a.Xo[((size_t)g * (t.Ns - n) + (nd - n)) * Fp + col] = v;
+      }
     }
+    const int nE = n * S;
+    for (int base = 0; base < nE; base += 64) {
+      const int idx = base + lane;
+      bool mask = false;
+      if (idx < nE) {
+        const int i = (int)__umulhi((uint32_t)idx, a.rcp_S), s = idx - i * S;
+        float4 f;
+        const float4 fi = feat4<SD>(s_ag + i * SD);
+        const float px = s_ag[i * SD], py = s_ag[i * SD + 1];
+        if (s < n) {
+          const float4 fj = feat4<SD>(s_ag + s * SD);
+          f = make_float4(__fsub_rn(fi.x, fj.x), __fsub_rn(fi.y, fj.y), __fsub_rn(fi.z, fj.z), __fsub_rn(fi.w, fj.w));
+          float d = __fadd_rn(dist_rn(__fsub_rn(px, s_ag[s * SD]), __fsub_rn(py, s_ag[s * SD + 1])), (i == s) ? c.eye_offset : 0.0f);
+          mask = d < c.comm_radius;
+        } else if (s < n + t.gs) {
+          const int gi = t.spread ? (s - n) : i;
+          const float4 fg = feat4<SD>(s_go + gi * SD);
+          f = make_float4(__fsub_rn(fi.x, fg.x), __fsub_rn(fi.y, fg.y), __fsub_rn(fi.z, fg.z), __fsub_rn(fi.w, fg.w));
+          mask = true;
+        } else {
+          const int m = s - n - t.gs;
+          if (t.lidar) {
+            const float* hp = s_ob + (i * t.per + m) * 2;
+            const float lx = __fsub_rn(px, hp[0]), ly = __fsub_rn(py, hp[1]);
+            f = make_float4(lx, ly, 0.0f, 0.0f);
+            mask = dist_rn(lx, ly) < c.lidar_mask_radius;
+          } else {
+            const float* xo = s_ob + m * SD;
+            const float* xi = s_ag + i * SD;
+            f = make_float4(__fsub_rn(xi[0], xo[0]), __fsub_rn(xi[1], xo[1]), __fsub_rn(xi[2], xo[2]), __fsub_rn(xi[3], xo[3]));
+            mask = dist_rn(__fsub_rn(xi[0], xo[0]), __fsub_rn(xi[1], xo[1])) < c.obs_mask_radius;
+          }
+        }
+        reinterpret_cast<float4*>(a.efeat)[(size_t)g * nE + idx] = f;
+        if (!a.vecM) a.emask[(size_t)g * nE + idx] = mask ? 1.0f : 0.0f;
+      }
+      if (a.vecM) {
+        const unsigned long long bits = __ballot(mask);
+        const int i4 = base + 4 * lane;
+        if (lane < 16 && i4 < nE) {
+          const unsigned b = (unsigned)(bits >> (4 * lane));
+          *reinterpret_cast<float4*>(a.emask + (size_t)g * nE + i4) =
+              make_float4((b & 1u) ? 1.0f : 0.0f, (b & 2u) ? 1.0f : 0.0f, (b & 4u) ? 1.0f : 0.0f, (b & 8u) ? 1.0f : 0.0f);
+        }
+      }
+    }
+    GF_WAVE_SYNC();
+    if (!more) break;
+    g = gn;
+    gn += stride;
   }
-  __syncthreads();
-  for (int i = tid; i < n + ng; i += nt) {
-    const float* s = (i < n) ? s_ag + i * SD : s_go + (i - n) * SD;
-    float* f = (i < n) ? s_fa + i * 4 : s_fg + (i - n) * 4;
-    if constexpr (SD == 5) {
-      f[0] = s[0]; f[1] = s[1]; f[2] = __fmul_rn(s[4], s[2]); f[3] = __fmul_rn(s[4], s[3]);
-    } else {
-      f[0] = s[0]; f[1] = s[1]; f[2] = s[2]; f[3] = s[3];
-    }
-  }
-  __syncthreads();
-  constexpr int ND = SD + 3;
-  for (int idx = tid; idx < t.Ns * Fp; idx += nt) {
-    const int nd = (int)__umulhi((uint32_t)idx, a.rcp_fp), col = idx - nd * Fp;
-    float v = 0.0f;
-    if (nd < n) v = (col < SD) ? s_ag[nd * SD + col] : ((col == SD + 2) ? 1.0f : 0.0f);
-    else if (nd < n + ng) v = (col < SD) ? s_go[(nd - n) * SD + col] : ((col == SD + 1) ? 1.0f : 0.0f);
-    else v = (col < SD) ? s_ob[(nd - n - ng) * SD + col] : ((col == SD) ? 1.0f : 0.0f);
-    if (col >= ND) v = 0.0f;
-    if (nd < n) a.Xa[((size_t)g * n + nd) * Fp + col] = v;
-    else a.Xo[((size_t)g * (t.Ns - n) + (nd - n)) * Fp + col] = v;
-  }
-  for (int idx = tid; idx < n * S; idx += nt) {
-    const int i = (int)__umulhi((uint32_t)idx, a.rcp_S), s = idx - i * S;
-    float4 f;
-    bool mask;
-    const float* fi = s_fa + i * 4;
-    const float px = s_ag[i * SD], py = s_ag[i * SD + 1];
-    if (s < n) {
-      const float* fj = s_fa + s * 4;
-      f = make_float4(__fsub_rn(fi[0], fj[0]), __fsub_rn(fi[1], fj[1]), __fsub_rn(fi[2], fj[2]), __fsub_rn(fi[3], fj[3]));
-      float d = __fadd_rn(dist_rn(__fsub_rn(px, s_ag[s * SD]), __fsub_rn(py, s_ag[s * SD + 1])), (i == s) ? c.eye_offset : 0.0f);
-      mask = d < c.comm_radius;
-    } else if (s < n + t.gs) {
-      const int gi = t.spread ? (s - n) : i;
-      const float* fg = s_fg + gi * 4;
-      f = make_float4(__fsub_rn(fi[0], fg[0]), __fsub_rn(fi[1], fg[1]), __fsub_rn(fi[2], fg[2]), __fsub_rn(fi[3], fg[3]));
-      mask = true;
-    } else {
-      const int m = s - n - t.gs;
-      if (t.lidar) {
-        const float* hp = s_ob + (i * t.per + m) * SD;
-        const float lx = __fsub_rn(px, hp[0]), ly = __fsub_rn(py, hp[1]);
-        f = make_float4(lx, ly, 0.0f, 0.0f);
-        mask = dist_rn(lx, ly) < c.lidar_mask_radius;
-      } else {
-        const float* xo = s_ob + m * SD;
-        const float* xi = s_ag + i * SD;
-        f = make_float4(__fsub_rn(xi[0], xo[0]), __fsub_rn(xi[1], xo[1]), __fsub_rn(xi[2], xo[2]), __fsub_rn(xi[3], xo[3]));
-        mask = dist_rn(__fsub_rn(xi[0], xo[0]), __fsub_rn(xi[1], xo[1])) < c.obs_mask_radius;
-      }
-    }
-    reinterpret_cast<float4*>(a.efeat)[(size_t)g * n * S + idx] = f;
-    a.emask[(size_t)g * n * S + idx] = mask ? 1.0f : 0.0f;
-  }
+#undef GF_EACH
+#undef GF_REQUEST
+#undef GF_COMMIT
+}
+
+static int feats_grid_cap(const void* fn, int wpb, size_t smem) {
+  static thread_local const void* k_fn = nullptr;
+  static thread_local int k_wpb = 0, k_cap = 0;
+  static thread_local size_t k_smem = 0;
+  if (fn == k_fn && wpb == k_wpb && smem == k_smem) return k_cap;
+  int per_cu = 0, dev = 0, cus = 256;
+  if (hipOccupancyMaxActiveBlocksPerMultiprocessor(&per_cu, fn, 64 * wpb, smem) != hipSuccess || per_cu < 1) per_cu = 1;
+  if (hipGetDevice(&dev) != hipSuccess ||
+      hipDeviceGetAttribute(&cus, hipDeviceAttributeMultiprocessorCount, dev) != hipSuccess || cus < 1) cus = 256;
+  k_fn = fn; k_wpb = wpb; k_smem = smem; k_cap = per_cu * cus;
+  return k_cap;
 }
 
 extern "C" int32_t dgppo_graph_feats(const dgppo_env_cfg* cfg, const float* agent, int64_t agent_se, int64_t agent_st,
@@ -135,11 +211,20 @@
   a.rcp_fp = (uint32_t)((0x100000000ull + (uint64_t)Fp - 1) / (uint64_t)Fp);
   a.rcp_S = (uint32_t)((0x100000000ull + (uint64_t)a.t.S - 1) / (uint64_t)a.t.S);
   DGPPO_REQUIRE(Fp >= 2 && a.t.S >= 2 && (long)a.t.Ns * Fp < 65536 && (long)a.t.n * a.t.S < 65536, "graph_feats: sizes out of range");
+  a.vecX = (Fp % 4 == 0 && ((uintptr_t)Xa & 15) == 0 && ((uintptr_t)Xo & 15) == 0) ? 1 : 0;
+  a.vecM = ((a.t.n * a.t.S) % 4 == 0 && ((uintptr_t)emask & 15) == 0) ? 1 : 0;
+  a.rcp_fq = a.vecX ? (uint32_t)((0x100000000ull + (uint64_t)(Fp / 4) - 1) / (uint64_t)(Fp / 4)) : 0u;
   const int SD = cfg->state_dim;
-  const size_t smem = sizeof(float) * ((size_t)a.t.n * SD + a.t.ng * SD + (size_t)n_on * SD + a.t.n * 4 + a.t.ng * 4);
+  const size_t rec = sizeof(float) * ((size_t)a.t.n * SD + (size_t)a.t.ng * SD + (size_t)n_on * (a.t.lidar ? 2 : SD));
+  int wpb = 4;
+  while (wpb > 1 && rec * wpb > 65536) wpb >>= 1;
   const long G = (long)n_env * n_time;
-  if (SD == 5) hipLaunchKernelGGL(graph_feats_kernel<5>, dim3(G), dim3(128), smem, (hipStream_t)stream, a);
-  else hipLaunchKernelGGL(graph_feats_kernel<4>, dim3(G), dim3(128), smem, (hipStream_t)stream, a);
+  const void* fn = SD == 5 ? reinterpret_cast<const void*>(&graph_feats_kernel<5>) : reinterpret_cast<const void*>(&graph_feats_kernel<4>);
+  const int cap = feats_grid_cap(fn, wpb, rec * wpb);
+  const long wgs = (G + wpb - 1) / wpb;
+  const dim3 grid((unsigned)(wgs < cap ? wgs : cap)), block(64 * wpb);
+  if (SD == 5) hipLaunchKernelGGL(graph_feats_kernel<5>, grid, block, rec * wpb, (hipStream_t)stream, a);
+  else hipLaunchKernelGGL(graph_feats_kernel<4>, grid, block, rec * wpb, (hipStream_t)stream, a);
   DGPPO_LAUNCH_CHECK();
   return 0;
 }
diff --git a/dgppo_amd/csrc/nn_elem.hip b/dgppo_amd/csrc/nn_elem.hip
--- a/dgppo_amd/csrc/nn_elem.hip
+++ b/dgppo_amd/csrc/nn_elem.hip
@@ -149,6 +149,8 @@
   float* dgh;
   float* dhn;
   int n_seq, T, n_inner;
+  int h0_rpb;
+  long h0_bstride;
 };
 
 __device__ inline size_t gru_row(const GruArgs& a, int s, int tau) {
@@ -187,7 +189,11 @@
       int s = tile * RB + r;
       s = s < a.n_seq ? s : a.n_seq - 1;
       float4 v = z4;
-      if (a.h0 != nullptr) v = reinterpret_cast<const float4*>(a.h0 + (size_t)s * GRU_H)[q];
+      if (a.h0 != nullptr) {
+        const float* hp = a.h0 + (size_t)s * GRU_H;
+        if (a.h0_rpb > 0) { const int b = s / a.h0_rpb; hp = a.h0 + (size_t)b * a.h0_bstride + (size_t)(s - b * a.h0_rpb) * GRU_H; }
+        v = reinterpret_cast<const float4*>(hp)[q];
+      }
       hpf[u][0] = v.x; hpf[u][1] = v.y; hpf[u][2] = v.z; hpf[u][3] = v.w;
     }
   };
@@ -408,30 +414,49 @@
   return 0;
 }
 
+static int32_t gru_fwd_launch(GruArgs a, hipStream_t stream) {
+  int32_t rc = gru_check(a);
+  if (rc) return rc;
+  const int n_seq = a.n_seq;
+  if (n_seq == 0) return 0;
+  DGPPO_REQUIRE(a.gi && a.Wh && a.bhn && a.hs, "gru_fwd: NULL operand");
+  if (cdiv(n_seq, 32) >= 512) {
+    const size_t smem = sizeof(float) * 2 * 32 * GRU_HL;
+    static thread_local int cap = 0;
+    if (cap == 0) cap = gru_resident(reinterpret_cast<const void*>(&gru_fwd_kernel<2>), smem);
+    const int tiles = cdiv(n_seq, 32);
+    hipLaunchKernelGGL(gru_fwd_kernel<2>, dim3(tiles < cap ? tiles : cap), dim3(256), smem, stream, a);
+  } else {
+    const size_t smem = sizeof(float) * 2 * 16 * GRU_HL;
+    static thread_local int cap = 0;
+    if (cap == 0) cap = gru_resident(reinterpret_cast<const void*>(&gru_fwd_kernel<1>), smem);
+    const int tiles = cdiv(n_seq, 16);
+    hipLaunchKernelGGL(gru_fwd_kernel<1>, dim3(tiles < cap ? tiles : cap), dim3(256), smem, stream, a);
+  }
+  DGPPO_LAUNCH_CHECK();
+  return 0;
+}
+
 extern "C" int32_t dgppo_gru_fwd(const float* gi, const float* Wh, const float* bhn, const float* h0, float* hs,
                                  float* hprev, float* gates, int32_t n_seq, int32_t T, int32_t n_inner, void* stream) {
   GruArgs a{};
   a.gi = gi; a.Wh = Wh; a.bhn = bhn; a.h0 = h0; a.hs = hs; a.hprev = hprev; a.gates = gates;
   a.n_seq = n_seq; a.T = T; a.n_inner = n_inner;
-  int32_t rc = gru_check(a);
-  if (rc) return rc;
-  if (n_seq == 0) return 0;
-  DGPPO_REQUIRE(gi && Wh && bhn && hs, "gru_fwd: NULL operand");
-  if (cdiv(n_seq, 32) >= 512) {
-    const size_t smem = sizeof(float) * 2 * 32 * GRU_HL;
-    static thread_local int cap = 0;
-    if (cap == 0) cap = gru_resident(reinterpret_cast<const void*>(&gru_fwd_kernel<2>), smem);
-    const int tiles = cdiv(n_seq, 32);
-    hipLaunchKernelGGL(gru_fwd_kernel<2>, dim3(tiles < cap ? tiles : cap), dim3(256), smem, (hipStream_t)stream, a);
-  } else {
-    const size_t smem = sizeof(float) * 2 * 16 * GRU_HL;
-    static thread_local int cap = 0;
-    if (cap == 0) cap = gru_resident(reinterpret_cast<const void*>(&gru_fwd_kernel<1>), smem);
-    const int tiles = cdiv(n_seq, 16);
-    hipLaunchKernelGGL(gru_fwd_kernel<1>, dim3(tiles < cap ? tiles : cap), dim3(256), smem, (hipStream_t)stream, a);
-  }
-  DGPPO_LAUNCH_CHECK();
-  return 0;
+  return gru_fwd_launch(a, (hipStream_t)stream);
+}
+
+extern "C" int32_t dgppo_gru_fwd_h0_blocks(const float* gi, const float* Wh, const float* bhn, const float* h0,
+                                           int32_t rows_per_block, int64_t block_stride, float* hs, float* hprev,
+                                           float* gates, int32_t n_seq, int32_t T, int32_t n_inner, void* stream) {
+  GruArgs a{};
+  a.gi = gi; a.Wh = Wh; a.bhn = bhn; a.h0 = h0; a.hs = hs; a.hprev = hprev; a.gates = gates;
+  a.n_seq = n_seq; a.T = T; a.n_inner = n_inner;
+  DGPPO_REQUIRE(h0 != nullptr && ((uintptr_t)h0 & 15) == 0, "gru_fwd_h0_blocks: h0 must be a 16-byte aligned pointer");
+  DGPPO_REQUIRE(rows_per_block >= 1, "gru_fwd_h0_blocks: rows_per_block must be >= 1 (got %d)", rows_per_block);
+  DGPPO_REQUIRE(block_stride >= (int64_t)rows_per_block * GRU_H && block_stride % 4 == 0,
+                "gru_fwd_h0_blocks: block_stride must be a multiple of 4 and >= rows_per_block * 64");
+  a.h0_rpb = rows_per_block; a.h0_bstride = (long)block_stride;
+  return gru_fwd_launch(a, (hipStream_t)stream);
 }
 
 template <bool DHN_ONLY>
diff --git a/dgppo_amd/engine.py b/dgppo_amd/engine.py
--- a/dgppo_amd/engine.py
+++ b/dgppo_amd/engine.py
@@ -86,8 +86,14 @@
             setattr(self, k, self.step[k])
         self.actions = tr("actions", self.action_tm)
         self.log_pis = tr("log_pis", self.log_pi_tm) if self.stochastic else None
-        self._rnn_em = tr("_rnn_em", self.rnn_tm)
-        self.rnn_states = self._rnn_em[:, :self.T] if self.stochastic else self._rnn_em[:, 1:]
+        T, x = self.T, self.rnn_tm
+        want = (x.shape[1], T + 2) + tuple(x.shape[2:])
+        cur = getattr(self, "_rnn_em", None)
+        if cur is None or tuple(cur.shape) != want:
+            cur = torch.empty(want, device=x.device, dtype=x.dtype)
+        cur[:, :T + 1].copy_(x.transpose(0, 1))
+        self._rnn_em = cur
+        self.rnn_states = self._rnn_em[:, :T] if self.stochastic else self._rnn_em[:, 1:T + 1]
         self.rewards = tr("rewards", self.reward_tm)
         self.costs = tr("costs", self.cost_tm)
         self._env_major = True
@@ -329,13 +335,20 @@
             HC = self.HC
             h_last = self.arena.get("pre.hlast", Eb * n, HC)
             h_last.view(Eb, n, HC).copy_(ro.rnn_states[e0:e0 + Eb, T - 1])
-            h0_all = self.arena.get("pre.h0all", Eb, T + 1, n, H)
             hstar = self.arena.get("pre.hstar", Eb * n, HC)
             self.policy.forward(fin, n_seq=Eb * n, T=1, h0=h_last, tag="fin", hs_out=hstar, train=False)
-            h0_all[:, :T].copy_(self._vh_carry(ro, e0, Eb))
-            h0_all[:, T].copy_(hstar.view(Eb, n, HC)[..., :H])
-            act = self.Vh.forward(feats, n_seq=Eb * (T + 1) * n, T=1, h0=h0_all.view(-1, H) if self.hp.use_rnn else None,
-                                  tag="pre", train=False)
+            if not self.hp.use_rnn:
+                h0 = None
+            elif HC == H:
+                s0 = 0 if ro.stochastic else 1
+                ro._rnn_em[e0:e0 + Eb, s0 + T].copy_(hstar.view(Eb, n, H))
+                h0 = K.H0Blocks(ro._rnn_em[e0, s0], (T + 1) * n, (T + 2) * n * H, Eb)
+            else:
+                h0_all = self.arena.get("pre.h0all", Eb, T + 1, n, H)
+                h0_all[:, :T].copy_(self._vh_carry(ro, e0, Eb))
+                h0_all[:, T].copy_(hstar.view(Eb, n, HC)[..., :H])
+                h0 = h0_all.view(-1, H)
+            act = self.Vh.forward(feats, n_seq=Eb * (T + 1) * n, T=1, h0=h0, tag="pre", train=False)
             Vh_buf[e0:e0 + Eb].copy_(act["v"].view(Eb, T + 1, n, nh))
         return Vl_buf, Vh_buf
 
@@ -552,14 +565,15 @@
               self.targets_hcbfcrpo(ro, step) if self.algo == "hcbfcrpo" else
               self.targets_lagr(ro, step) if lagr else self.targets(ro, det, step))
         th.append(_time.perf_counter())
-        idx_all = torch.from_numpy(np.ascontiguousarray(perm.astype(np.int64))).to(self.device)
+        perm = np.asarray(perm)
+        assert perm.size == 0 or (0 <= int(perm.min()) and int(perm.max()) < B), "perm holds env ids outside [0, B)"
+        idx_all = torch.from_numpy(np.ascontiguousarray(perm.astype(np.int32))).to(self.device)
         n_mb = B // Eb
         G = Eb * T
         R = G * n
         is_cuda = self.device.type == "cuda"
         reduce = self.allreduce is not None
         A = self.arena
-        mb_idx = A.get("mb.idx", Eb, dtype=torch.int64)
         mb_idx32 = A.get("mb.idx32", Eb, dtype=torch.int32)
         Ql_mb = A.get("mb.Ql", Eb, T)
         act_mb = A.get("mb.act", Eb, T, n, 2)
@@ -589,23 +603,22 @@
             side = self._net_streams() if (self.multi_stream and main is not None) else None
             self.stats[:3].zero_()
             feats = ctx["feats"] = self._block_feats("mb", ro, 0, Eb, 0, T, env_ids=mb_idx32)
-            torch.index_select(tg["Ql"], 0, mb_idx, out=Ql_mb)
+            pairs = [(tg["Ql"], Ql_mb)]
             if self.algo == "dgppo":
                 feats_det = self._block_feats("mbd", det, 0, Eb, 0, T, env_ids=mb_idx32)
+                full = None
                 if self.HC == H:
-                    torch.index_select(det.rnn_states, 0, mb_idx, out=h0_det)
+                    pairs.append((det.rnn_states, h0_det))
                 else:
                     full = A.get("mb.h0_det_full", Eb, T, n, self.HC)
-                    torch.index_select(det.rnn_states, 0, mb_idx, out=full)
-                    h0_det.copy_(full[..., :H])
-                torch.index_select(tg["Qh_det"], 0, mb_idx, out=Qh_det_mb)
+                    pairs.append((det.rnn_states, full))
+                pairs.append((tg["Qh_det"], Qh_det_mb))
             if lagr:
-                torch.index_select(tg["Qh"], 0, mb_idx, out=Qh_mb)
-                torch.index_select(tg["Vh"], 0, mb_idx, out=Vh_mb)
-                torch.index_select(tg["Ah"], 0, mb_idx, out=Ah_mb)
-            torch.index_select(ro.actions, 0, mb_idx, out=act_mb)
-            torch.index_select(ro.log_pis, 0, mb_idx, out=lp_old_mb)
-            torch.index_select(tg["adv"], 0, mb_idx, out=adv_mb)
+                pairs += [(tg["Qh"], Qh_mb), (tg["Vh"], Vh_mb), (tg["Ah"], Ah_mb)]
+            pairs += [(ro.actions, act_mb), (ro.log_pis, lp_old_mb), (tg["adv"], adv_mb)]
+            K.gather_rows(pairs, mb_idx32)
+            if self.algo == "dgppo" and full is not None:
+                h0_det.copy_(full[..., :H])
 
             def update_Vl():
                 act = self.Vl.forward(feats, n_seq=Eb * C, T=hp.rnn_step, h0=None, tag="tr")
@@ -683,15 +696,14 @@
         slot = None
         if self.use_graphs and is_cuda and self.grad_hook is None:
             key = (self.algo, B, Eb, ro.agent.data_ptr(), det.agent.data_ptr() if det is not None else 0,
-                   tg["adv"].data_ptr(), tg["Ql"].data_ptr(), mb_idx.data_ptr(), self._update_generation())
+                   tg["adv"].data_ptr(), tg["Ql"].data_ptr(), mb_idx32.data_ptr(), self._update_generation())
             slot = self._upd_graph
             if slot.get("key") != key:
                 slot.clear()
                 slot["key"] = key
         for mb in range(n_mb):
             self._mb = mb
-            mb_idx.copy_(idx_all[mb * Eb:(mb + 1) * Eb])
-            mb_idx32.copy_(mb_idx)
+            mb_idx32.copy_(idx_all[mb * Eb:(mb + 1) * Eb])
             if slot is not None and slot.get("graph") is not None:
                 slot["graph"].replay()
                 if reduce:
diff --git a/dgppo_amd/nets.py b/dgppo_amd/nets.py
--- a/dgppo_amd/nets.py
+++ b/dgppo_amd/nets.py
@@ -280,7 +280,11 @@
                          self.p("mlp.b2"), self.p("mlp.g2"), self.p("mlp.be2"), self.p("gru.Wi"), self.p("gru.bi"), gi, saves)
         assert n_seq * T == Rh, (n_seq, T, Rh)
         L, CD = self.rnn_layers, self.carry_dim
-        if h0 is not None:
+        h0_blocks = isinstance(h0, K.H0Blocks)
+        if h0_blocks:
+            assert self.rnn == "gru" and L == 1 and T == 1 and not train and self.kind != "policy", \
+                "a blocked h0 serves the one-cell GRU value nets' T = 1 inference pass"
+        elif h0 is not None:
             assert tuple(h0.shape) == (n_seq, CD), (tuple(h0.shape), n_seq, CD)
         if hs_out is not None:
             assert tuple(hs_out.shape) == (Rh, CD), (tuple(hs_out.shape), Rh, CD)
@@ -295,7 +299,10 @@
             act["hs"], act["hprev"], act["gates"] = hs, hprev, gates
         fused_tail = (simple and T == 1 and self.kind == "policy")
         if simple and not fused_tail:
-            K.gru_fwd(gi, self.p("gru.Wh"), self.p("gru.bhn"), h0, hs, hprev, gates, n_seq, T, n_inner)
+            if h0_blocks:
+                K.gru_fwd_h0_blocks(gi, self.p("gru.Wh"), self.p("gru.bhn"), h0, hs, hprev, gates, n_seq, T, n_inner)
+            else:
+                K.gru_fwd(gi, self.p("gru.Wh"), self.p("gru.bhn"), h0, hs, hprev, gates, n_seq, T, n_inner)
             if hprev_is_h0:
                 act["hprev"] = h0
         if self.rnn == "none":
diff --git a/dgppo_amd/ops_nn.py b/dgppo_amd/ops_nn.py
--- a/dgppo_amd/ops_nn.py
+++ b/dgppo_amd/ops_nn.py
@@ -488,6 +488,62 @@
     rc = N.lib().dgppo_gru_fwd(_p(gi), _p(Wh), _p(bhn), _p(h0), _p(hs), _p(hprev), _p(gates), n_seq, T, n_inner,
                                N.stream_ptr())
     N.check(rc, "dgppo_gru_fwd")
+
+
+class H0Blocks:
+
+    def __init__(self, base: torch.Tensor, rows_per_block: int, block_stride: int, n_blocks: int):
+        assert base.dtype == torch.float32 and base.is_cuda
+        st = base.untyped_storage()
+        last = base.storage_offset() + (n_blocks - 1) * block_stride + rows_per_block * 64
+        assert n_blocks >= 1 and last * 4 <= st.nbytes(), "H0Blocks: the blocks leave the storage of base"
+        self.base, self.rows_per_block, self.block_stride, self.n_blocks = base, int(rows_per_block), int(block_stride), int(n_blocks)
+
+    @property
+    def n_seq(self) -> int:
+        return self.n_blocks * self.rows_per_block
+
+
+def gru_fwd_h0_blocks(gi, Wh, bhn, h0: H0Blocks, hs, hprev, gates, n_seq, T, n_inner):
+    rows = n_seq * T
+    N.expect_shape(gi, (rows, 192), "gi")
+    N.expect_shape(hs, (rows, 64), "hs")
+    N.expect_shape(Wh, (64, 192), "Wh")
+    if n_seq > h0.n_seq:
+        raise ValueError(f"h0: {h0.n_blocks} blocks of {h0.rows_per_block} rows hold fewer than n_seq = {n_seq} carries")
+    FLOPS[0] += 2.0 * rows * 64 * 192
+    rc = N.lib().dgppo_gru_fwd_h0_blocks(_p(gi), _p(Wh), _p(bhn), C.c_void_p(h0.base.data_ptr()), h0.rows_per_block,
+                                         C.c_int64(h0.block_stride), _p(hs), _p(hprev), _p(gates), n_seq, T, n_inner,
+                                         N.stream_ptr())
+    N.check(rc, "dgppo_gru_fwd_h0_blocks")
+
+
+class GatherDesc(C.Structure):
+    _fields_ = [("src", C.c_void_p), ("dst", C.c_void_p), ("row_bytes", C.c_int64), ("src_stride", C.c_int64)]
+
+
+GATHER_MAX = 8
+
+
+def gather_rows(pairs, ids):
+    if ids.dtype != torch.int32 or not ids.is_cuda or not ids.is_contiguous():
+        raise TypeError("ids must be a contiguous int32 CUDA tensor")
+    n_ids = int(ids.numel())
+    if len(pairs) > GATHER_MAX:
+        raise ValueError(f"gather_rows takes at most {GATHER_MAX} tensors per launch, got {len(pairs)}")
+    descs = (GatherDesc * max(len(pairs), 1))()
+    for k, (src, dst) in enumerate(pairs):
+        if not (src.is_cuda and dst.is_cuda):
+            raise RuntimeError("gather_rows: tensors must live on the GPU (the HIP path has no CPU fallback)")
+        if src.dtype != dst.dtype or tuple(dst.shape) != (n_ids,) + tuple(src.shape[1:]):
+            raise ValueError(f"gather_rows: pair {k}: dst {tuple(dst.shape)} {dst.dtype} does not fit src {tuple(src.shape)} "
+                             f"{src.dtype} gathered by {n_ids} ids")
+        if not dst.is_contiguous() or (src.shape[0] > 0 and not src[0].is_contiguous()):
+            raise ValueError(f"gather_rows: pair {k}: dst and the rows of src must be contiguous")
+        row = (src[0].numel() if src.shape[0] > 0 else 0) * src.element_size()
+        descs[k] = GatherDesc(src.data_ptr(), dst.data_ptr(), row, src.stride(0) * src.element_size())
+    rc = N.lib().dgppo_gather_rows(descs, len(pairs), C.c_void_p(ids.data_ptr()), n_ids, N.stream_ptr())
+    N.check(rc, "dgppo_gather_rows")
 
 
 def gru_bwd(dhs, Wh, hprev, gates, dgi, dgh, n_seq, T, n_inner):
diff --git a/include/dgppo_hip.h b/include/dgppo_hip.h
--- a/include/dgppo_hip.h
+++ b/include/dgppo_hip.h
@@ -146,6 +146,14 @@
                             float* u, float* out, int32_t M, int32_t n_out, void* stream);
 int64_t dgppo_dense_bwd_w_workspace_bytes(int32_t K, int32_t N);
 
+#define DGPPO_GATHER_MAX 8
+typedef struct dgppo_gather_desc {
+  const void* src;
+  void* dst;
+  int64_t row_bytes, src_stride;
+} dgppo_gather_desc;
+int32_t dgppo_gather_rows(const dgppo_gather_desc* descs, int32_t n_desc, const int32_t* ids, int32_t n_ids, void* stream);
+
 int32_t dgppo_graph_feats(const dgppo_env_cfg* cfg, const float* agent, int64_t agent_se, int64_t agent_st,
                           const float* goal, const float* obst, const float* hits, int64_t hits_se, int64_t hits_st,
                           const int32_t* env_ids, int32_t n_env, int32_t n_time, float* Xa, float* Xo, float* efeat,
@@ -196,6 +204,9 @@
 
 int32_t dgppo_gru_fwd(const float* gi, const float* Wh, const float* bhn, const float* h0, float* hs, float* hprev,
                       float* gates, int32_t n_seq, int32_t T, int32_t n_inner, void* stream);
+int32_t dgppo_gru_fwd_h0_blocks(const float* gi, const float* Wh, const float* bhn, const float* h0,
+                                int32_t rows_per_block, int64_t block_stride, float* hs, float* hprev, float* gates,
+                                int32_t n_seq, int32_t T, int32_t n_inner, void* stream);
 int32_t dgppo_gru_bwd(const float* dhs, const float* Wh, const float* hprev, const float* gates, float* dgi,
                       float* dgh, int32_t n_seq, int32_t T, int32_t n_inner, void* stream);
 int32_t dgppo_gru_bwd_dhn(const float* dhs, const float* Wh, const float* hprev, const float* gates, float* dgi,
```

Result: faster. 4.198 million (median of 6 runs) (+2.7%).
